# rimelq/VISTAF-RoboSkin-Vision-Integrated-Multimodal-Sensor

Hardware: AMD Instinct MI355X
Metric: frames/sec (224x224 -> force-map) at batch 256 (higher is better)
Workload: dtype f32; 1 GPU; BASELINE configs[2]: batch 256/GPU of 224x224x3 fp16 fringe frames (256 distinct frames) -> 224x224 f32 depth map + force scalars, full FTP path (inpaint, demod, unwrap, detrend, compose, force tail), constants scaled-224; inputs resident in HBM; global_batch=256, input_dtype=fp16, constants=scaled, parallelism=dp1, inflight_batches=3, frames_with_nonzero_status=0

## Files before the change

### vistaf-roboskin-vision-integrated-multimodal-sensor_amd/_lib.py

```python
from __future__ import annotations

import ctypes
import os

_HERE = os.path.dirname(os.path.abspath(__file__))
LIB_PATH = os.path.join(_HERE, "libvistaf_ftp.so")

NSCALARS = 16
NREFINFO = 8
NCONTACT = 16
MAX_CONTACTS = 64

FMT_GRAY_U8, FMT_BGR_U8, FMT_GRAY_F16, FMT_BGR_F16 = 0, 1, 2, 3
FRAME_OK, FRAME_EMPTY_RELIABLE, FRAME_QUEUE_OVERFLOW, FRAME_NO_CARRIER = 0, 1, 2, 3
CURVE_TYPES = {"linear0": 0, "linear": 1, "poly2": 2, "sat_exp": 3, "growth": 4, "hinge_saturating": 5}

EXPORTS = [
    "vistaf_ftp_abi_version", "vistaf_ftp_last_error", "vistaf_ftp_default_config", "vistaf_ftp_create",
    "vistaf_ftp_set_reference", "vistaf_ftp_get_reference_info", "vistaf_ftp_predict_batch", "vistaf_ftp_predict_pairs",
    "vistaf_ftp_get_pair_info", "vistaf_ftp_contacts",
    "vistaf_ftp_get_intermediate", "vistaf_ftp_stage_count", "vistaf_ftp_stage_name",
    "vistaf_ftp_enable_stage_timing", "vistaf_ftp_get_stage_times", "vistaf_ftp_destroy",
    "vistaf_depth_map_to_volume", "vistaf_predict_force_from_volume",
]
TEST_EXPORTS = ["vistaf_ftp_test_set", "vistaf_ftp_test_select", "vistaf_ftp_test_polyfit", "vistaf_ftp_test_gauss"]
TEMP_EXPORTS = ["vistaf_tempseg_default_config", "vistaf_tempseg_create", "vistaf_tempseg_destroy", "vistaf_tempseg_segment",
                "vistaf_temp_feature_planes", "vistaf_temp_color_support",
                "vistaf_temp_clamp_map", "vistaf_temp_inpaint_map", "vistaf_temp_fuse_maps", "vistaf_temp_oriented_blur"]
TEMPSEG_NINFO = 16
TEMPMODEL_EXPORTS = ["vistaf_tmodel_create", "vistaf_tmodel_destroy", "vistaf_tmodel_predict_maps", "vistaf_tmodel_predict_rows"]
TSENSOR_EXPORTS = ["vistaf_tsensor_default_config", "vistaf_tsensor_create", "vistaf_tsensor_destroy", "vistaf_tsensor_predict",
                   "vistaf_tsensor_stats_create", "vistaf_tsensor_stats_destroy", "vistaf_tsensor_map_statistics"]
TSENSOR_NINFO, TSENSOR_NMASKS, TSENSOR_NSTATS = TEMPSEG_NINFO + 4, 5, 6
ALIGN_EXPORTS = [
    "vistaf_align_default_config", "vistaf_align_create", "vistaf_align_destroy", "vistaf_align_geometry",
    "vistaf_align_set_reference", "vistaf_align_batch",
]


class Curve(ctypes.Structure):
    _fields_ = [("type", ctypes.c_int32), ("reserved", ctypes.c_int32),
                ("a", ctypes.c_double), ("b", ctypes.c_double), ("c", ctypes.c_double)]


_INT_FIELDS = [
    "patch_half_width_bins", "dc_exclusion", "fft_pad_px", "roi_erode_px", "apod_taper_px", "reliable_edge_margin_px",
    "poly_order", "frontier_zero_band_px", "valid_close_kernel", "valid_close_iters", "bad_pixel_enable",
    "bad_dilate_ksize", "bad_dilate_iters", "bad_inpaint_radius", "dilate_kernel_size", "dilate_iters", "n_fft_peaks",
    "plane_order_for_removal", "irls_iters", "hole_neighborhood_px", "hole_min_dist_px", "inpaint_radius",
]
_DBL_FIELDS = [
    "pre_blur_sigma_px", "amp_valid_percentile", "quality_smooth_sigma_px", "reliable_smooth_sigma_px", "illum_sigma_px",
    "bad_intensity_percentile", "bad_gradient_percentile", "contact_core_percentile", "contact_percentile",
    "min_contact_frac", "max_contact_frac", "unreliable_smooth_sigma_px", "contact_blob_min_peak_mm",
    "contact_blob_min_peak_rel_frac", "peak_max_dy_from_center", "irls_c", "grating_pitch_mm", "depth_eps_mm", "hole_known_fraction",
]


class CConfig(ctypes.Structure):
    _fields_ = [(n, ctypes.c_int32) for n in _INT_FIELDS] + [(n, ctypes.c_double) for n in _DBL_FIELDS]


class CTempFuseConfig(ctypes.Structure):
    _fields_ = [(n, ctypes.c_double) for n in ("color_t_min", "color_t_max", "color_guard_band", "switch_margin_c", "final_t_min", "final_t_max")]


class CTempSegConfig(ctypes.Structure):
    _fields_ = [(n, ctypes.c_int32) for n in ("seg_band_radius", "seg_dc_exclusion", "seg_illum_sigma", "sat_thresh_gray", "sat_dilate_ksize",
                                                "post_close_kx", "post_close_ky", "post_open_kx", "post_open_ky", "n_peaks")] + \
               [("seg_peak_max_dy_from_center", ctypes.c_double)]


class CTSensorConfig(ctypes.Structure):
    _fields_ = [("seg", CTempSegConfig), ("fuse", CTempFuseConfig)] + \
               [(n, ctypes.c_int32) for n in ("blur_ksize", "color_support_dilate", "wide_inpaint_radius", "color_inpaint_radius")] + \
               [(n, ctypes.c_double) for n in ("color_chroma_min", "color_clamp_pad", "smooth_sigma_across", "smooth_sigma_along")]


_lib = None


def load():
    global _lib
    if _lib is not None:
        return _lib
    if not os.path.exists(LIB_PATH):
        raise RuntimeError(
            f"{LIB_PATH} is missing: build it with `python __graft_entry__.py` (hipcc --offload-arch=gfx950). "
            "This package has no CPU path."
        )
    lib = ctypes.CDLL(LIB_PATH)
    vp, ci, cd = ctypes.c_void_p, ctypes.c_int, ctypes.c_double
    lib.vistaf_ftp_abi_version.restype = ci
    lib.vistaf_ftp_last_error.restype = ctypes.c_char_p
    lib.vistaf_ftp_default_config.argtypes = [ctypes.POINTER(CConfig)]
    lib.vistaf_ftp_create.argtypes = [ctypes.POINTER(CConfig), ci, ci, ci, ci, ci, ci, ctypes.POINTER(Curve), ci,
                                      ctypes.POINTER(Curve), ctypes.POINTER(vp)]
    lib.vistaf_ftp_set_reference.argtypes = [vp, vp, ci, vp]
    lib.vistaf_ftp_get_reference_info.argtypes = [vp, ctypes.POINTER(cd)]
    lib.vistaf_ftp_predict_batch.argtypes = [vp, vp, ci, ci, vp, vp, vp, vp, vp]
    lib.vistaf_ftp_predict_pairs.argtypes = [vp, vp, vp, ci, ci, vp, vp, vp, vp, vp]
    lib.vistaf_ftp_get_pair_info.argtypes = [vp, ci, ctypes.POINTER(cd), vp]
    lib.vistaf_ftp_contacts.argtypes = [vp, ci, ci, vp, vp, vp, vp]
    lib.vistaf_ftp_get_intermediate.argtypes = [vp, ctypes.c_char_p, vp, ci, ctypes.POINTER(ctypes.c_size_t), vp]
    lib.vistaf_ftp_stage_count.restype = ci
    lib.vistaf_ftp_stage_name.restype = ctypes.c_char_p
    lib.vistaf_ftp_stage_name.argtypes = [ci]
    lib.vistaf_ftp_enable_stage_timing.argtypes = [vp, ci]
    lib.vistaf_ftp_get_stage_times.argtypes = [vp, ctypes.POINTER(ctypes.c_float), ci]
    lib.vistaf_ftp_destroy.argtypes = [vp]
    lib.vistaf_ftp_destroy.restype = None
    lib.vistaf_depth_map_to_volume.argtypes = [vp, vp, ci, ci, ci, cd, cd, vp, vp]
    lib.vistaf_predict_force_from_volume.argtypes = [ctypes.POINTER(Curve), cd, ctypes.POINTER(cd)]
    lib.vistaf_ftp_test_set.argtypes = [vp, ctypes.c_char_p, ci]
    lib.vistaf_ftp_test_select.argtypes = [vp, vp, ctypes.c_size_t, vp, ci, vp, ci, vp, vp, ci, ci, ci, vp]
    lib.vistaf_ftp_test_polyfit.argtypes = [vp, vp, ci, ci, ctypes.c_float, ci, ci, vp, vp, ci, ci, ci, ci, vp]
    lib.vistaf_ftp_test_gauss.argtypes = [vp, vp, cd, ci, ci, ci, vp]
    lib.vistaf_tempseg_default_config.argtypes = [ctypes.POINTER(CTempSegConfig)]
    lib.vistaf_tempseg_create.argtypes = [ctypes.POINTER(CTempSegConfig), ci, ci, ctypes.POINTER(vp)]
    lib.vistaf_tempseg_destroy.argtypes = [vp]
    lib.vistaf_tempseg_destroy.restype = None
    lib.vistaf_tempseg_segment.argtypes = [vp, vp, vp, vp, vp, vp, vp, ctypes.POINTER(cd), vp]
    lib.vistaf_temp_feature_planes.argtypes = [vp, vp, ci, vp, vp, vp, vp, vp]
    lib.vistaf_temp_color_support.argtypes = [vp, vp, vp, vp, vp, vp, cd, ci, vp, vp, vp]
    lib.vistaf_temp_clamp_map.argtypes = [vp, vp, vp, cd, cd, vp, vp]
    lib.vistaf_temp_inpaint_map.argtypes = [vp, vp, vp, ci, vp, vp]
    lib.vistaf_temp_fuse_maps.argtypes = [vp, vp, vp, vp, ctypes.POINTER(CTempFuseConfig), vp, vp, ctypes.POINTER(ctypes.c_int64), vp]
    lib.vistaf_temp_oriented_blur.argtypes = [vp, vp, vp, cd, cd, cd, vp, vp]
    i32p, dp = ctypes.POINTER(ctypes.c_int32), ctypes.POINTER(cd)
    lib.vistaf_tmodel_create.argtypes = [ci, i32p, dp, dp, ci, ci, ci, i32p, dp, cd, ci, dp, dp, cd, cd, ci, ctypes.POINTER(vp)]
    lib.vistaf_tmodel_destroy.argtypes = [vp]
    lib.vistaf_tmodel_destroy.restype = None
    lib.vistaf_tmodel_predict_maps.argtypes = [ci, ctypes.POINTER(vp), ctypes.POINTER(vp), ctypes.POINTER(vp), ctypes.POINTER(vp), ctypes.c_int64,
                                               ctypes.c_int64, vp]
    lib.vistaf_tmodel_predict_rows.argtypes = [vp, vp, ci, ctypes.c_int64, vp, vp]
    lib.vistaf_tsensor_default_config.argtypes = [ctypes.POINTER(CTSensorConfig)]
    lib.vistaf_tsensor_create.argtypes = [ctypes.POINTER(CTSensorConfig), ci, ci, vp, vp, ctypes.POINTER(vp)]
    lib.vistaf_tsensor_destroy.argtypes = [vp]
    lib.vistaf_tsensor_destroy.restype = None
    lib.vistaf_tsensor_predict.argtypes = [vp, vp, vp, vp, vp, vp, vp, vp, ctypes.POINTER(cd), vp, ctypes.POINTER(cd), vp]
    lib.vistaf_tsensor_stats_create.argtypes = [ci, ci, ctypes.POINTER(vp)]
    lib.vistaf_tsensor_stats_destroy.argtypes = [vp]
    lib.vistaf_tsensor_stats_destroy.restype = None
    lib.vistaf_tsensor_map_statistics.argtypes = [vp, vp, vp, vp, ctypes.POINTER(cd), vp]
    for fn in EXPORTS + ALIGN_EXPORTS + TEST_EXPORTS + TEMP_EXPORTS + TEMPMODEL_EXPORTS + TSENSOR_EXPORTS:
        getattr(lib, fn)
    _lib = lib
    return lib


def check(rc: int):
    if rc != 0:
        msg = load().vistaf_ftp_last_error().decode("utf-8", "replace")
        if rc == -1:
            raise ValueError(msg)
        raise RuntimeError(f"vistaf_ftp error {rc}: {msg}")
```

### vistaf-roboskin-vision-integrated-multimodal-sensor_amd/csrc/api.hip

```cpp
#include <hip/hip_runtime.h>
#include <algorithm>
#include <cmath>
#include <cstdio>
#include <cstdlib>
#include <cstring>
#include <map>
#include <string>
#include <vector>

#include "../../include/vistaf_ftp.h"
#include "kernels.hpp"

using namespace vf;
#include "test_hooks.h"
#ifdef VISTAF_DEBUG
namespace vf { void telea_debug_dump(); void telea_window_debug_dump(int B); void telea_window_mw_debug_dump(int B); void fit_debug_dump(); void unwrap_big_debug_dump(); void unwrap_batch_debug_dump(); }
#endif

static thread_local std::string g_err;
static int fail(int code, const std::string &msg) { g_err = msg; return code; }
namespace vf { int set_error(int code, const std::string &msg) { return fail(code, msg); } }
#define HIPCHK(x)                                                                                         \
    do {                                                                                                  \
        hipError_t e_ = (x);                                                                              \
        if (e_ != hipSuccess) return fail(VISTAF_E_HIP, std::string(#x) + ": " + hipGetErrorString(e_)); \
    } while (0)

namespace {

struct GKern { float *d = nullptr; int k = 0; };

enum Stage { ST_GRAY_BAD = 0, ST_INPAINT, ST_PREPROC, ST_DEMOD, ST_RELIABLE, ST_UNWRAP_RANK, ST_UNWRAP, ST_UNWRAP_TREE, ST_DETREND, ST_SMOOTH_FLIP, ST_COMPOSE, ST_MM_BLOB,
             ST_TAIL, ST_COUNT };
const char *kStageNames[ST_COUNT] = {"gray+badpix", "inpaint (k_telea_window_mw)", "illum+blur+apod+median", "pruned-dft demod", "reliable mask",
                                     "unwrap check (k_unwrap_fast)", "unwrap flood (fallback)", "unwrap tree (fallback)", "detrend (3x IRLS)", "smooth+flip", "frontier+compose", "mm+blob filter", "tail"};

int cv_round(double v) { return (int)std::nearbyint(v); }

}

struct vistaf_ftp_handle {
    vistaf_ftp_config cfg;
    int h = 0, w = 0, P = 0, cx = 0, cy = 0, r = 0, maxB = 0;
    Curve hcurve, fcurve;
    int use_neg = 1;
    bool have_ref = false;

    uint8_t *roi = nullptr, *valid = nullptr;
    float *apo = nullptr, *roi_den = nullptr;
    GKern g_illum, g_pre, g_qual, g_rel, g_unrel;
    RowSpanSE se_bad, se_close, se_contact;

    double peak_x = 0, peak_y = 0, kx = 0, ky = 0, period = 0, mm_per_px = 0;
    int Hf = 0, Wf = 0, ph = 0, pw = 0, pmax = 0;
    double2 *Ex = nullptr, *Ey = nullptr, *Gx = nullptr, *Gy = nullptr, *cref = nullptr;
    float *win = nullptr, *amp_ref = nullptr;
    CarrierGeom *geom = nullptr;
    double2 *Exf = nullptr, *Eyf = nullptr, *search_tmp = nullptr;
    double *search_mag = nullptr, *search_peaks = nullptr;
    int search_cap = 0;
    CarrierGeom *pgeom = nullptr;
    double2 *pEx = nullptr, *pEy = nullptr, *pGx = nullptr, *pGy = nullptr, *pcref = nullptr;
    float *pamp_ref = nullptr, *pwin = nullptr, *hann_tab = nullptr;
    bool pairs_ready = false;
    Tiers tiers;
    bool keep_planes = false;

    std::map<std::string, std::pair<void *, size_t>> named;
    std::vector<void *> allocs;
    float *img, *grad, *tmpf, *blurA, *inorm, *iw, *amp, *prod, *quality, *wrapped, *unwrapped, *phase1, *resid0, *detr, *z0, *mplane,
        *num, *den, *hmap, *dist, *z0f, *snum, *unitless, *depth;
    double2 *field, *patch;
    double2 *tmpT;
    uint8_t *bad0, *bad1, *rel0, *rel1, *rel2, *reliable, *contact, *contact_d, *background, *cand, *kept;
    uint8_t *out_rel = nullptr, *hole_cand = nullptr;
    float *hole_med = nullptr, *hole_fill = nullptr;
    int32_t *labels, *area, *rowdist, *parent;
    unsigned int *peak_bits;
    uint16_t *morph_pre;
    void *inpaint_scratch, *inpaint_cl_scratch, *inpaint_win_scratch, *unwrap_scratch;
    void *big_scratch = nullptr;
    int32_t *unwrap_need;
    float *thr_hi, *thr_g, *mu, *amp_thr, *thr3, *thr_used, *bg_med, *core_thr, *core_med, *coef;
    int *cnt_a, *cnt_valid, *rel_count, *contact_count, *bg_count, *bad_count, *flipped;
    unsigned int *gmax;
    int32_t *status;
    int32_t *big_only;
    unsigned long long *cc_best;
    double *scalars;
    float *req_hi, *req_g, *req_med, *req_amp, *req_contact, *req_core;

    ContactScratch contacts_ws{};
    int last_batch = 0;
    bool last_pairs = false;

    bool timing = false;
    hipEvent_t ev[ST_COUNT + 1];
    bool ev_made = false;
    float stage_ms[ST_COUNT];
};

namespace {

template <typename T>
int dalloc(vistaf_ftp_handle *hd, T **p, size_t count, const char *name = nullptr, size_t per_frame = 0)
{
    void *q = nullptr;
    hipError_t e = hipMalloc(&q, count * sizeof(T) + 256);
    if (e != hipSuccess) return fail(VISTAF_E_HIP, std::string("hipMalloc: ") + hipGetErrorString(e));
    hd->allocs.push_back(q);
    *p = (T *)q;
    if (name) hd->named[name] = {q, per_frame};
    return 0;
}

int gauss_taps(double sigma, std::vector<float> &f)
{
    int n = cv_round(sigma * 4 * 2 + 1) | 1;
    if (n > 511) return fail(VISTAF_E_INVALID, "gaussian sigma too large (ksize > 511)");
    std::vector<double> t(n);
    double s2 = -0.5 / (sigma * sigma), sum = 0;
    for (int i = 0; i < n; i++) { double x = i - (n - 1) * 0.5; t[i] = std::exp(s2 * x * x); sum += t[i]; }
    f.resize(n);
    for (int i = 0; i < n; i++) f[i] = (float)(t[i] * (1.0 / sum));
    return 0;
}

int make_gkern(vistaf_ftp_handle *hd, double sigma, GKern *g)
{
    g->k = 0; g->d = nullptr;
    if (!(sigma > 0)) return 0;
    std::vector<float> f;
    int rc = gauss_taps(sigma, f);
    if (rc) return rc;
    const int n = (int)f.size();
    rc = dalloc(hd, &g->d, n);
    if (rc) return rc;
    if (hipMemcpy(g->d, f.data(), n * sizeof(float), hipMemcpyHostToDevice) != hipSuccess) return fail(VISTAF_E_HIP, "memcpy gkern");
    g->k = n;
    return 0;
}

bool chamfer_ball(float margin, RowSpanSE *se)
{
    const long long HV = 62587, DG = 89738;
    const long long M = (long long)std::floor((double)margin * 65536.0);
    if (M < 0) return false;
    const int R = (int)(M / HV);
    if (2 * R + 1 > 33 || R > 63) return false;
    se->k = std::max(3, 2 * R + 1);
    const int r = se->k / 2;
    for (int i = 0; i < se->k; i++) {
        const int dy = std::abs(i - r);
        int a = -1;
        for (int dx = 0; dx <= 63; dx++) {
            const long long mn = std::min(dx, dy), mx = std::max(dx, dy);
            if (HV * (mx - mn) + DG * mn <= M) a = dx; else break;
        }
        if (a < 0) { se->lo[i] = 1; se->hi[i] = -1; }
        else { se->lo[i] = (int8_t)-a; se->hi[i] = (int8_t)a; }
    }
    return true;
}

int make_se(int k, RowSpanSE *se, bool force_odd = true)
{
    if (force_odd) k = std::max(3, k | 1);
    if (k > 33) return fail(VISTAF_E_INVALID, "structuring element larger than 33");
    se->k = k;
    int r = k / 2, c = k / 2;
    double inv_r2 = r ? 1.0 / ((double)r * r) : 0.0;
    for (int i = 0; i < k; i++) {
        int dy = i - r;
        int dx = cv_round(c * std::sqrt((r * r - dy * dy) * inv_r2));
        int j1 = std::max(c - dx, 0), j2 = std::min(c + dx + 1, k);
        se->lo[i] = (int8_t)(j1 - c);
        se->hi[i] = (int8_t)(j2 - 1 - c);
    }
    return 0;
}

void blur(vistaf_ftp_handle *hd, const float *src, float *dst, const GKern &g, int B, hipStream_t st)
{
    launch_gauss_blur(src, hd->tmpf, dst, g.d, g.k, B, hd->h, hd->w, st);
}

bool fuses(const vistaf_ftp_handle *hd, const GKern &g) { return hd->tiers.fused_chains && g.k > 0 && g.k <= GF_MAXK; }

float q32_of(double pct) { return (float)pct / 100.0f; }

int upload_req(vistaf_ftp_handle *hd, float **d, const std::vector<float> &v)
{
    int rc = dalloc(hd, d, v.size());
    if (rc) return rc;
    if (hipMemcpy(*d, v.data(), v.size() * sizeof(float), hipMemcpyHostToDevice) != hipSuccess) return fail(VISTAF_E_HIP, "memcpy req");
    return 0;
}

void preprocess(vistaf_ftp_handle *hd, const void *frames, int format, int nframes, hipStream_t st, bool timed, const void *frames2 = nullptr)
{
    const vistaf_ftp_config &c = hd->cfg;
    int h = hd->h, w = hd->w, P = hd->P;
    if (timed) hipEventRecord(hd->ev[ST_GRAY_BAD], st);
    launch_to_gray(frames, format, hd->img, nframes, P, st);
    if (frames2) launch_to_gray(frames2, format, hd->img + (size_t)nframes * P, nframes, P, st);
    const int B = frames2 ? 2 * nframes : nframes;
    hipMemsetAsync(hd->bad_count, 0, sizeof(int) * B, st);
    if (c.bad_pixel_enable) {
        launch_sobel_mag(hd->img, hd->grad, B, h, w, st);
        launch_select(hd->img, hd->valid, 0, nullptr, false, hd->req_hi, 1, hd->thr_hi, hd->cnt_valid, B, P, st, hd->tiers.big_chain ? hd->big_scratch : nullptr);
        launch_select(hd->grad, hd->valid, 0, nullptr, false, hd->req_g, 1, hd->thr_g, nullptr, B, P, st, hd->tiers.big_chain ? hd->big_scratch : nullptr);
        launch_bad_flags(hd->img, hd->grad, hd->valid, hd->thr_hi, hd->thr_g, hd->bad0, B, P, st);
        uint8_t *src = hd->bad0, *dst = hd->bad1;
        if (c.bad_dilate_ksize > 1)
            for (int it = 0; it < c.bad_dilate_iters; it++) { launch_morph(src, dst, B, h, w, hd->se_bad, true, nullptr, nullptr, st); std::swap(src, dst); }
        if (src != hd->bad1) hipMemcpyAsync(hd->bad1, src, (size_t)B * P, hipMemcpyDeviceToDevice, st);
        launch_count_u8(hd->bad1, hd->bad_count, B, P, st);
        {
            int range = std::min(100, std::max(1, cv_round((double)c.bad_inpaint_radius)));
            const uint8_t *seq_mask = hd->bad1;
            const int32_t *only = nullptr;
            int mode = hd->tiers.inpaint;
            if (mode == 2 && (size_t)h * w > (size_t)8 * 14464) mode = 0;
            if (mode == 0 && inpaint_clusters_supported(range)) {
                uint8_t *bad_big = nullptr;
                ClusterPlanes left;
                launch_inpaint_clusters(hd->img, hd->bad1, range, hd->inpaint_cl_scratch, &bad_big, &left, B, h, w, st);
                if (timed) hipEventRecord(hd->ev[ST_INPAINT], st);
                launch_inpaint_big_clusters(hd->img, bad_big, range, hd->inpaint_scratch, hd->status, left, B, h, w, st, hd->tiers.big_queue_lds != 0,
                                            hd->tiers.big_gq_cap);
                if (hd->tiers.big_fallback) {
                    launch_inpaint_big_handback(hd->status, hd->big_only, B, st);
                    launch_inpaint_telea(hd->img, bad_big, range, hd->inpaint_scratch, hd->status, hd->big_only, B, h, w, st);
                }
            } else {
                if (timed && mode == 1) hipEventRecord(hd->ev[ST_INPAINT], st);
                if (mode != 1) only = launch_inpaint_window(hd->img, seq_mask, range, hd->inpaint_win_scratch, B, h, w, st, timed ? hd->ev[ST_INPAINT] : nullptr,
                                                               hd->tiers.telea_two_tier != 0, hd->tiers.telea_mw != 0);
                launch_inpaint_telea(hd->img, seq_mask, range, hd->inpaint_scratch, hd->status, only, B, h, w, st);
            }
        }
    } else if (timed) hipEventRecord(hd->ev[ST_INPAINT], st);
    if (timed) hipEventRecord(hd->ev[ST_PREPROC], st);
    blur(hd, hd->img, hd->blurA, hd->g_illum, B, st);
    if (fuses(hd, hd->g_pre)) launch_illum_pre_apod(hd->img, hd->blurA, hd->apo, hd->iw, hd->g_pre.d, hd->g_pre.k, B, h, w, st);
    else {
        launch_illum_norm(hd->img, hd->blurA, hd->inorm, B, P, st);
        const float *in = hd->inorm;
        if (hd->g_pre.k) { blur(hd, hd->inorm, hd->blurA, hd->g_pre, B, st); in = hd->blurA; }
        launch_mul_static(in, hd->apo, hd->iw, B, P, st);
    }
    launch_select(hd->iw, hd->valid, 0, nullptr, false, hd->req_med, 1, hd->mu, nullptr, B, P, st, hd->tiers.big_chain ? hd->big_scratch : nullptr);
}

std::vector<float> hann_patch(int ph, int pw)
{
    auto hann = [](int M, int i) -> float { return M == 1 ? 1.0f : (float)(0.5 + 0.5 * std::cos(3.14159265358979323846 * (double)(1 - M + 2 * i) / (double)(M - 1))); };
    std::vector<float> win((size_t)ph * pw);
    for (int a = 0; a < ph; a++)
        for (int c = 0; c < pw; c++) win[(size_t)a * pw + c] = hann(ph, a) * hann(pw, c);
    return win;
}

template <typename T>
int upload(vistaf_ftp_handle *hd, T **d, const std::vector<T> &v)
{
    int rc = dalloc(hd, d, v.size());
    if (rc) return rc;
    if (hipMemcpy(*d, v.data(), v.size() * sizeof(T), hipMemcpyHostToDevice) != hipSuccess) return fail(VISTAF_E_HIP, "memcpy upload");
    return 0;
}

}

extern "C" {

int vistaf_ftp_abi_version(void) { return VISTAF_FTP_ABI_VERSION; }
const char *vistaf_ftp_last_error(void) { return g_err.c_str(); }

int vistaf_ftp_default_config(vistaf_ftp_config *c)
{
    if (!c) return fail(VISTAF_E_INVALID, "null config");
    memset(c, 0, sizeof(*c));
    c->patch_half_width_bins = 10; c->dc_exclusion = 10; c->fft_pad_px = 96; c->roi_erode_px = 0; c->apod_taper_px = 120;
    c->reliable_edge_margin_px = 6; c->poly_order = 2; c->frontier_zero_band_px = 200; c->valid_close_kernel = 7;
    c->valid_close_iters = 1; c->bad_pixel_enable = 1; c->bad_dilate_ksize = 5; c->bad_dilate_iters = 1; c->bad_inpaint_radius = 3;
    c->dilate_kernel_size = 15; c->dilate_iters = 2; c->n_fft_peaks = 12; c->plane_order_for_removal = 1; c->irls_iters = 6;
    c->pre_blur_sigma_px = 1.5; c->amp_valid_percentile = 25.0; c->quality_smooth_sigma_px = 6.0; c->reliable_smooth_sigma_px = 2.5;
    c->illum_sigma_px = 45.0; c->bad_intensity_percentile = 99.9; c->bad_gradient_percentile = 99.7; c->contact_core_percentile = 8.0;
    c->contact_percentile = 92.0; c->min_contact_frac = 0.002; c->max_contact_frac = 0.40; c->unreliable_smooth_sigma_px = 9.0;
    c->contact_blob_min_peak_mm = 0.1; c->contact_blob_min_peak_rel_frac = 1.0 / 3.0; c->peak_max_dy_from_center = 0.12;
    c->irls_c = 4.685; c->grating_pitch_mm = 2.0; c->depth_eps_mm = 0.01;
    c->hole_neighborhood_px = 11; c->hole_min_dist_px = 4; c->inpaint_radius = 5; c->hole_known_fraction = 0.70;
    return 0;
}

void vistaf_ftp_destroy(vistaf_ftp_handle *hd)
{
    if (!hd) return;
    for (void *p : hd->allocs) hipFree(p);
    if (hd->ev_made) for (int i = 0; i <= ST_COUNT; i++) hipEventDestroy(hd->ev[i]);
    delete hd;
}

int vistaf_ftp_create(const vistaf_ftp_config *cfg, int h, int w, int cx, int cy, int r, int max_batch,
                      const vistaf_curve *height_curve, int use_negated_height, const vistaf_curve *force_curve,
                      vistaf_ftp_handle **out)
{
    if (!cfg || !out || !height_curve || !force_curve) return fail(VISTAF_E_INVALID, "null argument");
    if (h < 8 || w < 8 || max_batch < 1 || r < 1) return fail(VISTAF_E_INVALID, "bad geometry");
    if (height_curve->type < 0 || height_curve->type > 5 || force_curve->type < 0 || force_curve->type > 5)
        return fail(VISTAF_E_INVALID, "Unknown model type in calibration");
    if (cfg->poly_order < 1 || cfg->poly_order > 2 || cfg->plane_order_for_removal < 0 || cfg->plane_order_for_removal > 2)
        return fail(VISTAF_E_INVALID, "polynomial order must be 1 or 2 (plane_order_for_removal: 0 = no pre-removal)");
    if (cfg->irls_iters < 1) return fail(VISTAF_E_INVALID, "irls_iters must be >= 1 (robust_polyfit2d binds no coefficients otherwise)");
    if (cfg->n_fft_peaks < 1 || cfg->n_fft_peaks > 64) return fail(VISTAF_E_INVALID, "n_fft_peaks must be 1..64");
    int bwp = std::max(3, cfg->patch_half_width_bins);
    if (2 * bwp + 1 > 255) return fail(VISTAF_E_INVALID, "patch too wide");
    vistaf_ftp_handle *hd = new vistaf_ftp_handle();
    hd->cfg = *cfg; hd->h = h; hd->w = w; hd->P = h * w; hd->cx = cx; hd->cy = cy; hd->r = r; hd->maxB = max_batch;
    hd->hcurve = Curve{height_curve->type, height_curve->a, height_curve->b, height_curve->c};
    hd->fcurve = Curve{force_curve->type, force_curve->a, force_curve->b, force_curve->c};
    hd->use_neg = use_negated_height ? 1 : 0;
    int P = hd->P;
    size_t n = (size_t)max_batch * P;
    int rc = 0;
#define TRY(x) do { rc = (x); if (rc) { vistaf_ftp_destroy(hd); return rc; } } while (0)
    std::vector<uint8_t> roi(P), valid(P);
    std::vector<float> apo(P), roif(P);
    int r_valid = std::max(0, r - cfg->roi_erode_px);
    double r_in = std::max(0.0, (double)(r - cfg->apod_taper_px));
    for (int y = 0; y < h; y++)
        for (int x = 0; x < w; x++) {
            long d2 = (long)(x - cx) * (x - cx) + (long)(y - cy) * (y - cy);
            roi[(size_t)y * w + x] = d2 <= (long)r_valid * r_valid;
            double d = std::sqrt((double)d2);
            float a = 0.f;
            if (d <= r_in) a = 1.0f;
            else if (d <= r && cfg->apod_taper_px > 0) {
                double t = (d - r_in) / std::max(1e-6, (double)cfg->apod_taper_px);
                a = (float)(0.5 * (1.0 + std::cos(3.14159265358979323846 * t)));
            }
            apo[(size_t)y * w + x] = a;
            valid[(size_t)y * w + x] = a > 1e-6f;
            roif[(size_t)y * w + x] = roi[(size_t)y * w + x] ? 1.f : 0.f;
        }
    TRY(upload(hd, &hd->roi, roi)); TRY(upload(hd, &hd->valid, valid)); TRY(upload(hd, &hd->apo, apo));
    hd->named["roi"] = {hd->roi, 0};
    TRY(make_gkern(hd, cfg->illum_sigma_px, &hd->g_illum));
    if (!hd->g_illum.k) { vistaf_ftp_destroy(hd); return fail(VISTAF_E_INVALID, "illum_sigma_px must be > 0"); }
    TRY(make_gkern(hd, cfg->pre_blur_sigma_px, &hd->g_pre));
    TRY(make_gkern(hd, cfg->quality_smooth_sigma_px, &hd->g_qual));
    TRY(make_gkern(hd, cfg->reliable_smooth_sigma_px, &hd->g_rel));
    TRY(make_gkern(hd, cfg->unreliable_smooth_sigma_px, &hd->g_unrel));
    TRY(make_se(cfg->bad_dilate_ksize, &hd->se_bad));
    TRY(make_se(cfg->valid_close_kernel, &hd->se_close));
    {
        int k = cfg->dilate_kernel_size;
        if (k < 1 || k > 33) { vistaf_ftp_destroy(hd); return fail(VISTAF_E_INVALID, "dilate_kernel_size out of range"); }
        TRY(make_se(k, &hd->se_contact, false));
    }
    if (!(cfg->reliable_smooth_sigma_px > 0)) {
        if (cfg->hole_neighborhood_px < 1 || cfg->hole_neighborhood_px > 255 || cfg->hole_min_dist_px < 0 || cfg->inpaint_radius < 1 ||
            !(cfg->hole_known_fraction >= 0.0)) {
            vistaf_ftp_destroy(hd);
            return fail(VISTAF_E_INVALID, "hole-stage constants out of range");
        }
    }
#define PLANE(T, name) TRY(dalloc(hd, &hd->name, n, #name, (size_t)P * sizeof(T)))
    PLANE(float, img); PLANE(float, grad); PLANE(float, tmpf); PLANE(float, blurA); PLANE(float, inorm); PLANE(float, iw);
    PLANE(float, amp); PLANE(float, prod); PLANE(float, quality); PLANE(float, wrapped); PLANE(float, unwrapped); PLANE(float, phase1);
    PLANE(float, resid0); PLANE(float, detr); PLANE(float, z0); PLANE(float, mplane); PLANE(float, num); PLANE(float, den);
    PLANE(float, hmap); PLANE(float, dist); PLANE(float, z0f); PLANE(float, snum); PLANE(float, unitless); PLANE(float, depth);
    PLANE(double2, field);
    PLANE(uint8_t, bad0); PLANE(uint8_t, bad1); PLANE(uint8_t, rel0); PLANE(uint8_t, rel1); PLANE(uint8_t, rel2); PLANE(uint8_t, reliable);
    PLANE(uint8_t, contact); PLANE(uint8_t, contact_d); PLANE(uint8_t, background); PLANE(uint8_t, cand); PLANE(uint8_t, kept);
    if (!(cfg->reliable_smooth_sigma_px > 0)) { PLANE(uint8_t, out_rel); PLANE(uint8_t, hole_cand); }
    PLANE(int32_t, labels); PLANE(int32_t, area); PLANE(int32_t, rowdist); PLANE(int32_t, parent);
    PLANE(unsigned int, peak_bits);
    PLANE(uint16_t, morph_pre);
#undef PLANE
    {
        void *p = nullptr;
        TRY(dalloc(hd, (uint8_t **)&p, inpaint_scratch_bytes_per_frame(h, w) * max_batch)); hd->inpaint_scratch = p;
        TRY(dalloc(hd, (uint8_t **)&p, inpaint_cl_scratch_bytes_per_frame(h, w) * max_batch + 2048)); hd->inpaint_cl_scratch = p;
        TRY(dalloc(hd, (uint8_t **)&p, inpaint_win_scratch_bytes(max_batch))); hd->inpaint_win_scratch = p;
        TRY(dalloc(hd, (uint8_t **)&p, unwrap_scratch_bytes_per_frame(h, w) * max_batch + 1024)); hd->unwrap_scratch = p;
        if ((size_t)h * w >= 262144) { TRY(dalloc(hd, (uint8_t **)&p, big_scratch_bytes(max_batch, h, w))); hd->big_scratch = p; }
        TRY(dalloc(hd, &hd->unwrap_need, (size_t)max_batch, "unwrap_need", sizeof(int32_t)));
        HIPCHK(hipMemset(hd->unwrap_need, 0xff, (size_t)max_batch * sizeof(int32_t)));
    }
    int pmax = 2 * bwp + 1;
    hd->pmax = pmax;
    TRY(dalloc(hd, &hd->patch, (size_t)max_batch * pmax * pmax, "patch", (size_t)pmax * pmax * sizeof(double2)));
    TRY(dalloc(hd, &hd->tmpT, (size_t)max_batch * (size_t)std::max(h, w) * pmax));
    TRY(dalloc(hd, &hd->Ex, (size_t)w * pmax)); TRY(dalloc(hd, &hd->Gx, (size_t)w * pmax));
    TRY(dalloc(hd, &hd->Ey, (size_t)h * pmax)); TRY(dalloc(hd, &hd->Gy, (size_t)h * pmax));
    TRY(dalloc(hd, &hd->win, (size_t)pmax * pmax)); TRY(dalloc(hd, &hd->geom, 1));
    TRY(dalloc(hd, &hd->cref, (size_t)P)); TRY(dalloc(hd, &hd->amp_ref, (size_t)P));
    hd->named["cref"] = {hd->cref, 0}; hd->named["amp_ref"] = {hd->amp_ref, 0};
    size_t mb = max_batch;
    TRY(dalloc(hd, &hd->thr_hi, mb)); TRY(dalloc(hd, &hd->thr_g, mb)); TRY(dalloc(hd, &hd->mu, mb)); TRY(dalloc(hd, &hd->amp_thr, mb));
    TRY(dalloc(hd, &hd->thr3, mb * 3)); TRY(dalloc(hd, &hd->thr_used, mb)); TRY(dalloc(hd, &hd->bg_med, mb));
    TRY(dalloc(hd, &hd->core_thr, mb)); TRY(dalloc(hd, &hd->core_med, mb)); TRY(dalloc(hd, &hd->coef, mb * 6));
    TRY(dalloc(hd, &hd->cnt_a, mb)); TRY(dalloc(hd, &hd->cnt_valid, mb)); TRY(dalloc(hd, &hd->rel_count, mb));
    TRY(dalloc(hd, &hd->contact_count, mb)); TRY(dalloc(hd, &hd->bg_count, mb)); TRY(dalloc(hd, &hd->bad_count, mb));
    TRY(dalloc(hd, &hd->flipped, mb)); TRY(dalloc(hd, &hd->gmax, mb)); TRY(dalloc(hd, &hd->status, mb)); TRY(dalloc(hd, &hd->cc_best, mb));
    TRY(dalloc(hd, &hd->big_only, mb));
    TRY(dalloc(hd, &hd->scalars, mb * VISTAF_NSCALARS));
    TRY(dalloc(hd, &hd->hole_med, mb)); TRY(dalloc(hd, &hd->hole_fill, mb));
    {
        ContactScratch &cs = hd->contacts_ws;
        cs.cap = contact_root_capacity(h, w);
        TRY(dalloc(hd, &cs.arg, n)); TRY(dalloc(hd, &cs.list, mb * cs.cap)); TRY(dalloc(hd, &cs.nroots, mb)); TRY(dalloc(hd, &cs.nsel, mb));
        TRY(dalloc(hd, &cs.selkey, mb * VISTAF_MAX_CONTACTS)); TRY(dalloc(hd, &cs.part, contact_part_words(max_batch, P)));
    }
    hd->named["mu"] = {hd->mu, sizeof(float)}; hd->named["thr_hi"] = {hd->thr_hi, sizeof(float)}; hd->named["thr_g"] = {hd->thr_g, sizeof(float)};
    hd->named["coef"] = {hd->coef, 6 * sizeof(float)}; hd->named["thr3"] = {hd->thr3, 3 * sizeof(float)};
    hd->named["core_thr"] = {hd->core_thr, sizeof(float)}; hd->named["core_med"] = {hd->core_med, sizeof(float)};
    TRY(upload_req(hd, &hd->req_hi, {q32_of(cfg->bad_intensity_percentile)}));
    TRY(upload_req(hd, &hd->req_g, {q32_of(cfg->bad_gradient_percentile)}));
    TRY(upload_req(hd, &hd->req_med, {-1.0f}));
    TRY(upload_req(hd, &hd->req_amp, {q32_of(cfg->amp_valid_percentile)}));
    TRY(upload_req(hd, &hd->req_contact, {q32_of(cfg->contact_percentile), q32_of(95.0), q32_of(98.0)}));
    TRY(upload_req(hd, &hd->req_core, {q32_of(cfg->contact_core_percentile)}));
    TRY(dalloc(hd, &hd->roi_den, (size_t)P));
    if (hd->g_unrel.k) {
        float *tmp_roi = nullptr;
        TRY(upload(hd, &tmp_roi, roif));
        launch_gauss_rows(tmp_roi, hd->tmpf, hd->g_unrel.d, hd->g_unrel.k, 1, h, w, 0);
        launch_gauss_cols(hd->tmpf, hd->roi_den, hd->g_unrel.d, hd->g_unrel.k, 1, h, w, 0);
        std::vector<float> hden(P);
        if (hipMemcpy(hden.data(), hd->roi_den, P * sizeof(float), hipMemcpyDeviceToHost) != hipSuccess) { vistaf_ftp_destroy(hd); return fail(VISTAF_E_HIP, "roi_den readback"); }
        for (int i = 0; i < P; i++) hden[i] = hden[i] + 1e-6f;
        if (hipMemcpy(hd->roi_den, hden.data(), P * sizeof(float), hipMemcpyHostToDevice) != hipSuccess) { vistaf_ftp_destroy(hd); return fail(VISTAF_E_HIP, "roi_den upload"); }
    }
    hd->Hf = h + 2 * std::max(0, cfg->fft_pad_px);
    hd->Wf = w + 2 * std::max(0, cfg->fft_pad_px);
    if (hipDeviceSynchronize() != hipSuccess) { vistaf_ftp_destroy(hd); return fail(VISTAF_E_HIP, "create sync"); }
#undef TRY
    *out = hd;
    return 0;
}

static int reference_search(vistaf_ftp_handle *hd, int nb, CarrierGeom *geom_dev, hipStream_t st)
{
    const vistaf_ftp_config &c = hd->cfg;
    const int h = hd->h, w = hd->w, Hf = hd->Hf, Wf = hd->Wf, pad = std::max(0, c.fft_pad_px);
    if (hd->search_cap < nb) {
        int rc;
        if (!hd->Exf) {
            if ((rc = dalloc(hd, &hd->Exf, (size_t)w * (Wf / 2 + 1))) || (rc = dalloc(hd, &hd->Eyf, (size_t)Hf * h))) return rc;
            launch_build_full_tables(hd->Exf, hd->Eyf, h, w, pad, Hf, Wf, st);
        }
        const int cap = std::min(std::max(nb, 2 * hd->search_cap), std::max(nb, hd->maxB));
        if (hd->search_cap > 0) {
            HIPCHK(hipStreamSynchronize(st));
            for (void *q : {(void *)hd->search_tmp, (void *)hd->search_mag, (void *)hd->search_peaks}) {
                auto it = std::find(hd->allocs.begin(), hd->allocs.end(), q);
                if (it != hd->allocs.end()) { hipFree(q); hd->allocs.erase(it); }
            }
            hd->search_tmp = nullptr; hd->search_mag = nullptr; hd->search_peaks = nullptr; hd->search_cap = 0;
        }
        if ((rc = dalloc(hd, &hd->search_tmp, (size_t)cap * h * (Wf / 2 + 1) + 64)) || (rc = dalloc(hd, &hd->search_mag, (size_t)cap * Hf * Wf)) ||
            (rc = dalloc(hd, &hd->search_peaks, (size_t)cap * 192)))
            return rc;
        hd->search_cap = cap;
    }
    const int npk = c.n_fft_peaks;
    launch_dft_full_mag(hd->iw, hd->mu, hd->Exf, hd->Eyf, hd->search_tmp, hd->search_mag, nb, h, w, Hf, Wf, st);
    launch_top_peaks(hd->search_mag, nb, Hf, Wf, c.dc_exclusion, npk, hd->search_peaks, st);
    launch_carrier_choose(hd->search_peaks, npk, hd->search_mag, Hf, Wf, std::max(3, c.patch_half_width_bins), c.peak_max_dy_from_center, geom_dev, nb, st);
    return 0;
}

int vistaf_ftp_set_reference(vistaf_ftp_handle *hd, const void *d_ref, int format, void *stream)
{
    if (!hd || !d_ref) return fail(VISTAF_E_INVALID, "null argument");
    if (format < 0 || format > 3) return fail(VISTAF_E_INVALID, "bad frame format");
    hipStream_t st = (hipStream_t)stream;
    const vistaf_ftp_config &c = hd->cfg;
    int h = hd->h, w = hd->w, P = hd->P, Hf = hd->Hf, Wf = hd->Wf, pad = std::max(0, c.fft_pad_px);
    hd->have_ref = false;
    HIPCHK(hipMemsetAsync(hd->status, 0, sizeof(int32_t) * hd->maxB, st));
    preprocess(hd, d_ref, format, 1, st, false);
    int rc = reference_search(hd, 1, hd->geom, st);
    if (rc) return rc;
    CarrierGeom g;
    HIPCHK(hipMemcpyAsync(&g, hd->geom, sizeof(g), hipMemcpyDeviceToHost, st));
    HIPCHK(hipStreamSynchronize(st));
    if (!g.ok) return fail(VISTAF_E_NOCARRIER, "no carrier peak in the reference spectrum");
    hd->peak_x = g.peak_x; hd->peak_y = g.peak_y; hd->kx = g.kx; hd->ky = g.ky;
    hd->ph = g.ph; hd->pw = g.pw;
    {
        std::vector<float> win = hann_patch(g.ph, g.pw);
        HIPCHK(hipMemcpyAsync(hd->win, win.data(), win.size() * sizeof(float), hipMemcpyHostToDevice, st));
        HIPCHK(hipStreamSynchronize(st));
    }
    launch_build_tables(hd->geom, 0, hd->Ex, hd->Ey, hd->Gx, hd->Gy, 0, 0, 1, h, w, pad, Hf, Wf, hd->pmax, st);
    launch_dft_forward(hd->iw, hd->mu, hd->Ex, hd->Ey, 0, 0, hd->win, hd->tmpT, hd->patch, hd->pmax * hd->pmax, 1, h, w, hd->ph, hd->pw, st);
    launch_dft_inverse(hd->patch, hd->pmax * hd->pmax, hd->Gx, hd->Gy, 0, 0, hd->tmpT, hd->cref, hd->amp_ref, nullptr, nullptr, 0, nullptr, nullptr,
                       1, h, w, hd->ph, hd->pw, st);
    HIPCHK(hipStreamSynchronize(st));
    hd->period = g.period;
    hd->mm_per_px = hd->period > 1e-12 ? c.grating_pitch_mm / hd->period : 0.0;
    hd->have_ref = true;
    (void)P;
    return 0;
}

int vistaf_ftp_get_reference_info(const vistaf_ftp_handle *hd, double *o)
{
    if (!hd || !o) return fail(VISTAF_E_INVALID, "null argument");
    if (!hd->have_ref) return fail(VISTAF_E_STATE, "set_reference has not been called");
    o[0] = hd->peak_x; o[1] = hd->peak_y; o[2] = hd->kx; o[3] = hd->ky; o[4] = hd->Hf; o[5] = hd->Wf; o[6] = hd->period; o[7] = hd->mm_per_px;
    return 0;
}

static int post_demod(vistaf_ftp_handle *hd, int B, float *d_height_mm, uint8_t *d_reliable, double *d_scalars, int32_t *d_status,
                      const CarrierGeom *pair_geom, hipStream_t st, const int *bad_count = nullptr)
{
    if (!bad_count) bad_count = hd->bad_count;
    const vistaf_ftp_config &c = hd->cfg;
    int h = hd->h, w = hd->w, P = hd->P;
    bool timed = hd->timing;

    if (timed) hipEventRecord(hd->ev[ST_RELIABLE], st);
    const float *qual = hd->prod;
    if (hd->g_qual.k) { blur(hd, hd->prod, hd->quality, hd->g_qual, B, st); qual = hd->quality; }
    else HIPCHK(hipMemcpyAsync(hd->quality, hd->prod, (size_t)B * P * sizeof(float), hipMemcpyDeviceToDevice, st));
    qual = hd->quality;
    launch_select(qual, hd->roi, 0, nullptr, false, hd->req_amp, 1, hd->amp_thr, nullptr, B, P, st, hd->tiers.big_chain ? hd->big_scratch : nullptr);
    launch_threshold_mask(qual, hd->roi, hd->amp_thr, hd->rel0, B, P, st);
    {
        uint8_t *src = hd->rel0, *dst = hd->rel1;
        if (c.valid_close_iters >= 1 && 2 * c.valid_close_iters <= 4) {
            int ops[4];
            for (int it = 0; it < c.valid_close_iters; it++) { ops[it] = 1; ops[c.valid_close_iters + it] = 0; }
            launch_morph_seq(hd->rel0, hd->rel1, hd->rel2, B, h, w, hd->se_close, ops, 2 * c.valid_close_iters, hd->roi, nullptr, st, hd->morph_pre);
            src = hd->rel1;
        } else {
            for (int it = 0; it < 2 * c.valid_close_iters; it++) {
                const bool dil = it < c.valid_close_iters;
                launch_morph(src, dst, B, h, w, hd->se_close, dil, it == 2 * c.valid_close_iters - 1 ? hd->roi : nullptr, nullptr, st, hd->morph_pre);
                src = dst;
                dst = dst == hd->rel1 ? hd->rel2 : hd->rel1;
            }
        }
        launch_cc_label(src, hd->labels, B, h, w, st);
        launch_cc_largest(hd->labels, hd->area, hd->cc_best, hd->roi, hd->rel2, B, P, st);
    }
    if (c.reliable_edge_margin_px > 0) {
        RowSpanSE ball;
        if (chamfer_ball((float)c.reliable_edge_margin_px, &ball))
            launch_morph(hd->rel2, hd->reliable, B, h, w, ball, false, nullptr, nullptr, st, hd->morph_pre);
        else {
            launch_chamfer(hd->rel2, false, hd->rowdist, hd->dist, B, h, w, c.reliable_edge_margin_px + 1, st, hd->tiers.chamfer_twopass != 0);
            launch_erode_by_dist(hd->dist, hd->rel2, (float)c.reliable_edge_margin_px, hd->reliable, B, P, st);
        }
    } else HIPCHK(hipMemcpyAsync(hd->reliable, hd->rel2, (size_t)B * P, hipMemcpyDeviceToDevice, st));
    launch_count_u8(hd->reliable, hd->rel_count, B, P, st);
    launch_mark_empty(hd->rel_count, hd->status, B, st);

    if (timed) hipEventRecord(hd->ev[ST_UNWRAP_RANK], st);
    launch_unwrap(hd->wrapped, qual, hd->reliable, hd->unwrapped, hd->parent, hd->unwrap_scratch, hd->status, B, h, w, st,
                  timed ? hd->ev[ST_UNWRAP_TREE] : nullptr, timed ? hd->ev[ST_UNWRAP] : nullptr, hd->tiers.big_flood_handback != 0, hd->tiers.unwrap_fast ? hd->unwrap_need : nullptr);

    if (timed) hipEventRecord(hd->ev[ST_DETREND], st);
    if (c.plane_order_for_removal > 0)
        launch_robust_polyfit(hd->unwrapped, hd->reliable, c.plane_order_for_removal, c.irls_iters, (float)c.irls_c, 200, 500, hd->coef, hd->phase1, B, h, w, st, hd->tiers.big_chain ? hd->big_scratch : nullptr);
    else
        HIPCHK(hipMemcpyAsync(hd->phase1, hd->unwrapped, (size_t)B * P * sizeof(float), hipMemcpyDeviceToDevice, st));
    launch_robust_polyfit(hd->phase1, hd->reliable, c.poly_order, c.irls_iters, (float)c.irls_c, 200, 0, hd->coef, hd->resid0, B, h, w, st, hd->tiers.big_chain ? hd->big_scratch : nullptr);
    launch_select(hd->resid0, hd->reliable, (size_t)P, nullptr, true, hd->req_contact, 3, hd->thr3, nullptr, B, P, st, hd->tiers.big_chain ? hd->big_scratch : nullptr);
    launch_contact_mask(hd->resid0, hd->reliable, hd->thr3, hd->rel_count, hd->contact_count, c.min_contact_frac, c.max_contact_frac,
                        hd->contact, hd->thr_used, B, P, st);
    {
        int iters = c.dilate_iters;
        if (iters <= 0) HIPCHK(hipMemcpyAsync(hd->contact_d, hd->contact, (size_t)B * P, hipMemcpyDeviceToDevice, st));
        else if (iters <= 4) {
            int ops[4] = {1, 1, 1, 1};
            launch_morph_seq(hd->contact, hd->contact_d, hd->cand, B, h, w, hd->se_contact, ops, iters, nullptr, hd->reliable, st, hd->morph_pre);
        } else {
            uint8_t *src = hd->contact, *dst = hd->contact_d;
            uint8_t *bufs[2] = {hd->contact_d, hd->cand};
            for (int it = 0; it < iters; it++) {
                dst = bufs[it & 1];
                launch_morph(src, dst, B, h, w, hd->se_contact, true, nullptr, it == iters - 1 ? hd->reliable : nullptr, st, hd->morph_pre);
                src = dst;
            }
            if (src != hd->contact_d) HIPCHK(hipMemcpyAsync(hd->contact_d, src, (size_t)B * P, hipMemcpyDeviceToDevice, st));
        }
    }
    launch_background(hd->reliable, hd->contact_d, hd->rel_count, hd->bg_count, hd->background, B, P, st);
    launch_robust_polyfit(hd->phase1, hd->background, c.poly_order, c.irls_iters, (float)c.irls_c, 200, 0, hd->coef, hd->detr, B, h, w, st, hd->tiers.big_chain ? hd->big_scratch : nullptr);
    launch_select(hd->detr, hd->background, (size_t)P, nullptr, false, hd->req_med, 1, hd->bg_med, nullptr, B, P, st, hd->tiers.big_chain ? hd->big_scratch : nullptr);

    if (timed) hipEventRecord(hd->ev[ST_SMOOTH_FLIP], st);
    const bool smooth_rel = hd->g_rel.k > 0;
    if (fuses(hd, hd->g_rel)) launch_smooth_reliable(hd->detr, hd->bg_med, hd->reliable, hd->hmap, hd->g_rel.d, hd->g_rel.k, B, h, w, st);
    else if (smooth_rel) {
        launch_sub_scalar_mask(hd->detr, hd->bg_med, hd->reliable, hd->z0, hd->mplane, B, P, st);
        blur(hd, hd->z0, hd->num, hd->g_rel, B, st);
        blur(hd, hd->mplane, hd->den, hd->g_rel, B, st);
        launch_div_planes(hd->num, hd->den, hd->hmap, B, P, st);
    } else launch_zeroed_keep_nan(hd->detr, hd->bg_med, hd->reliable, hd->hmap, B, P, st);
    launch_select(hd->hmap, hd->reliable, (size_t)P, nullptr, false, hd->req_core, 1, hd->core_thr, nullptr, B, P, st, hd->tiers.big_chain ? hd->big_scratch : nullptr);
    launch_select(hd->hmap, hd->reliable, (size_t)P, hd->core_thr, false, hd->req_med, 1, hd->core_med, nullptr, B, P, st, hd->tiers.big_chain ? hd->big_scratch : nullptr);
    launch_core_flip(hd->hmap, hd->core_med, hd->flipped, B, P, st);

    const uint8_t *orel = hd->reliable;
    if (!smooth_rel) {
        const int ksz = std::max(3, c.hole_neighborhood_px | 1);
        launch_chamfer(hd->reliable, false, hd->rowdist, hd->dist, B, h, w, c.hole_min_dist_px + 1, st, hd->tiers.chamfer_twopass != 0);
        launch_hole_candidates(hd->hmap, hd->reliable, hd->dist, ksz, (float)c.hole_known_fraction, (float)c.hole_min_dist_px, hd->hole_cand, B, h, w, st);
        launch_select(hd->hmap, hd->reliable, (size_t)P, nullptr, false, hd->req_med, 1, hd->hole_med, nullptr, B, P, st, hd->tiers.big_chain ? hd->big_scratch : nullptr);
        launch_hole_tmp(hd->hmap, hd->reliable, hd->hole_cand, hd->hole_med, hd->z0, B, P, st);
        launch_select(hd->z0, hd->reliable, (size_t)P, nullptr, false, hd->req_med, 1, hd->hole_fill, nullptr, B, P, st, hd->tiers.big_chain ? hd->big_scratch : nullptr);
        launch_hole_zin(hd->z0, hd->hole_fill, B, P, st);
        {
            const int range = std::min(100, std::max(1, cv_round((double)c.inpaint_radius)));
            const int32_t *only = nullptr;
            if (hd->tiers.inpaint != 1) only = launch_inpaint_window(hd->z0, hd->hole_cand, range, hd->inpaint_win_scratch, B, h, w, st, nullptr, hd->tiers.telea_two_tier != 0, hd->tiers.telea_mw != 0);
            launch_inpaint_telea(hd->z0, hd->hole_cand, range, hd->inpaint_scratch, hd->status, only, B, h, w, st);
        }
        launch_hole_merge(hd->hmap, hd->reliable, hd->hole_cand, hd->z0, hd->out_rel, B, P, st);
        orel = hd->out_rel;
    }

    if (timed) hipEventRecord(hd->ev[ST_COMPOSE], st);
    bool use_band = c.frontier_zero_band_px > 0;
    float band = (float)c.frontier_zero_band_px;
    if (use_band) launch_chamfer_pair(orel, hd->rowdist, hd->dist, hd->area, hd->depth, B, h, w, c.frontier_zero_band_px + 2, st, hd->tiers.chamfer_twopass != 0);
    else HIPCHK(hipMemsetAsync(hd->dist, 0x7f, (size_t)B * P * sizeof(float), st));
    const bool fuse_compose = fuses(hd, hd->g_unrel);
    if (fuse_compose)
        launch_compose_finalize_mm(hd->hmap, orel, hd->roi, hd->dist, use_band ? band : 1.0f, hd->roi_den, use_band ? hd->depth : hd->dist, band,
                                   use_band ? 1 : 0, hd->hcurve, hd->use_neg, hd->unitless, hd->depth, hd->cand, hd->gmax, hd->g_unrel.d, hd->g_unrel.k,
                                   B, h, w, st);
    else {
        launch_frontier_compose(hd->hmap, orel, hd->roi, hd->dist, use_band ? band : 1.0f, hd->z0f, B, P, st);
        if (hd->g_unrel.k) blur(hd, hd->z0f, hd->snum, hd->g_unrel, B, st);
        launch_finalize_unitless(hd->z0f, hd->g_unrel.k ? hd->snum : nullptr, hd->roi_den, orel, hd->roi, use_band ? hd->depth : hd->dist, band, use_band ? 1 : 0,
                                 hd->unitless, B, P, st);
    }

    if (timed) hipEventRecord(hd->ev[ST_MM_BLOB], st);
    if (!fuse_compose) launch_to_mm(hd->unitless, hd->roi, hd->hcurve, hd->use_neg, hd->depth, hd->cand, hd->gmax, B, P, st);
    launch_cc_label(hd->cand, hd->labels, B, h, w, st);
    launch_blob_filter(hd->depth, hd->cand, hd->labels, hd->peak_bits, hd->gmax, c.contact_blob_min_peak_mm,
                       c.contact_blob_min_peak_rel_frac, hd->kept, B, P, st);

    if (timed) hipEventRecord(hd->ev[ST_TAIL], st);
    PostParams pp;
    pp.mm_per_px = hd->mm_per_px; pp.depth_eps_mm = c.depth_eps_mm; pp.period_px = hd->period; pp.force_curve = hd->fcurve;
    pp.pair_geom = pair_geom; pp.grating_pitch_mm = c.grating_pitch_mm;
    launch_tail(hd->depth, nullptr, hd->unitless, hd->roi, pp, hd->scalars, VISTAF_NSCALARS, nullptr, B, P, st, hd->tiers.big_chain ? hd->big_scratch : nullptr,
                hd->big_scratch ? big_scratch_bytes(hd->maxB, h, w) : 0);
    launch_fill_scalars(hd->scalars, VISTAF_NSCALARS, hd->rel_count, hd->flipped, hd->amp_thr, hd->thr_used, hd->bg_med, bad_count, B, st);
    launch_copy_out(hd->depth, orel, hd->status, d_height_mm, d_reliable, B, P, st);
    if (d_scalars) HIPCHK(hipMemcpyAsync(d_scalars, hd->scalars, sizeof(double) * VISTAF_NSCALARS * B, hipMemcpyDeviceToDevice, st));
    if (d_status) HIPCHK(hipMemcpyAsync(d_status, hd->status, sizeof(int32_t) * B, hipMemcpyDeviceToDevice, st));
    if (timed) {
        hipEventRecord(hd->ev[ST_COUNT], st);
        hipEventSynchronize(hd->ev[ST_COUNT]);
        for (int i = 0; i < ST_COUNT; i++) hipEventElapsedTime(&hd->stage_ms[i], hd->ev[i], hd->ev[i + 1]);
    }
#ifdef VISTAF_DEBUG
    if (getenv("VISTAF_TELEA_DBG")) { hipStreamSynchronize(st); telea_debug_dump(); telea_window_debug_dump(B); telea_window_mw_debug_dump(B); fit_debug_dump(); unwrap_big_debug_dump(); unwrap_batch_debug_dump(); }
#endif
    hipError_t e = hipGetLastError();
    if (e != hipSuccess) return fail(VISTAF_E_HIP, std::string("launch: ") + hipGetErrorString(e));
    hd->last_batch = B; hd->last_pairs = pair_geom != nullptr;
    return 0;
}

int vistaf_ftp_predict_batch(vistaf_ftp_handle *hd, const void *d_frames, int format, int B, float *d_height_mm, uint8_t *d_reliable,
                             double *d_scalars, int32_t *d_status, void *stream)
{
    if (!hd || !d_frames) return fail(VISTAF_E_INVALID, "null argument");
    if (!hd->have_ref) return fail(VISTAF_E_STATE, "set_reference has not been called");
    if (B < 1 || B > hd->maxB) return fail(VISTAF_E_STATE, "batch exceeds max_batch");
    if (format < 0 || format > 3) return fail(VISTAF_E_INVALID, "bad frame format");
    if (!(hd->period > 1e-12)) return fail(VISTAF_E_STATE, "Invalid estimated_grating_period_px");
    hipStream_t st = (hipStream_t)stream;
    int h = hd->h, w = hd->w;
    bool timed = hd->timing;
    if (timed && !hd->ev_made) { for (int i = 0; i <= ST_COUNT; i++) hipEventCreate(&hd->ev[i]); hd->ev_made = true; }
    HIPCHK(hipMemsetAsync(hd->status, 0, sizeof(int32_t) * B, st));

    preprocess(hd, d_frames, format, B, st, timed);

    if (timed) hipEventRecord(hd->ev[ST_DEMOD], st);
    launch_dft_forward(hd->iw, hd->mu, hd->Ex, hd->Ey, 0, 0, hd->win, hd->tmpT, hd->patch, hd->pmax * hd->pmax, B, h, w, hd->ph, hd->pw, st);
    launch_dft_inverse(hd->patch, hd->pmax * hd->pmax, hd->Gx, hd->Gy, 0, 0, hd->tmpT, hd->keep_planes ? hd->field : nullptr, hd->amp, hd->cref,
                       hd->amp_ref, 0, hd->prod, hd->wrapped, B, h, w, hd->ph, hd->pw, st);
    return post_demod(hd, B, d_height_mm, d_reliable, d_scalars, d_status, nullptr, st);
}

int vistaf_ftp_predict_pairs(vistaf_ftp_handle *hd, const void *d_refs, const void *d_defs, int format, int B, float *d_height_mm,
                             uint8_t *d_reliable, double *d_scalars, int32_t *d_status, void *stream)
{
    if (!hd || !d_refs || !d_defs) return fail(VISTAF_E_INVALID, "null argument");
    if (B < 1 || B > hd->maxB) return fail(VISTAF_E_STATE, "batch exceeds max_batch");
    if (format < 0 || format > 3) return fail(VISTAF_E_INVALID, "bad frame format");
    hipStream_t st = (hipStream_t)stream;
    const vistaf_ftp_config &c = hd->cfg;
    int h = hd->h, w = hd->w, P = hd->P, pad = std::max(0, c.fft_pad_px), pm = hd->pmax;
    bool timed = hd->timing;
    if (timed && !hd->ev_made) { for (int i = 0; i <= ST_COUNT; i++) hipEventCreate(&hd->ev[i]); hd->ev_made = true; }
    if (!hd->pairs_ready) {
        int rc;
        size_t mb = hd->maxB;
        if ((rc = dalloc(hd, &hd->pgeom, mb)) || (rc = dalloc(hd, &hd->pEx, mb * w * pm)) || (rc = dalloc(hd, &hd->pGx, mb * w * pm)) ||
            (rc = dalloc(hd, &hd->pEy, mb * h * pm)) || (rc = dalloc(hd, &hd->pGy, mb * h * pm)) || (rc = dalloc(hd, &hd->pcref, mb * P)) ||
            (rc = dalloc(hd, &hd->pamp_ref, mb * P)) || (rc = dalloc(hd, &hd->pwin, mb * pm * pm)) || (rc = dalloc(hd, &hd->hann_tab, (size_t)(pm + 1) * pm)))
            return rc;
        std::vector<float> tab((size_t)(pm + 1) * pm, 0.0f);
        for (int M = 1; M <= pm; M++) {
            const std::vector<float> row = hann_patch(1, M);
            std::copy(row.begin(), row.end(), tab.begin() + (size_t)M * pm);
        }
        HIPCHK(hipMemcpy(hd->hann_tab, tab.data(), tab.size() * sizeof(float), hipMemcpyHostToDevice));
        hd->pairs_ready = true;
    }
    HIPCHK(hipMemsetAsync(hd->status, 0, sizeof(int32_t) * B, st));
    const size_t sx = (size_t)w * pm, sy = (size_t)h * pm;
    const bool together = 2 * B <= hd->maxB;
    const float *iw_def = hd->iw, *mu_def = hd->mu;
    const int *bad_def = hd->bad_count;
    if (together) {
        HIPCHK(hipMemsetAsync(hd->status + B, 0, sizeof(int32_t) * B, st));
        preprocess(hd, d_refs, format, B, st, timed, d_defs);
        iw_def = hd->iw + (size_t)B * P; mu_def = hd->mu + B; bad_def = hd->bad_count + B;
    } else preprocess(hd, d_refs, format, B, st, false);
    int rc = reference_search(hd, B, hd->pgeom, st);
    if (rc) return rc;
    launch_pair_status(hd->pgeom, pm, hd->status, together ? hd->status + B : nullptr, B, st);
    launch_build_tables(hd->pgeom, 1, hd->pEx, hd->pEy, hd->pGx, hd->pGy, sx, sy, B, h, w, pad, hd->Hf, hd->Wf, pm, st, hd->hann_tab, hd->pwin);
    launch_dft_forward(hd->iw, hd->mu, hd->pEx, hd->pEy, sx, sy, hd->pwin, hd->tmpT, hd->patch, pm * pm, B, h, w, pm, pm, st, pm * pm);
    launch_dft_inverse(hd->patch, pm * pm, hd->pGx, hd->pGy, sx, sy, hd->tmpT, hd->pcref, hd->pamp_ref, nullptr, nullptr, 0, nullptr, nullptr, B, h, w,
                       pm, pm, st, hd->pgeom);
    if (!together) preprocess(hd, d_defs, format, B, st, timed);
    if (timed) hipEventRecord(hd->ev[ST_DEMOD], st);
    launch_dft_forward(iw_def, mu_def, hd->pEx, hd->pEy, sx, sy, hd->pwin, hd->tmpT, hd->patch, pm * pm, B, h, w, pm, pm, st, pm * pm);
    launch_dft_inverse(hd->patch, pm * pm, hd->pGx, hd->pGy, sx, sy, hd->tmpT, hd->keep_planes ? hd->field : nullptr, hd->amp, hd->pcref, hd->pamp_ref,
                       (size_t)P, hd->prod, hd->wrapped, B, h, w, pm, pm, st, hd->pgeom);
    return post_demod(hd, B, d_height_mm, d_reliable, d_scalars, d_status, hd->pgeom, st, bad_def);
}

int vistaf_ftp_get_pair_info(vistaf_ftp_handle *hd, int batch, double *out , void *stream)
{
    if (!hd || !out) return fail(VISTAF_E_INVALID, "null argument");
    if (!hd->pairs_ready || batch < 1 || batch > hd->maxB) return fail(VISTAF_E_STATE, "predict_pairs has not been called");
    std::vector<CarrierGeom> g(batch);
    HIPCHK(hipMemcpyAsync(g.data(), hd->pgeom, sizeof(CarrierGeom) * batch, hipMemcpyDeviceToHost, (hipStream_t)stream));
    HIPCHK(hipStreamSynchronize((hipStream_t)stream));
    for (int b = 0; b < batch; b++) {
        double *o = out + (size_t)b * VISTAF_NREFINFO;
        o[0] = g[b].peak_x; o[1] = g[b].peak_y; o[2] = g[b].kx; o[3] = g[b].ky; o[4] = hd->Hf; o[5] = hd->Wf; o[6] = g[b].period;
        o[7] = g[b].period > 1e-12 ? hd->cfg.grating_pitch_mm / g[b].period : 0.0;
    }
    return 0;
}

int vistaf_ftp_contacts(vistaf_ftp_handle *hd, int B, int max_contacts, double *d_contacts, int32_t *d_count, int8_t *d_contact_index, void *stream)
{
    if (!hd || !d_contacts || !d_count) return fail(VISTAF_E_INVALID, "null argument");
    if (max_contacts < 1 || max_contacts > VISTAF_MAX_CONTACTS) return fail(VISTAF_E_INVALID, "max_contacts must be 1..64");
    if (hd->last_batch == 0) return fail(VISTAF_E_STATE, "no predict_batch / predict_pairs before contacts");
    if (B != hd->last_batch) return fail(VISTAF_E_STATE, "batch differs from the last predict's");
    const vistaf_ftp_config &c = hd->cfg;
    PostParams pp;
    pp.mm_per_px = hd->mm_per_px; pp.depth_eps_mm = c.depth_eps_mm; pp.period_px = hd->period; pp.force_curve = hd->fcurve;
    pp.pair_geom = hd->last_pairs ? hd->pgeom : nullptr; pp.grating_pitch_mm = c.grating_pitch_mm;
    launch_contacts(hd->depth, hd->kept, hd->labels, hd->peak_bits, hd->status, pp, hd->contacts_ws, max_contacts, d_contacts, VISTAF_NCONTACT, d_count,
                    d_contact_index, B, hd->h, hd->w, (hipStream_t)stream);
    hipError_t e = hipGetLastError();
    if (e != hipSuccess) return fail(VISTAF_E_HIP, std::string("launch: ") + hipGetErrorString(e));
    return 0;
}

int vistaf_ftp_get_intermediate(vistaf_ftp_handle *hd, const char *name, void *d_dst, int batch, size_t *bytes_per_frame, void *stream)
{
    if (!hd || !name) return fail(VISTAF_E_INVALID, "null argument");
    auto it = hd->named.find(name);
    if (it == hd->named.end()) return fail(VISTAF_E_INVALID, std::string("unknown intermediate: ") + name);
    size_t per = it->second.second;
    size_t total = per ? per * (size_t)batch : (std::string(name) == "cref" ? (size_t)hd->P * sizeof(double2) : std::string(name) == "amp_ref" ? (size_t)hd->P * sizeof(float) : (size_t)hd->P);
    if (bytes_per_frame) *bytes_per_frame = per ? per : total;
    if (d_dst) HIPCHK(hipMemcpyAsync(d_dst, it->second.first, total, hipMemcpyDeviceToDevice, (hipStream_t)stream));
    return 0;
}

int vistaf_ftp_stage_count(void) { return ST_COUNT; }
const char *vistaf_ftp_stage_name(int i) { return (i >= 0 && i < ST_COUNT) ? kStageNames[i] : ""; }
int vistaf_ftp_enable_stage_timing(vistaf_ftp_handle *hd, int enable)
{
    if (!hd) return fail(VISTAF_E_INVALID, "null handle");
    hd->timing = enable != 0;
    return 0;
}
int vistaf_ftp_get_stage_times(vistaf_ftp_handle *hd, float *ms_out, int n)
{
    if (!hd || !ms_out) return fail(VISTAF_E_INVALID, "null argument");
    for (int i = 0; i < n && i < ST_COUNT; i++) ms_out[i] = hd->stage_ms[i];
    return 0;
}

int vistaf_ftp_test_set(vistaf_ftp_handle *hd, const char *name, int value)
{
    if (!hd || !name) return fail(VISTAF_E_INVALID, "null argument");
    const std::string n(name);
    if (n == "inpaint_tier" && value >= 0 && value <= 2) hd->tiers.inpaint = value;
    else if (n == "big_flood_handback") hd->tiers.big_flood_handback = value != 0;
    else if (n == "chamfer_twopass") hd->tiers.chamfer_twopass = value != 0;
    else if (n == "telea_two_tier") hd->tiers.telea_two_tier = value != 0;
    else if (n == "telea_mw") hd->tiers.telea_mw = value != 0;
    else if (n == "big_queue_lds") hd->tiers.big_queue_lds = value != 0;
    else if (n == "big_gq_cap" && (value == 0 || (value >= 64 && (value & (value - 1)) == 0))) hd->tiers.big_gq_cap = value;
    else if (n == "big_fallback") hd->tiers.big_fallback = value != 0;
    else if (n == "unwrap_fast") hd->tiers.unwrap_fast = value != 0;
    else if (n == "big_chain") hd->tiers.big_chain = value != 0;
    else if (n == "fused_chains") hd->tiers.fused_chains = value != 0;
    else if (n == "keep_planes") hd->keep_planes = value != 0;
    else return fail(VISTAF_E_INVALID, "unknown test hook or value: " + n);
    return 0;
}

namespace {
int hook_scratch(int variant, int B, int h, int w, bool chain_ok, void **scratch)
{
    *scratch = nullptr;
    if (variant < 0 || variant > 2) return fail(VISTAF_E_INVALID, "variant must be 0, 1 or 2");
    if (variant == 2 && !chain_ok) return fail(VISTAF_E_INVALID, "variant 2: the k_big.hip chain does not take this batch");
    if (variant == 1 || (variant == 0 && (size_t)h * w < 262144)) return 0;
    HIPCHK(hipMalloc(scratch, big_scratch_bytes(B, h, w) + 256));
    return 0;
}
int hook_finish(void *a, void *b, hipStream_t st)
{
    const hipError_t e1 = hipGetLastError(), e2 = hipStreamSynchronize(st);
    if (a) (void)hipFree(a);
    if (b) (void)hipFree(b);
    if (e1 != hipSuccess) return fail(VISTAF_E_HIP, std::string("launch: ") + hipGetErrorString(e1));
    if (e2 != hipSuccess) return fail(VISTAF_E_HIP, std::string("sync: ") + hipGetErrorString(e2));
    return 0;
}
}

int vistaf_ftp_test_select(const float *vals, const uint8_t *mask, size_t mask_stride, const float *le_thr, int use_abs, const float *reqs, int nreq,
                           float *out, int *counts, int B, int P, int variant, void *stream)
{
    if (!vals || !mask || !reqs || !out || B < 1 || P < 1 || nreq < 1 || (mask_stride != 0 && mask_stride != (size_t)P))
        return fail(VISTAF_E_INVALID, "bad argument");
    void *scratch = nullptr;
    int rc = hook_scratch(variant, B, 1, P, nreq <= 4 && big_frames(B, P), &scratch);
    if (rc) return rc;
    launch_select(vals, mask, mask_stride, le_thr, use_abs != 0, reqs, nreq, out, counts, B, P, (hipStream_t)stream, scratch);
    return hook_finish(scratch, nullptr, (hipStream_t)stream);
}

int vistaf_ftp_test_polyfit(const float *z, const uint8_t *mask, int order, int iters, float c, int min_count, int min_mask_count, float *coef,
                            float *resid, int B, int h, int w, int variant, void *stream)
{
    if (!z || !mask || !coef || !resid || B < 1 || h < 1 || w < 1 || (size_t)h * w > 0x7fffffffull || order < 1 || order > 2 || iters < 1)
        return fail(VISTAF_E_INVALID, "bad argument");
    void *scratch = nullptr;
    int rc = hook_scratch(variant, B, h, w, big_frames(B, h * w), &scratch);
    if (rc) return rc;
    const int inst = polyfit_variant(B, h, w, scratch != nullptr);
    launch_robust_polyfit(z, mask, order, iters, c, min_count, min_mask_count, coef, resid, B, h, w, (hipStream_t)stream, scratch);
    rc = hook_finish(scratch, nullptr, (hipStream_t)stream);
    return rc ? rc : inst;
}

int vistaf_ftp_test_gauss(const float *src, float *dst, double sigma, int B, int h, int w, void *stream)
{
    if (!src || !dst || src == dst || B < 1 || h < 1 || w < 1 || !(sigma > 0)) return fail(VISTAF_E_INVALID, "bad argument");
    std::vector<float> f;
    int rc = gauss_taps(sigma, f);
    if (rc) return rc;
    float *taps = nullptr, *tmp = nullptr;
    HIPCHK(hipMalloc((void **)&taps, f.size() * sizeof(float)));
    if (hipMalloc((void **)&tmp, (size_t)B * h * w * sizeof(float)) != hipSuccess) { (void)hipFree(taps); return fail(VISTAF_E_HIP, "hipMalloc"); }
    if (hipMemcpy(taps, f.data(), f.size() * sizeof(float), hipMemcpyHostToDevice) != hipSuccess) {
        (void)hipFree(taps); (void)hipFree(tmp);
        return fail(VISTAF_E_HIP, "memcpy taps");
    }
    launch_gauss_blur(src, tmp, dst, taps, (int)f.size(), B, h, w, (hipStream_t)stream);
    return hook_finish(taps, tmp, (hipStream_t)stream);
}

int vistaf_depth_map_to_volume(const float *d_height, const uint8_t *d_roi, int batch, int h, int w, double mm_per_px,
                               double depth_eps_mm, double *d_out, void *stream)
{
    if (!d_height || !d_out || batch < 1 || h < 1 || w < 1) return fail(VISTAF_E_INVALID, "bad argument");
    PostParams pp;
    pp.mm_per_px = mm_per_px; pp.depth_eps_mm = depth_eps_mm; pp.period_px = 0; pp.force_curve = Curve{0, 0, 0, 0};
    launch_tail(d_height, d_roi, nullptr, nullptr, pp, nullptr, 0, d_out, batch, h * w, (hipStream_t)stream);
    hipError_t e = hipGetLastError();
    if (e != hipSuccess) return fail(VISTAF_E_HIP, std::string("launch: ") + hipGetErrorString(e));
    return 0;
}

int vistaf_predict_force_from_volume(const vistaf_curve *curve, double volume_cm3, double *force_out)
{
    if (!curve || !force_out) return fail(VISTAF_E_INVALID, "null argument");
    if (curve->type < 0 || curve->type > 5) return fail(VISTAF_E_INVALID, "Unknown model type in force calibration JSON");
    Curve cv{curve->type, curve->a, curve->b, curve->c};
    *force_out = curve_eval(cv, volume_cm3);
    return 0;
}

}
```

### vistaf-roboskin-vision-integrated-multimodal-sensor_amd/csrc/k_cc_dist.hip

```cpp
#include <cstdlib>
#include "kernels.hpp"

namespace vf {

__global__ void k_threshold_mask(const float *__restrict__ q, const uint8_t *__restrict__ roi, const float *__restrict__ thr,
                                 uint8_t *__restrict__ out, int P)
{
    int p = blockIdx.x * blockDim.x + threadIdx.x;
    size_t b = blockIdx.y;
    if (p >= P) return;
    float v = q[b * (size_t)P + p];
    out[b * (size_t)P + p] = (uint8_t)(roi[p] && finitef(v) && v >= thr[b]);
}
void launch_threshold_mask(const float *q, const uint8_t *roi, const float *thr, uint8_t *out, int B, int P, hipStream_t st)
{
    hipLaunchKernelGGL(k_threshold_mask, dim3((P + 255) / 256, B), dim3(256), 0, st, q, roi, thr, out, P);
}

__device__ inline int ld_label(const int32_t *L, int i)
{
    return __hip_atomic_load(&L[i], __ATOMIC_RELAXED, __HIP_MEMORY_SCOPE_AGENT);
}
__device__ inline int cc_find(const int32_t *L, int i)
{
    int p = ld_label(L, i);
    while (p != i) { i = p; p = ld_label(L, i); }
    return i;
}
__device__ inline void cc_unite(int32_t *L, int a, int b)
{
    for (;;) {
        a = cc_find(L, a);
        b = cc_find(L, b);
        if (a == b) return;
        if (a > b) { int t = a; a = b; b = t; }
        int old = atomicMin(&L[b], a);
        if (old == b) return;
        b = old;
    }
}

__global__ void k_cc_init(const uint8_t *__restrict__ mask, int32_t *__restrict__ labels, int P, int w)
{
    const int p = blockIdx.x * blockDim.x + threadIdx.x;
    const size_t b = blockIdx.y;
    const int lane = threadIdx.x & 63;
    const bool in = p < P && mask[b * (size_t)P + (p < P ? p : 0)] != 0;
    const int x = p % w;
    const unsigned long long bits = __ballot(in);
    const unsigned long long rowstart = __ballot(x == 0);
    const unsigned long long starts = bits & (~(bits << 1) | rowstart | 1ull);
    if (p >= P) return;
    int lab = -1;
    if (in) {
        const unsigned long long upto = starts & (lane == 63 ? ~0ull : ((2ull << lane) - 1ull));
        lab = p - lane + (63 - __clzll((long long)upto));
    }
    labels[b * (size_t)P + p] = lab;
}
__global__ void k_cc_merge(const uint8_t *__restrict__ mask, int32_t *__restrict__ labels, int h, int w)
{
    int p = blockIdx.x * blockDim.x + threadIdx.x;
    size_t b = blockIdx.y;
    int P = h * w;
    if (p >= P) return;
    const uint8_t *m = mask + b * (size_t)P;
    int32_t *L = labels + b * (size_t)P;
    if (!m[p]) return;
    int y = p / w, x = p - y * w;
    const bool left = x > 0 && m[p - 1];
    if ((threadIdx.x & 63) == 0 && left) cc_unite(L, p, p - 1);
    if (y > 0) {
        const bool ul = x > 0 && m[p - w - 1], up = m[p - w] != 0, ur = x < w - 1 && m[p - w + 1];
        if ((ul || up) && !left) cc_unite(L, p, ul ? p - w - 1 : p - w);
        if (ur && !up) cc_unite(L, p, p - w + 1);
    }
}
__global__ void k_cc_flatten(const uint8_t *__restrict__ mask, int32_t *__restrict__ labels, int P)
{
    int p = blockIdx.x * blockDim.x + threadIdx.x;
    size_t b = blockIdx.y;
    if (p >= P) return;
    int32_t *L = labels + b * (size_t)P;
    if (mask[b * (size_t)P + p]) { int r = cc_find(L, p); if (r != p) atomicMin(&L[p], r); }
}

__device__ inline uint32_t cc16_min(uint16_t *L, int i, uint32_t val)
{
    uint32_t *wp = (uint32_t *)L + (i >> 1);
    const int sh = (i & 1) * 16;
    uint32_t old = *(volatile uint32_t *)wp;
    for (;;) {
        uint32_t cur = (old >> sh) & 0xffffu;
        if (cur <= val) return cur;
        uint32_t nw = (old & ~(0xffffu << sh)) | (val << sh);
        uint32_t prev = atomicCAS(wp, old, nw);
        if (prev == old) return cur;
        old = prev;
    }
}
__device__ inline int cc16_find(uint16_t *L, int i)
{
    volatile uint16_t *V = L;
    for (;;) {
        int p = V[i];
        if (p == i) return i;
        int g = V[p];
        if (g == p) return p;
        V[i] = (uint16_t)g;
        i = g;
    }
}
__device__ inline void cc16_unite(uint16_t *L, int a, int b)
{
    for (;;) {
        a = cc16_find(L, a);
        b = cc16_find(L, b);
        if (a == b) return;
        if (a > b) { int t = a; a = b; b = t; }
        uint32_t old = cc16_min(L, b, (uint32_t)a);
        if ((int)old == b) return;
        b = (int)old;
    }
}

template <bool MLDS>
__global__ __launch_bounds__(1024) void k_cc_label_lds(const uint8_t *__restrict__ mask, int32_t *__restrict__ labels, int h, int w)
{
    extern __shared__ __attribute__((aligned(16))) uint16_t L16[];
    size_t b = blockIdx.x;
    int P = h * w;
    const uint8_t *mg = mask + b * (size_t)P;
    uint8_t *ml = (uint8_t *)(L16 + ((P + 2 + 7) & ~7));
    if (MLDS) {
        for (int p = threadIdx.x * 4; p < P; p += blockDim.x * 4) {
            if (p + 3 < P && ((((uintptr_t)mg) & 3) == 0)) *(uint32_t *)(ml + p) = *(const uint32_t *)(mg + p);
            else for (int k = 0; k < 4 && p + k < P; k++) ml[p + k] = mg[p + k];
        }
        __syncthreads();
    }
    const uint8_t *m = MLDS ? (const uint8_t *)ml : mg;
    {
        const int lane = threadIdx.x & 63, wid = threadIdx.x >> 6, nwv = blockDim.x >> 6;
        for (int y = wid; y < h; y += nwv) {
            int carry = -1;
            for (int x0 = 0; x0 < w; x0 += 64) {
                const int x = x0 + lane;
                const bool on = x < w && m[y * w + x];
                int lz = (x < w && !on) ? x : (int)0x80000000;
                int t;
                t = __builtin_amdgcn_update_dpp((int)0x80000000, lz, 0x111, 0xf, 0xf, false); lz = t > lz ? t : lz;
                t = __builtin_amdgcn_update_dpp((int)0x80000000, lz, 0x112, 0xf, 0xf, false); lz = t > lz ? t : lz;
                t = __builtin_amdgcn_update_dpp((int)0x80000000, lz, 0x114, 0xf, 0xf, false); lz = t > lz ? t : lz;
                t = __builtin_amdgcn_update_dpp((int)0x80000000, lz, 0x118, 0xf, 0xf, false); lz = t > lz ? t : lz;
                t = __builtin_amdgcn_update_dpp((int)0x80000000, lz, 0x142, 0xa, 0xf, false); lz = t > lz ? t : lz;
                t = __builtin_amdgcn_update_dpp((int)0x80000000, lz, 0x143, 0xc, 0xf, false); lz = t > lz ? t : lz;
                lz = lz > carry ? lz : carry;
                carry = __builtin_amdgcn_readlane(lz, 63);
                if (x < w) L16[y * w + x] = on ? (uint16_t)(y * w + lz + 1) : (uint16_t)0xffffu;
            }
        }
    }
    if ((P & 1) && threadIdx.x == 0) L16[P] = 0xffffu;
    __syncthreads();
    for (int p = threadIdx.x; p < P; p += blockDim.x) {
        if (!m[p]) continue;
        const int y = p / w, x = p - y * w;
        if (y == 0) continue;
        const bool left = x > 0 && m[p - 1];
        const bool ul = x > 0 && m[p - w - 1], up = m[p - w] != 0, ur = x < w - 1 && m[p - w + 1];
        if ((ul || up) && !left) cc16_unite(L16, p, ul ? p - w - 1 : p - w);
        if (ur && !up) cc16_unite(L16, p, p - w + 1);
    }
    __syncthreads();
    int32_t *out = labels + b * (size_t)P;
    for (int p = threadIdx.x; p < P; p += blockDim.x) out[p] = m[p] ? cc16_find(L16, p) : -1;
}

void launch_cc_label(const uint8_t *mask, int32_t *labels, int B, int h, int w, hipStream_t st)
{
    int P = h * w;
    const size_t forest = (size_t)((P + 2 + 7) & ~7) * 2;
    if (P <= 65535 && forest + (size_t)P + 16 <= 160 * 1024) {
        static DynLdsOnce lds_once;
        ensure_dyn_lds(lds_once, (const void *)k_cc_label_lds<true>, 160 * 1024);
        hipLaunchKernelGGL(k_cc_label_lds<true>, dim3(B), dim3(1024), forest + (size_t)P + 16, st, mask, labels, h, w);
        return;
    }
    if (P <= 65535 && forest <= 150 * 1024) {
        static DynLdsOnce lds_once;
        ensure_dyn_lds(lds_once, (const void *)k_cc_label_lds<false>, 160 * 1024);
        hipLaunchKernelGGL(k_cc_label_lds<false>, dim3(B), dim3(1024), forest, st, mask, labels, h, w);
        return;
    }
    const dim3 g((P + 255) / 256, B);
    hipLaunchKernelGGL(k_cc_init, g, dim3(256), 0, st, mask, labels, P, w);
    hipLaunchKernelGGL(k_cc_merge, g, dim3(256), 0, st, mask, labels, h, w);
    hipLaunchKernelGGL(k_cc_flatten, g, dim3(256), 0, st, mask, labels, P);
}

__global__ __launch_bounds__(1024) void k_cc_largest(const int32_t *__restrict__ labels, int32_t *__restrict__ area,
                                                     const uint8_t *__restrict__ and_static, uint8_t *__restrict__ out, int P)
{
    __shared__ unsigned long long scratch[16];
    size_t b = blockIdx.x;
    const int32_t *L = labels + b * (size_t)P;
    int32_t *A = area + b * (size_t)P;
    int lane = threadIdx.x & 63;
    constexpr int U = 4;
    const int T = blockDim.x;
    for (int p = threadIdx.x; p < P; p += T) A[p] = 0;
    __threadfence_block();
    __syncthreads();
    int Pr = ((P + U * 1024 - 1) / (U * 1024)) * (U * 1024);
    int run_root = -1, run_cnt = 0;
    for (int p0 = threadIdx.x; p0 < Pr; p0 += U * T) {
        int root[U];
#pragma unroll
        for (int u = 0; u < U; u++) { int p = p0 + u * T; root[u] = p < P ? L[p] : -1; }
#pragma unroll
        for (int u = 0; u < U; u++) {
            unsigned long long active = __ballot(root[u] >= 0);
            while (active) {
                int leader = __ffsll((long long)active) - 1;
                int r0 = __builtin_amdgcn_readlane(root[u], leader);
                unsigned long long same = __ballot(root[u] == r0);
                if (r0 == run_root) run_cnt += (int)__popcll(same);
                else {
                    if (run_root >= 0 && lane == 0) atomicAdd(&A[run_root], run_cnt);
                    run_root = r0; run_cnt = (int)__popcll(same);
                }
                active &= ~same;
            }
        }
    }
    if (run_root >= 0 && lane == 0) atomicAdd(&A[run_root], run_cnt);
    __threadfence_block();
    __syncthreads();
    unsigned long long best = 0;
    for (int p0 = threadIdx.x; p0 < P; p0 += U * T) {
        int lab[U], ar[U];
#pragma unroll
        for (int u = 0; u < U; u++) {
            int p = p0 + u * T;
            lab[u] = p < P ? L[p] : -1;
            ar[u] = p < P ? __hip_atomic_load(&A[p], __ATOMIC_RELAXED, __HIP_MEMORY_SCOPE_AGENT) : 0;
        }
#pragma unroll
        for (int u = 0; u < U; u++) {
            int p = p0 + u * T;
            if (lab[u] != p) continue;
            unsigned long long key = ((unsigned long long)(unsigned int)ar[u] << 32) | (unsigned int)(0x7fffffff - p);
            if (key > best) best = key;
        }
    }
    best = block_max_u64(best, scratch);
    int broot = (best >> 32) ? (0x7fffffff - (int)(best & 0xffffffffu)) : -2;
    for (int p0 = threadIdx.x; p0 < P; p0 += U * T) {
        int lab[U];
        uint8_t as[U];
#pragma unroll
        for (int u = 0; u < U; u++) { int p = p0 + u * T; lab[u] = p < P ? L[p] : -1; as[u] = (p < P && and_static) ? and_static[p] : (uint8_t)1; }
#pragma unroll
        for (int u = 0; u < U; u++) { int p = p0 + u * T; if (p < P) out[b * (size_t)P + p] = (uint8_t)(lab[u] == broot && as[u]); }
    }
}

__global__ __launch_bounds__(256) void k_ccl_area(const int32_t *__restrict__ labels, int32_t *__restrict__ area, int P)
{
    constexpr int U = 4;
    const size_t b = blockIdx.y;
    const int32_t *L = labels + b * (size_t)P;
    int32_t *A = area + b * (size_t)P;
    const int lane = threadIdx.x & 63;
    const int p0 = (blockIdx.x * (blockDim.x >> 6) + (threadIdx.x >> 6)) * (64 * U) + lane;
    int root[U];
#pragma unroll
    for (int u = 0; u < U; u++) { const int p = p0 + u * 64; root[u] = p < P ? L[p] : -1; }
    int run_root = -1, run_cnt = 0;
#pragma unroll
    for (int u = 0; u < U; u++) {
        unsigned long long active = __ballot(root[u] >= 0);
        while (active) {
            const int leader = __ffsll((long long)active) - 1;
            const int r0 = __builtin_amdgcn_readlane(root[u], leader);
            const unsigned long long same = __ballot(root[u] == r0);
            if (r0 == run_root) run_cnt += (int)__popcll(same);
            else {
                if (run_root >= 0 && lane == 0) atomicAdd(&A[run_root], run_cnt);
                run_root = r0; run_cnt = (int)__popcll(same);
            }
            active &= ~same;
        }
    }
    if (run_root >= 0 && lane == 0) atomicAdd(&A[run_root], run_cnt);
}
__global__ __launch_bounds__(256) void k_ccl_best(const int32_t *__restrict__ labels, const int32_t *__restrict__ area, unsigned long long *__restrict__ best, int P)
{
    const size_t b = blockIdx.y;
    const int p = blockIdx.x * blockDim.x + threadIdx.x;
    unsigned long long key = 0;
    if (p < P && labels[b * (size_t)P + p] == p)
        key = ((unsigned long long)(unsigned int)area[b * (size_t)P + p] << 32) | (unsigned int)(0x7fffffff - p);
    if (!__ballot(key != 0)) return;
    for (int o = 32; o; o >>= 1) { const unsigned long long v = __shfl_xor(key, o, 64); key = v > key ? v : key; }
    if ((threadIdx.x & 63) == 0) atomicMax(&best[b], key);
}
__global__ __launch_bounds__(256) void k_ccl_out(const int32_t *__restrict__ labels, const unsigned long long *__restrict__ best,
                                                 const uint8_t *__restrict__ and_static, uint8_t *__restrict__ out, int P)
{
    const size_t b = blockIdx.y;
    const int p = blockIdx.x * blockDim.x + threadIdx.x;
    if (p >= P) return;
    const unsigned long long k = best[b];
    const int broot = (k >> 32) ? (0x7fffffff - (int)(k & 0xffffffffu)) : -2;
    out[b * (size_t)P + p] = (uint8_t)(labels[b * (size_t)P + p] == broot && (and_static ? and_static[p] : (uint8_t)1));
}

void launch_cc_largest(const int32_t *labels, int32_t *area_scratch, unsigned long long *best, const uint8_t *and_static,
                       uint8_t *out, int B, int P, hipStream_t st)
{
    if (best && P >= 262144 && B <= 192) {
        (void)hipMemsetAsync(area_scratch, 0, (size_t)B * P * sizeof(int32_t), st);
        (void)hipMemsetAsync(best, 0, (size_t)B * sizeof(unsigned long long), st);
        hipLaunchKernelGGL(k_ccl_area, dim3((P + 1023) / 1024, B), dim3(256), 0, st, labels, area_scratch, P);
        const dim3 g((P + 255) / 256, B);
        hipLaunchKernelGGL(k_ccl_best, g, dim3(256), 0, st, labels, area_scratch, best, P);
        hipLaunchKernelGGL(k_ccl_out, g, dim3(256), 0, st, labels, best, and_static, out, P);
        return;
    }
    hipLaunchKernelGGL(k_cc_largest, dim3(B), dim3(1024), 0, st, labels, area_scratch, and_static, out, P);
}

constexpr int CH_INF = 1 << 20;
constexpr int CH_HV = 62587;
constexpr int CH_DG = 89738;
constexpr int CH_DIST_MAX = 0x7fffffff >> 2;

__global__ __launch_bounds__(256) void k_rowdist(const uint8_t *__restrict__ src, int invert, int32_t *__restrict__ g, int h, int w, int B)
{
    const int row = blockIdx.x * 4 + (threadIdx.x >> 6), lane = threadIdx.x & 63;
    if (row >= B * h) return;
    const uint8_t *s = src + (size_t)row * w;
    int32_t *o = g + (size_t)row * w;
    const int none = (int)0x80000000;
    int carry = none;
    for (int x0 = 0; x0 < w; x0 += 64) {
        const int x = x0 + lane;
        const bool zero = x < w && (invert ? (s[x] != 0) : (s[x] == 0));
        int lz = zero ? x : none, t;
        t = __builtin_amdgcn_update_dpp(none, lz, 0x111, 0xf, 0xf, false); lz = t > lz ? t : lz;
        t = __builtin_amdgcn_update_dpp(none, lz, 0x112, 0xf, 0xf, false); lz = t > lz ? t : lz;
        t = __builtin_amdgcn_update_dpp(none, lz, 0x114, 0xf, 0xf, false); lz = t > lz ? t : lz;
        t = __builtin_amdgcn_update_dpp(none, lz, 0x118, 0xf, 0xf, false); lz = t > lz ? t : lz;
        t = __builtin_amdgcn_update_dpp(none, lz, 0x142, 0xa, 0xf, false); lz = t > lz ? t : lz;
        t = __builtin_amdgcn_update_dpp(none, lz, 0x143, 0xc, 0xf, false); lz = t > lz ? t : lz;
        lz = lz > carry ? lz : carry;
        carry = __builtin_amdgcn_readlane(lz, 63);
        if (x < w) o[x] = lz == none ? CH_INF : x - lz;
    }
    const int far = 0x7fffffff;
    carry = far;
    for (int x0 = ((w - 1) / 64) * 64; x0 >= 0; x0 -= 64) {
        const int x = x0 + lane;
        const bool zero = x < w && (invert ? (s[x] != 0) : (s[x] == 0));
        int nz = zero ? x : far, t;
        nz = __builtin_amdgcn_ds_bpermute((63 - lane) << 2, nz);
        t = __builtin_amdgcn_update_dpp(far, nz, 0x111, 0xf, 0xf, false); nz = t < nz ? t : nz;
        t = __builtin_amdgcn_update_dpp(far, nz, 0x112, 0xf, 0xf, false); nz = t < nz ? t : nz;
        t = __builtin_amdgcn_update_dpp(far, nz, 0x114, 0xf, 0xf, false); nz = t < nz ? t : nz;
        t = __builtin_amdgcn_update_dpp(far, nz, 0x118, 0xf, 0xf, false); nz = t < nz ? t : nz;
        t = __builtin_amdgcn_update_dpp(far, nz, 0x142, 0xa, 0xf, false); nz = t < nz ? t : nz;
        t = __builtin_amdgcn_update_dpp(far, nz, 0x143, 0xc, 0xf, false); nz = t < nz ? t : nz;
        nz = __builtin_amdgcn_ds_bpermute((63 - lane) << 2, nz);
        nz = nz < carry ? nz : carry;
        carry = __builtin_amdgcn_readlane(nz, 0);
        if (x < w && nz != far) { const int d = nz - x; if (d < o[x]) o[x] = d; }
    }
}

__global__ void k_chamfer_cols(const int32_t *__restrict__ g, float *__restrict__ dist, int h, int w, int cap)
{
    int x = blockIdx.x * blockDim.x + threadIdx.x;
    int y = blockIdx.y;
    size_t b = blockIdx.z;
    if (x >= w) return;
    const int32_t *G = g + b * (size_t)h * w;
    int best = CH_DIST_MAX;
    for (int dy = 0; dy <= cap; dy++) {
        if ((long long)dy * CH_HV >= best) break;
        for (int s = 0; s < 2; s++) {
            if (s && !dy) break;
            int yy = s ? y + dy : y - dy;
            if (yy < 0 || yy >= h) continue;
            int gx = G[(size_t)yy * w + x];
            if (gx >= CH_INF) continue;
            int mn = gx < dy ? gx : dy, mx = gx < dy ? dy : gx;
            int c = CH_HV * (mx - mn) + CH_DG * mn;
            if (c < best) best = c;
        }
    }
    dist[b * (size_t)h * w + (size_t)y * w + x] = (float)best * (1.0f / 65536.0f);
}

constexpr int CH2_INF = 0x7fffffff >> 2;
constexpr int CH2_RING = 4;

__device__ inline int ch2_shr1(int v, int fill) { return __builtin_amdgcn_update_dpp(fill, v, 0x138, 0xf, 0xf, false); }
__device__ inline int ch2_shl1(int v, int fill) { return __builtin_amdgcn_update_dpp(fill, v, 0x130, 0xf, 0xf, false); }
__device__ inline int ch2_scan_min_up(int v)
{
    const int big = 0x7fffffff;
    int t;
    t = __builtin_amdgcn_update_dpp(big, v, 0x111, 0xf, 0xf, false); v = t < v ? t : v;
    t = __builtin_amdgcn_update_dpp(big, v, 0x112, 0xf, 0xf, false); v = t < v ? t : v;
    t = __builtin_amdgcn_update_dpp(big, v, 0x114, 0xf, 0xf, false); v = t < v ? t : v;
    t = __builtin_amdgcn_update_dpp(big, v, 0x118, 0xf, 0xf, false); v = t < v ? t : v;
    t = __builtin_amdgcn_update_dpp(big, v, 0x142, 0xa, 0xf, false); v = t < v ? t : v;
    t = __builtin_amdgcn_update_dpp(big, v, 0x143, 0xc, 0xf, false); v = t < v ? t : v;
    return v;
}

template <int PPL>
__global__ __launch_bounds__(64) void k_chamfer2(const uint8_t *__restrict__ src_all, int invert, int32_t *__restrict__ tmp_all,
                                                 float *__restrict__ dist_all, int32_t *__restrict__ tmp2_all, float *__restrict__ dist2_all, int B,
                                                 int h, int w)
{
    const int lane = threadIdx.x;
    size_t b = blockIdx.x;
    if (b >= (size_t)B) { b -= B; invert = !invert; tmp_all = tmp2_all; dist_all = dist2_all; }
    const size_t P = (size_t)h * w;
    const uint8_t *src = src_all + b * P;
    int32_t *tmp = tmp_all + b * P;
    float *dist = dist_all + b * P;
    const int x0 = lane * PPL;
    const int step = CH_HV * PPL;

    {
        int up[PPL];
#pragma unroll
        for (int j = 0; j < PPL; j++) up[j] = CH2_INF;
        uint8_t ring[CH2_RING][PPL];
#pragma unroll
        for (int r = 0; r < CH2_RING; r++)
#pragma unroll
            for (int j = 0; j < PPL; j++) ring[r][j] = (r < h && x0 + j < w) ? src[(size_t)r * w + x0 + j] : (uint8_t)0;
        for (int y0 = 0; y0 < h; y0 += CH2_RING) {
#pragma unroll
            for (int r = 0; r < CH2_RING; r++) {
                const int y = y0 + r;
                if (y >= h) break;
                const int upl = ch2_shr1(up[PPL - 1], CH2_INF), upr = ch2_shl1(up[0], CH2_INF);
                int t[PPL];
#pragma unroll
                for (int j = 0; j < PPL; j++) {
                    const bool in = x0 + j < w;
                    const bool zero = in && (invert ? ring[r][j] != 0 : ring[r][j] == 0);
                    const int a = (j > 0 ? up[j - 1] : upl) + CH_DG, c = (j < PPL - 1 ? up[j + 1] : upr) + CH_DG, u = up[j] + CH_HV;
                    int m = a < u ? a : u;
                    m = c < m ? c : m;
                    t[j] = zero ? 0 : m;
                }
#pragma unroll
                for (int j = 0; j < PPL; j++) ring[r][j] = (y + CH2_RING < h && x0 + j < w) ? src[(size_t)(y + CH2_RING) * w + x0 + j] : (uint8_t)0;
#pragma unroll
                for (int j = 1; j < PPL; j++) { int v = t[j - 1] + CH_HV; t[j] = v < t[j] ? v : t[j]; }
                const int sc = ch2_scan_min_up(t[PPL - 1] - step * lane) + step * lane;
                const int carry = ch2_shr1(sc, CH2_INF);
#pragma unroll
                for (int j = 0; j < PPL; j++) {
                    int v = carry + CH_HV * (j + 1);
                    up[j] = v < t[j] ? v : t[j];
                    if (x0 + j < w) tmp[(size_t)y * w + x0 + j] = up[j];
                }
            }
        }
    }
    __threadfence_block();
    {
        int dn[PPL];
#pragma unroll
        for (int j = 0; j < PPL; j++) dn[j] = CH2_INF;
        int ring[CH2_RING][PPL];
#pragma unroll
        for (int r = 0; r < CH2_RING; r++)
#pragma unroll
            for (int j = 0; j < PPL; j++) ring[r][j] = (h - 1 - r >= 0 && x0 + j < w) ? tmp[(size_t)(h - 1 - r) * w + x0 + j] : CH2_INF;
        for (int y0 = 0; y0 < h; y0 += CH2_RING) {
#pragma unroll
            for (int r = 0; r < CH2_RING; r++) {
                const int y = h - 1 - (y0 + r);
                if (y < 0) break;
                const int dnl = ch2_shr1(dn[PPL - 1], CH2_INF), dnr = ch2_shl1(dn[0], CH2_INF);
                int t[PPL];
#pragma unroll
                for (int j = 0; j < PPL; j++) {
                    const int a = (j < PPL - 1 ? dn[j + 1] : dnr) + CH_DG, c = (j > 0 ? dn[j - 1] : dnl) + CH_DG, u = dn[j] + CH_HV;
                    int m = a < u ? a : u;
                    m = c < m ? c : m;
                    const int cur = x0 + j < w ? ring[r][j] : CH2_INF;
                    t[j] = m < cur ? m : cur;
                }
#pragma unroll
                for (int j = 0; j < PPL; j++) ring[r][j] = (y - CH2_RING >= 0 && x0 + j < w) ? tmp[(size_t)(y - CH2_RING) * w + x0 + j] : CH2_INF;
#pragma unroll
                for (int j = PPL - 2; j >= 0; j--) { int v = t[j + 1] + CH_HV; t[j] = v < t[j] ? v : t[j]; }
                const int ml = 63 - lane;
                int first = t[0] - step * ml;
                first = __builtin_amdgcn_ds_bpermute(ml << 2, first);
                first = ch2_scan_min_up(first);
                first = __builtin_amdgcn_ds_bpermute(ml << 2, first) + step * ml;
                const int carry = ch2_shl1(first, CH2_INF);
#pragma unroll
                for (int j = 0; j < PPL; j++) {
                    int v = carry + CH_HV * (PPL - j);
                    dn[j] = v < t[j] ? v : t[j];
                    if (x0 + j < w) {
                        int o = dn[j] > CH2_INF ? CH2_INF : dn[j];
                        dist[(size_t)y * w + x0 + j] = (float)o * (1.0f / 65536.0f);
                    }
                }
            }
        }
    }
}

constexpr uint16_t CHL_NONE = 0xffffu;
__global__ __launch_bounds__(1024) void k_chamfer_lds(const uint8_t *__restrict__ src_all, int invert, float *__restrict__ dist_all, int h, int w,
                                                      int cap)
{
    extern __shared__ uint16_t chl_g[];
    const int tid = threadIdx.x, lane = tid & 63, wid = tid >> 6;
    const size_t b = blockIdx.x;
    const int P = h * w;
    const uint8_t *src = src_all + b * (size_t)P;
    constexpr int CHL_W = 8;
    const int nwords = (w + 63) >> 6;
    for (int y = wid; y < h; y += 16) {
        const uint8_t *row = src + (size_t)y * w;
        uint8_t px[CHL_W];
#pragma unroll
        for (int c = 0; c < CHL_W; c++) { const int x = c * 64 + lane; px[c] = (c < nwords && x < w) ? row[x] : (uint8_t)(invert ? 0 : 1); }
        unsigned long long Z[CHL_W];
#pragma unroll
        for (int c = 0; c < CHL_W; c++) {
            const int x = c * 64 + lane;
            Z[c] = __ballot(c < nwords && x < w && (invert ? px[c] != 0 : px[c] == 0));
        }
#pragma unroll
        for (int c = 0; c < CHL_W; c++) {
            if (c >= nwords) break;
            const int x = c * 64 + lane;
            int dl = 0x7fff0000;
            {
                const unsigned long long zl = Z[c] & ((2ull << lane) - 1ull);
                if (zl) dl = lane - (63 - __clzll((long long)zl));
                else {
#pragma unroll
                    for (int k = 1; k < CHL_W; k++) {
                        if (c - k < 0) break;
                        if (Z[c - k]) { dl = lane + 64 * k - (63 - __clzll((long long)Z[c - k])); break; }
                    }
                }
            }
            int dr = 0x7fff0000;
            {
                const unsigned long long zr = Z[c] >> lane;
                if (zr) dr = __ffsll((long long)zr) - 1;
                else {
#pragma unroll
                    for (int k = 1; k < CHL_W; k++) {
                        if (c + k >= nwords) break;
                        if (Z[c + k]) { dr = 64 * k - lane + (__ffsll((long long)Z[c + k]) - 1); break; }
                    }
                }
            }
            const int d = dl < dr ? dl : dr;
            if (x < w) chl_g[y * w + x] = d > 0xfffe ? CHL_NONE : (uint16_t)d;
        }
    }
    __syncthreads();
    float *dist = dist_all + b * (size_t)P;
    for (int p = tid; p < P; p += 1024) {
        const int y = p / w, x = p - y * w;
        int best = CH_DIST_MAX;
        for (int dy = 0; dy <= cap; dy++) {
            if ((long long)dy * CH_HV >= best) break;
#pragma unroll
            for (int s = 0; s < 2; s++) {
                if (s && !dy) break;
                const int yy = s ? y + dy : y - dy;
                if (yy < 0 || yy >= h) continue;
                const int gx = (int)chl_g[yy * w + x];
                if (gx == (int)CHL_NONE) continue;
                const int mn = gx < dy ? gx : dy, mx = gx < dy ? dy : gx;
                const int c = CH_HV * (mx - mn) + CH_DG * mn;
                if (c < best) best = c;
            }
        }
        dist[p] = (float)best * (1.0f / 65536.0f);
    }
}

void launch_chamfer(const uint8_t *src, bool invert, int32_t *rowdist, float *dist, int B, int h, int w, int cap_px, hipStream_t st, bool force_twopass)
{
    int cap = (int)((cap_px + 2) / 0.955) + 2;
    if (cap > h) cap = h;
    if (!force_twopass && cap <= 16 && (size_t)h * w * 2 <= 150 * 1024 && w <= 512) {
        static DynLdsOnce lds_once;
        ensure_dyn_lds(lds_once, (const void *)k_chamfer_lds, 160 * 1024);
        hipLaunchKernelGGL(k_chamfer_lds, dim3(B), dim3(1024), (size_t)h * w * 2, st, src, invert ? 1 : 0, dist, h, w, cap);
        return;
    }
    (void)cap_px;
    if (w <= 256) { hipLaunchKernelGGL(k_chamfer2<4>, dim3(B), dim3(64), 0, st, src, invert ? 1 : 0, rowdist, dist, nullptr, nullptr, B, h, w); return; }
    if (w <= 512) { hipLaunchKernelGGL(k_chamfer2<8>, dim3(B), dim3(64), 0, st, src, invert ? 1 : 0, rowdist, dist, nullptr, nullptr, B, h, w); return; }
    int rows = B * h;
    hipLaunchKernelGGL(k_rowdist, dim3((rows + 3) / 4), dim3(256), 0, st, src, invert ? 1 : 0, rowdist, h, w, B);
    hipLaunchKernelGGL(k_chamfer_cols, dim3((w + 255) / 256, h, B), dim3(256), 0, st, rowdist, dist, h, w, cap);
}

void launch_chamfer_pair(const uint8_t *src, int32_t *tmp_a, float *dist_a, int32_t *tmp_b, float *dist_b, int B, int h, int w, int cap_px,
                         hipStream_t st, bool force_twopass)
{
    int cap = (int)((cap_px + 2) / 0.955) + 2;
    if (cap > h) cap = h;
    const bool two_pass = (force_twopass || cap > 16 || (size_t)h * w * 2 > 150 * 1024) && (w <= 512 || (w <= 1280 && cap > 64 && (B >= 16 || force_twopass)));
    if (!two_pass) {
        launch_chamfer(src, false, tmp_a, dist_a, B, h, w, cap_px, st, false);
        launch_chamfer(src, true, tmp_b, dist_b, B, h, w, cap_px, st, false);
        return;
    }
    if (w <= 256) hipLaunchKernelGGL(k_chamfer2<4>, dim3(2 * B), dim3(64), 0, st, src, 0, tmp_a, dist_a, tmp_b, dist_b, B, h, w);
    else if (w <= 512) hipLaunchKernelGGL(k_chamfer2<8>, dim3(2 * B), dim3(64), 0, st, src, 0, tmp_a, dist_a, tmp_b, dist_b, B, h, w);
    else hipLaunchKernelGGL(k_chamfer2<20>, dim3(2 * B), dim3(64), 0, st, src, 0, tmp_a, dist_a, tmp_b, dist_b, B, h, w);
}

__global__ void k_erode_by_dist(const float *__restrict__ dist, const uint8_t *__restrict__ src, float margin, uint8_t *__restrict__ out, size_t n)
{
    size_t i = (size_t)blockIdx.x * blockDim.x + threadIdx.x;
    if (i >= n) return;
    out[i] = (uint8_t)(src[i] && dist[i] > margin);
}
void launch_erode_by_dist(const float *dist, const uint8_t *src, float margin, uint8_t *out, int B, int P, hipStream_t st)
{
    size_t n = (size_t)B * P;
    hipLaunchKernelGGL(k_erode_by_dist, dim3((unsigned)((n + 255) / 256)), dim3(256), 0, st, dist, src, margin, out, n);
}

}
```

### vistaf-roboskin-vision-integrated-multimodal-sensor_amd/csrc/k_post.hip

```cpp
#include "kernels.hpp"
#include "pixel_ops.hpp"

namespace vf {

__global__ void k_contact_count(const float *__restrict__ res, const uint8_t *__restrict__ reliable, const float *__restrict__ thr3,
                                int *__restrict__ counts, int P)
{
    __shared__ int scratch[16];
    size_t b = blockIdx.y;
    float thr = thr3[b * 3];
    if (!finitef(thr)) thr = thr3[b * 3 + 1];
    int c = 0;
    for (int p = blockIdx.x * blockDim.x + threadIdx.x; p < P; p += gridDim.x * blockDim.x) {
        float v = fabsf(res[b * (size_t)P + p]);
        c += (reliable[b * (size_t)P + p] && finitef(v) && v >= thr);
    }
    c = block_sum<int>(c, scratch);
    if (threadIdx.x == 0 && c) atomicAdd(&counts[b], c);
}

__global__ void k_contact_mask(const float *__restrict__ res, const uint8_t *__restrict__ reliable, const float *__restrict__ thr3,
                               const int *__restrict__ contact_count, const int *__restrict__ rel_count, double min_frac, double max_frac,
                               uint8_t *__restrict__ contact, float *__restrict__ thr_used, int P)
{
    int p = blockIdx.x * blockDim.x + threadIdx.x;
    size_t b = blockIdx.y;
    float thr = thr3[b * 3];
    if (!finitef(thr)) thr = thr3[b * 3 + 1];
    int rc = rel_count[b];
    double frac = (double)contact_count[b] / (double)(rc > 1 ? rc : 1);
    if (frac < min_frac) { float t2 = thr3[b * 3 + 1]; if (finitef(t2)) thr = t2; }
    else if (frac > max_frac) { float t2 = thr3[b * 3 + 2]; if (finitef(t2)) thr = t2; }
    if (p == 0) thr_used[b] = thr;
    if (p >= P) return;
    float v = fabsf(res[b * (size_t)P + p]);
    contact[b * (size_t)P + p] = (uint8_t)(reliable[b * (size_t)P + p] && finitef(v) && v >= thr);
}

void launch_contact_mask(const float *res, const uint8_t *reliable, const float *thr3, const int *rel_count, int *contact_count,
                         double min_frac, double max_frac, uint8_t *contact, float *thr_used, int B, int P, hipStream_t st)
{
    hipMemsetAsync(contact_count, 0, sizeof(int) * B, st);
    int gx = (P + 256 * 16 - 1) / (256 * 16);
    hipLaunchKernelGGL(k_contact_count, dim3(gx, B), dim3(256), 0, st, res, reliable, thr3, contact_count, P);
    hipLaunchKernelGGL(k_contact_mask, dim3((P + 255) / 256, B), dim3(256), 0, st, res, reliable, thr3, contact_count, rel_count, min_frac,
                       max_frac, contact, thr_used, P);
}

__global__ void k_and_not(const uint8_t *__restrict__ a, const uint8_t *__restrict__ b, uint8_t *__restrict__ out, size_t n)
{
    size_t i = (size_t)blockIdx.x * blockDim.x + threadIdx.x;
    if (i < n) out[i] = (uint8_t)(a[i] && !b[i]);
}
__global__ void k_background_fix(const uint8_t *__restrict__ reliable, const int *__restrict__ rel_count, const int *__restrict__ bg_count,
                                 uint8_t *__restrict__ bg, int P)
{
    int p = blockIdx.x * blockDim.x + threadIdx.x;
    size_t b = blockIdx.y;
    if (p >= P) return;
    int limit = (int)(0.15 * (double)rel_count[b]);
    if (bg_count[b] < limit) bg[b * (size_t)P + p] = reliable[b * (size_t)P + p];
}
void launch_background(const uint8_t *reliable, const uint8_t *contact_d, const int *rel_count, int *bg_count, uint8_t *background,
                       int B, int P, hipStream_t st)
{
    size_t n = (size_t)B * P;
    hipLaunchKernelGGL(k_and_not, dim3((unsigned)((n + 255) / 256)), dim3(256), 0, st, reliable, contact_d, background, n);
    launch_count_u8(background, bg_count, B, P, st);
    hipLaunchKernelGGL(k_background_fix, dim3((P + 255) / 256, B), dim3(256), 0, st, reliable, rel_count, bg_count, background, P);
}

__global__ void k_sub_scalar_mask(const float *__restrict__ src, const float *__restrict__ scalar, const uint8_t *__restrict__ mask,
                                  float *__restrict__ z0, float *__restrict__ m_out, int P)
{
    int p = blockIdx.x * blockDim.x + threadIdx.x;
    size_t b = blockIdx.y;
    if (p >= P) return;
    size_t i = b * (size_t)P + p;
    float z, m;
    sub_scalar_mask_px(src[i], scalar[b], mask[i], z, m);
    z0[i] = z;
    m_out[i] = m;
}
void launch_sub_scalar_mask(const float *src, const float *scalar, const uint8_t *mask, float *z0, float *m_out, int B, int P,
                            hipStream_t st)
{
    hipLaunchKernelGGL(k_sub_scalar_mask, dim3((P + 255) / 256, B), dim3(256), 0, st, src, scalar, mask, z0, m_out, P);
}

__global__ void k_div_planes(const float *__restrict__ num, const float *__restrict__ den, float *__restrict__ out, size_t n)
{
    size_t i = (size_t)blockIdx.x * blockDim.x + threadIdx.x;
    if (i < n) out[i] = div_planes_px(num[i], den[i]);
}
void launch_div_planes(const float *num, const float *den, float *out, int B, int P, hipStream_t st)
{
    size_t n = (size_t)B * P;
    hipLaunchKernelGGL(k_div_planes, dim3((unsigned)((n + 255) / 256)), dim3(256), 0, st, num, den, out, n);
}

__global__ void k_core_flip(float *__restrict__ hmap, const float *__restrict__ core_med, int *__restrict__ flipped, int P)
{
    int p = blockIdx.x * blockDim.x + threadIdx.x;
    size_t b = blockIdx.y;
    float m = core_med[b];
    bool flip = finitef(m) && m > 0.f;
    if (p == 0) flipped[b] = flip ? 1 : 0;
    if (p >= P || !flip) return;
    hmap[b * (size_t)P + p] = __fmul_rn(hmap[b * (size_t)P + p], -1.0f);
}
void launch_core_flip(float *hmap, const float *core_med, int *flipped, int B, int P, hipStream_t st)
{
    hipLaunchKernelGGL(k_core_flip, dim3((P + 255) / 256, B), dim3(256), 0, st, hmap, core_med, flipped, P);
}

__global__ void k_frontier_compose(const float *__restrict__ hmap, const uint8_t *__restrict__ reliable, const uint8_t *__restrict__ roi,
                                   const float *__restrict__ dist_in, float band, float *__restrict__ z0, int P)
{
    int p = blockIdx.x * blockDim.x + threadIdx.x;
    size_t b = blockIdx.y;
    if (p >= P) return;
    size_t i = b * (size_t)P + p;
    const bool on = reliable[i] && roi[p];
    z0[i] = frontier_compose_px(on, on ? hmap[i] : 0.f, on ? dist_in[i] : 0.f, band);
}
void launch_frontier_compose(const float *hmap, const uint8_t *reliable, const uint8_t *roi, const float *dist_in, float band,
                             float *hfinal_z0, int B, int P, hipStream_t st)
{
    hipLaunchKernelGGL(k_frontier_compose, dim3((P + 255) / 256, B), dim3(256), 0, st, hmap, reliable, roi, dist_in, band, hfinal_z0, P);
}

__global__ void k_finalize_unitless(const float *__restrict__ z0, const float *__restrict__ smooth_num, const float *__restrict__ roi_den,
                                    const uint8_t *__restrict__ reliable, const uint8_t *__restrict__ roi, const float *__restrict__ dist_out,
                                    float band, int use_band, float *__restrict__ unitless, int P)
{
    int p = blockIdx.x * blockDim.x + threadIdx.x;
    size_t b = blockIdx.y;
    if (p >= P) return;
    size_t i = b * (size_t)P + p;
    const bool in_roi = roi[p] != 0, rel = in_roi && reliable[i] != 0, unrel = in_roi && !rel;
    const bool have_smooth = smooth_num != nullptr;
    unitless[i] = finalize_unitless_px(in_roi, rel, in_roi ? z0[i] : 0.f, have_smooth, unrel && have_smooth ? smooth_num[i] : 0.f,
                                       unrel && have_smooth ? roi_den[p] : 1.f, use_band != 0, unrel && use_band ? dist_out[i] : 0.f, band);
}
void launch_finalize_unitless(const float *hfinal_z0, const float *smooth_num, const float *roi_den, const uint8_t *reliable,
                              const uint8_t *roi, const float *dist_out, float band, int use_band, float *unitless, int B, int P,
                              hipStream_t st)
{
    hipLaunchKernelGGL(k_finalize_unitless, dim3((P + 255) / 256, B), dim3(256), 0, st, hfinal_z0, smooth_num, roi_den, reliable, roi,
                       dist_out, band, use_band, unitless, P);
}

__global__ void k_to_mm(const float *__restrict__ unitless, const uint8_t *__restrict__ roi, Curve curve, int use_neg,
                        float *__restrict__ depth, uint8_t *__restrict__ cand, unsigned int *__restrict__ gmax_bits, int P)
{
    __shared__ unsigned long long scratch[16];
    size_t b = blockIdx.y;
    unsigned int mx = 0;
    for (int p = blockIdx.x * blockDim.x + threadIdx.x; p < P; p += gridDim.x * blockDim.x) {
        size_t i = b * (size_t)P + p;
        float d;
        bool c = to_mm_px(unitless[i], roi[p] != 0, curve, use_neg, d);
        depth[i] = d;
        cand[i] = (uint8_t)c;
        if (c) { unsigned int u = __float_as_uint(d); if (u > mx) mx = u; }
    }
    unsigned long long m = block_max_u64(mx, scratch);
    if (threadIdx.x == 0 && m) atomicMax(&gmax_bits[b], (unsigned int)m);
}
void launch_to_mm(const float *unitless, const uint8_t *roi, Curve curve, int use_neg, float *depth, uint8_t *cand,
                  unsigned int *gmax_bits, int B, int P, hipStream_t st)
{
    hipMemsetAsync(gmax_bits, 0, sizeof(unsigned int) * B, st);
    int gx = (P + 256 * 8 - 1) / (256 * 8);
    hipLaunchKernelGGL(k_to_mm, dim3(gx, B), dim3(256), 0, st, unitless, roi, curve, use_neg, depth, cand, gmax_bits, P);
}

__global__ void k_blob_peaks(const float *__restrict__ depth, const int32_t *__restrict__ labels, unsigned int *__restrict__ peak_bits, int P)
{
    size_t b = blockIdx.y;
    int lane = threadIdx.x & 63;
    int Pr = ((P + 255) / 256) * 256;
    for (int p = blockIdx.x * blockDim.x + threadIdx.x; p < Pr; p += gridDim.x * blockDim.x) {
        int root = p < P ? labels[b * (size_t)P + p] : -1;
        unsigned int v = root >= 0 ? __float_as_uint(depth[b * (size_t)P + p]) : 0u;
        unsigned long long active = __ballot(root >= 0);
        while (active) {
            int leader = __ffsll((long long)active) - 1;
            int r0 = __shfl(root, leader, 64);
            bool same = root == r0;
            unsigned int m = wave_max_u32(same ? v : 0u);
            if (lane == leader) atomicMax(&peak_bits[b * (size_t)P + r0], m);
            active &= ~__ballot(same);
        }
    }
}
__global__ void k_blob_apply(float *__restrict__ depth, const uint8_t *__restrict__ cand, const int32_t *__restrict__ labels,
                             const unsigned int *__restrict__ peak_bits, const unsigned int *__restrict__ gmax_bits, double min_peak_mm,
                             double rel_frac, uint8_t *__restrict__ kept, int P)
{
    int p = blockIdx.x * blockDim.x + threadIdx.x;
    size_t b = blockIdx.y;
    if (p >= P) return;
    size_t i = b * (size_t)P + p;
    bool k = false;
    if (cand[i]) {
        double gmax = (double)__uint_as_float(gmax_bits[b]);
        double thr = min_peak_mm;
        if (rel_frac >= 0.0) thr = fmax(thr, rel_frac * gmax);
        float peak = __uint_as_float(peak_bits[b * (size_t)P + labels[i]]);
        k = peak >= (float)thr;
        if (!k) depth[i] = 0.f;
    }
    if (kept) kept[i] = (uint8_t)k;
}
void launch_blob_filter(float *depth, const uint8_t *cand, const int32_t *labels, unsigned int *peak_bits,
                        const unsigned int *gmax_bits, double min_peak_mm, double rel_frac, uint8_t *kept, int B, int P,
                        hipStream_t st)
{
    hipMemsetAsync(peak_bits, 0, sizeof(unsigned int) * (size_t)B * P, st);
    int gx = (P + 256 * 8 - 1) / (256 * 8);
    hipLaunchKernelGGL(k_blob_peaks, dim3(gx, B), dim3(256), 0, st, depth, labels, peak_bits, P);
    hipLaunchKernelGGL(k_blob_apply, dim3((P + 255) / 256, B), dim3(256), 0, st, depth, cand, labels, peak_bits, gmax_bits, min_peak_mm,
                       rel_frac, kept, P);
}

__global__ __launch_bounds__(1024) void k_tail(const float *__restrict__ height_mm, const uint8_t *__restrict__ roi_frame,
                                               const float *__restrict__ unitless, const uint8_t *__restrict__ roi_static, PostParams pp,
                                               double *__restrict__ scalars, int nscal, double *__restrict__ out3, int P)
{
    __shared__ double sd[16];
    __shared__ unsigned long long s64[16];
    size_t b = blockIdx.x;
    const float *H = height_mm + b * (size_t)P;
    const uint8_t *R = roi_frame ? roi_frame + b * (size_t)P : nullptr;
    const float *U = unitless ? unitless + b * (size_t)P : nullptr;
    const bool want_arg = scalars != nullptr;
    const float eps = (float)pp.depth_eps_mm;
    double sp = 0, sn = 0, volp = 0, voln = 0;
    int cntp = 0, cntn = 0;
    unsigned long long mxp = 0, mxn = 0, am = 0, an = ~0ull;
    constexpr int TU = 4;
    const int T = blockDim.x;
    for (int p0 = threadIdx.x; p0 < P; p0 += TU * T) {
        float v[TU], u[TU];
        uint8_t rf[TU], rs[TU];
#pragma unroll
        for (int k = 0; k < TU; k++) {
            const int p = p0 + k * T;
            const bool inb = p < P;
            v[k] = inb ? H[p] : nanf32();
            rf[k] = (inb && R) ? R[p] : (uint8_t)0;
            rs[k] = (inb && want_arg) ? roi_static[p] : (uint8_t)0;
            u[k] = (inb && U) ? U[p] : nanf32();
        }
#pragma unroll
        for (int k = 0; k < TU; k++) {
            const int p = p0 + k * T;
            if (p >= P) break;
            const float vv = v[k];
            if (vv == vv) { if (vv > 0.f) sp += vv; else sn += -vv; }
            const bool in = R ? rf[k] != 0 : finitef(vv);
            float dp = fmaxf(vv, 0.f), dn = fmaxf(-vv, 0.f);
            if (!in || !finitef(dp)) dp = 0.f;
            if (!in || !finitef(dn)) dn = 0.f;
            if (dp > eps) { volp += dp; cntp++; const unsigned long long key = (unsigned long long)__float_as_uint(dp) << 32; if (key > mxp) mxp = key; }
            if (dn > eps) { voln += dn; cntn++; const unsigned long long key = (unsigned long long)__float_as_uint(dn) << 32; if (key > mxn) mxn = key; }
            if (rs[k] && finitef(vv)) {
                const unsigned long long key = ((unsigned long long)f2key(vv) << 32) | (unsigned int)(0xffffffffu - (unsigned int)p);
                if (key > am) am = key;
            }
            if (rs[k] && finitef(u[k])) {
                const unsigned long long key = ((unsigned long long)f2key(u[k]) << 32) | (unsigned int)p;
                if (key < an) an = key;
            }
        }
    }
    sp = block_sum<double>(sp, sd);
    sn = block_sum<double>(sn, sd);
    const bool use_neg = (float)sn > (float)sp;
    double vol = block_sum<double>(use_neg ? voln : volp, sd);
    double cntd = block_sum<double>((double)(use_neg ? cntn : cntp), sd);
    unsigned long long mx = block_max_u64(use_neg ? mxn : mxp, s64);
    double period_px = pp.period_px, mm_per_px = pp.mm_per_px;
    if (pp.pair_geom) { period_px = pp.pair_geom[b].period; mm_per_px = period_px > 1e-12 ? pp.grating_pitch_mm / period_px : 0.0; }
    double area_px = mm_per_px * mm_per_px;
    double volume_cm3 = cntd > 0 ? (double)(float)vol * area_px / 1000.0 : 0.0;
    double area_mm2 = cntd * area_px;
    double maxd = cntd > 0 ? (double)__uint_as_float((unsigned int)(mx >> 32)) : 0.0;
    if (out3 && threadIdx.x == 0) { out3[b * 3] = volume_cm3; out3[b * 3 + 1] = area_mm2; out3[b * 3 + 2] = maxd; }
    if (!scalars) return;
    am = block_max_u64(am, s64);
    if (unitless) an = block_min_u64(an, s64);
    if (threadIdx.x == 0) {
        double *S = scalars + b * (size_t)nscal;
        S[0] = volume_cm3; S[1] = area_mm2; S[2] = maxd;
        S[3] = curve_eval(pp.force_curve, volume_cm3);
        S[4] = am ? (double)(0xffffffffu - (unsigned int)(am & 0xffffffffu)) : -1.0;
        S[5] = period_px; S[6] = mm_per_px;
        if (unitless && an != ~0ull) { S[7] = (double)key2f((unsigned int)(an >> 32)); S[8] = (double)(unsigned int)(an & 0xffffffffu); }
        else { S[7] = (double)nanf32(); S[8] = -1.0; }
    }
}
constexpr int TP_T = 256, TP_PX = 16, TP_WORDS = 10;
__global__ __launch_bounds__(TP_T) void k_tail_part(const float *__restrict__ height_mm, const uint8_t *__restrict__ roi_frame,
                                                    const float *__restrict__ unitless, const uint8_t *__restrict__ roi_static, float eps, int want_arg,
                                                    unsigned long long *__restrict__ part, int P)
{
    __shared__ double sd[16];
    __shared__ unsigned long long s64[16];
    const size_t b = blockIdx.y;
    const float *H = height_mm + b * (size_t)P;
    const uint8_t *R = roi_frame ? roi_frame + b * (size_t)P : nullptr;
    const float *U = unitless ? unitless + b * (size_t)P : nullptr;
    double sp = 0, sn = 0, volp = 0, voln = 0;
    unsigned long long cntp = 0, cntn = 0, mxp = 0, mxn = 0, am = 0, an = ~0ull;
    const int p0 = blockIdx.x * TP_T * TP_PX + threadIdx.x;
#pragma unroll 4
    for (int k = 0; k < TP_PX; k++) {
        const int p = p0 + k * TP_T;
        if (p >= P) break;
        const float vv = H[p];
        const uint8_t rf = R ? R[p] : (uint8_t)0, rs = want_arg ? roi_static[p] : (uint8_t)0;
        const float uu = U ? U[p] : nanf32();
        if (vv == vv) { if (vv > 0.f) sp += vv; else sn += -vv; }
        const bool in = R ? rf != 0 : finitef(vv);
        float dp = fmaxf(vv, 0.f), dn = fmaxf(-vv, 0.f);
        if (!in || !finitef(dp)) dp = 0.f;
        if (!in || !finitef(dn)) dn = 0.f;
        if (dp > eps) { volp += dp; cntp++; const unsigned long long key = (unsigned long long)__float_as_uint(dp) << 32; if (key > mxp) mxp = key; }
        if (dn > eps) { voln += dn; cntn++; const unsigned long long key = (unsigned long long)__float_as_uint(dn) << 32; if (key > mxn) mxn = key; }
        if (rs && finitef(vv)) {
            const unsigned long long key = ((unsigned long long)f2key(vv) << 32) | (unsigned int)(0xffffffffu - (unsigned int)p);
            if (key > am) am = key;
        }
        if (rs && finitef(uu)) {
            const unsigned long long key = ((unsigned long long)f2key(uu) << 32) | (unsigned int)p;
            if (key < an) an = key;
        }
    }
    sp = block_sum<double>(sp, sd); sn = block_sum<double>(sn, sd);
    volp = block_sum<double>(volp, sd); voln = block_sum<double>(voln, sd);
    cntp = block_sum<unsigned long long>(cntp, s64); cntn = block_sum<unsigned long long>(cntn, s64);
    mxp = block_max_u64(mxp, s64); mxn = block_max_u64(mxn, s64);
    am = block_max_u64(am, s64); an = block_min_u64(an, s64);
    if (threadIdx.x == 0) {
        unsigned long long *o = part + (b * gridDim.x + blockIdx.x) * TP_WORDS;
        o[0] = (unsigned long long)__double_as_longlong(sp); o[1] = (unsigned long long)__double_as_longlong(sn);
        o[2] = (unsigned long long)__double_as_longlong(volp); o[3] = (unsigned long long)__double_as_longlong(voln);
        o[4] = cntp; o[5] = cntn; o[6] = mxp; o[7] = mxn; o[8] = am; o[9] = an;
    }
}
__global__ __launch_bounds__(TP_T) void k_tail_final(const unsigned long long *__restrict__ part, int nblk, int has_unitless, PostParams pp,
                                                     double *__restrict__ scalars, int nscal, double *__restrict__ out3)
{
    __shared__ double sd[16];
    __shared__ unsigned long long s64[16];
    const size_t b = blockIdx.x;
    double sp = 0, sn = 0, volp = 0, voln = 0;
    unsigned long long cntp = 0, cntn = 0, mxp = 0, mxn = 0, am = 0, an = ~0ull;
    for (int k = threadIdx.x; k < nblk; k += TP_T) {
        const unsigned long long *o = part + (b * nblk + k) * TP_WORDS;
        sp += __longlong_as_double((long long)o[0]); sn += __longlong_as_double((long long)o[1]);
        volp += __longlong_as_double((long long)o[2]); voln += __longlong_as_double((long long)o[3]);
        cntp += o[4]; cntn += o[5];
        mxp = o[6] > mxp ? o[6] : mxp; mxn = o[7] > mxn ? o[7] : mxn; am = o[8] > am ? o[8] : am; an = o[9] < an ? o[9] : an;
    }
    sp = block_sum<double>(sp, sd);
    sn = block_sum<double>(sn, sd);
    const bool use_neg = (float)sn > (float)sp;
    const double vol = block_sum<double>(use_neg ? voln : volp, sd);
    const double cntd = (double)block_sum<unsigned long long>(use_neg ? cntn : cntp, s64);
    const unsigned long long mx = block_max_u64(use_neg ? mxn : mxp, s64);
    double period_px = pp.period_px, mm_per_px = pp.mm_per_px;
    if (pp.pair_geom) { period_px = pp.pair_geom[b].period; mm_per_px = period_px > 1e-12 ? pp.grating_pitch_mm / period_px : 0.0; }
    const double area_px = mm_per_px * mm_per_px;
    const double volume_cm3 = cntd > 0 ? (double)(float)vol * area_px / 1000.0 : 0.0;
    const double area_mm2 = cntd * area_px;
    const double maxd = cntd > 0 ? (double)__uint_as_float((unsigned int)(mx >> 32)) : 0.0;
    if (out3 && threadIdx.x == 0) { out3[b * 3] = volume_cm3; out3[b * 3 + 1] = area_mm2; out3[b * 3 + 2] = maxd; }
    if (!scalars) return;
    am = block_max_u64(am, s64);
    an = block_min_u64(an, s64);
    if (threadIdx.x == 0) {
        double *S = scalars + b * (size_t)nscal;
        S[0] = volume_cm3; S[1] = area_mm2; S[2] = maxd;
        S[3] = curve_eval(pp.force_curve, volume_cm3);
        S[4] = am ? (double)(0xffffffffu - (unsigned int)(am & 0xffffffffu)) : -1.0;
        S[5] = period_px; S[6] = mm_per_px;
        if (has_unitless && an != ~0ull) { S[7] = (double)key2f((unsigned int)(an >> 32)); S[8] = (double)(unsigned int)(an & 0xffffffffu); }
        else { S[7] = (double)nanf32(); S[8] = -1.0; }
    }
}

void launch_tail(const float *height_mm, const uint8_t *roi_or_null, const float *unitless_or_null, const uint8_t *roi_static,
                 PostParams pp, double *scalars, int nscal, double *out3_or_null, int B, int P, hipStream_t st, void *scratch, size_t scratch_bytes)
{
    const int nblk = (P + TP_T * TP_PX - 1) / (TP_T * TP_PX);
    if (scratch && P >= 262144 && B <= 192 && (size_t)B * nblk * TP_WORDS * 8 <= scratch_bytes) {
        unsigned long long *part = (unsigned long long *)scratch;
        hipLaunchKernelGGL(k_tail_part, dim3(nblk, B), dim3(TP_T), 0, st, height_mm, roi_or_null, unitless_or_null, roi_static, (float)pp.depth_eps_mm,
                           scalars != nullptr ? 1 : 0, part, P);
        hipLaunchKernelGGL(k_tail_final, dim3(B), dim3(TP_T), 0, st, part, nblk, unitless_or_null != nullptr ? 1 : 0, pp, scalars, nscal, out3_or_null);
        return;
    }
    hipLaunchKernelGGL(k_tail, dim3(B), dim3(1024), 0, st, height_mm, roi_or_null, unitless_or_null, roi_static, pp, scalars, nscal,
                       out3_or_null, P);
}

__global__ void k_fill_scalars(double *__restrict__ scalars, int nscal, const int *__restrict__ rel_count, const int *__restrict__ flipped,
                               const float *__restrict__ amp_thr, const float *__restrict__ contact_thr, const float *__restrict__ bg_med,
                               const int *__restrict__ bad_count, int B)
{
    int b = blockIdx.x * blockDim.x + threadIdx.x;
    if (b >= B) return;
    double *S = scalars + (size_t)b * nscal;
    S[9] = rel_count ? (double)rel_count[b] : 0.0;
    S[10] = flipped ? (double)flipped[b] : 0.0;
    S[11] = amp_thr ? (double)amp_thr[b] : 0.0;
    S[12] = contact_thr ? (double)contact_thr[b] : 0.0;
    S[13] = bg_med ? (double)bg_med[b] : 0.0;
    S[14] = bad_count ? (double)bad_count[b] : 0.0;
    S[15] = 0.0;
}
void launch_fill_scalars(double *scalars, int nscal, const int *rel_count, const int *flipped, const float *amp_thr,
                         const float *contact_thr, const float *bg_med, const int *bad_count, int B, hipStream_t st)
{
    hipLaunchKernelGGL(k_fill_scalars, dim3((B + 63) / 64), dim3(64), 0, st, scalars, nscal, rel_count, flipped, amp_thr, contact_thr, bg_med,
                       bad_count, B);
}

__global__ void k_mark_empty(const int *__restrict__ rel_count, int32_t *__restrict__ status, int B)
{
    int b = blockIdx.x * blockDim.x + threadIdx.x;
    if (b < B && rel_count[b] == 0 && status[b] == 0) status[b] = 1;
}
void launch_mark_empty(const int *rel_count, int32_t *status, int B, hipStream_t st)
{
    hipLaunchKernelGGL(k_mark_empty, dim3((B + 63) / 64), dim3(64), 0, st, rel_count, status, B);
}

__global__ void k_copy_out(const float *__restrict__ depth, const uint8_t *__restrict__ reliable, const int32_t *__restrict__ status,
                           float *__restrict__ out_h, uint8_t *__restrict__ out_r, int P)
{
    int p = blockIdx.x * blockDim.x + threadIdx.x;
    size_t b = blockIdx.y;
    if (p >= P) return;
    size_t i = b * (size_t)P + p;
    bool empty = status[b] == 1 || status[b] == 3;
    if (out_h) out_h[i] = empty ? nanf32() : depth[i];
    if (out_r) out_r[i] = empty ? 0 : reliable[i];
}
void launch_copy_out(const float *depth, const uint8_t *reliable, const int32_t *status, float *out_h, uint8_t *out_r, int B, int P,
                     hipStream_t st)
{
    hipLaunchKernelGGL(k_copy_out, dim3((P + 255) / 256, B), dim3(256), 0, st, depth, reliable, status, out_h, out_r, P);
}

}
```

### vistaf-roboskin-vision-integrated-multimodal-sensor_amd/csrc/kernels.hpp

```cpp
#pragma once
#include <hip/hip_runtime.h>
#include <stdint.h>
#include "common.hpp"

namespace vf {

struct Tiers {
    int inpaint = 2;
    int big_flood_handback = 0;
    int chamfer_twopass = 0;
    int telea_two_tier = 1;
    int unwrap_fast = 1;
    int big_chain = 1;
    int big_queue_lds = 1;
    int big_gq_cap = 0;
    int big_fallback = 1;
    int telea_mw = 1;
    int fused_chains = 1;
};

struct RowSpanSE {
    int k;
    int8_t lo[33];
    int8_t hi[33];
};

void launch_to_gray(const void *frames, int format, float *gray, int B, int P, hipStream_t st);
void launch_sobel_mag(const float *img, float *grad, int B, int h, int w, hipStream_t st);
void launch_bad_flags(const float *img, const float *grad, const uint8_t *valid, const float *thr_hi, const float *thr_g,
                      uint8_t *bad, int B, int P, hipStream_t st);
void launch_morph(const uint8_t *src, uint8_t *dst, int B, int h, int w, const RowSpanSE &se, bool dilate,
                  const uint8_t *and_static, const uint8_t *and_frame, hipStream_t st, uint16_t *prefix_scratch = nullptr);
void launch_morph_seq(const uint8_t *src, uint8_t *dst, uint8_t *tmp, int B, int h, int w, const RowSpanSE &se, const int *dilates, int n,
                      const uint8_t *and_static, const uint8_t *and_frame, hipStream_t st, uint16_t *prefix_scratch = nullptr);
void launch_gauss_rows(const float *src, float *dst, const float *kern, int ksize, int B, int h, int w, hipStream_t st);
void launch_gauss_blur(const float *src, float *tmp, float *dst, const float *kern, int ksize, int B, int h, int w, hipStream_t st);
void launch_gauss_cols(const float *src, float *dst, const float *kern, int ksize, int B, int h, int w, hipStream_t st);
void launch_illum_norm(const float *img, const float *blur, float *out, int B, int P, hipStream_t st);
void launch_mul_static(const float *a, const float *stat, float *out, int B, int P, hipStream_t st);
void launch_count_u8(const uint8_t *m, int *counts, int B, int P, hipStream_t st);

constexpr int GF_MAXK = 15;

void launch_illum_pre_apod(const float *img, const float *blur_illum, const float *apo, float *iw, const float *kern, int ksize, int B, int h,
                           int w, hipStream_t st);
void launch_smooth_reliable(const float *detr, const float *bg_med, const uint8_t *reliable, float *hmap, const float *kern, int ksize, int B,
                            int h, int w, hipStream_t st);
void launch_compose_finalize_mm(const float *hmap, const uint8_t *reliable, const uint8_t *roi, const float *dist_in, float taper_band,
                                const float *roi_den, const float *dist_out, float band, int use_band, Curve curve, int use_neg, float *unitless,
                                float *depth, uint8_t *cand, unsigned int *gmax_bits, const float *kern, int ksize, int B, int h, int w,
                                hipStream_t st);

void launch_select(const float *vals, const uint8_t *mask, size_t mask_stride, const float *le_thr, bool use_abs,
                   const float *reqs_dev, int nreq, float *out, int *counts, int B, int P, hipStream_t st, void *big_scratch = nullptr);

struct CarrierGeom {
    double peak_x, peak_y;
    double kx, ky;
    double dpx, dpy;
    double period;
    int x0, y0, ph, pw;
    int px_i, py_i;
    int px_raw, py_raw;
    int ok;
    int keep_carrier;
};
void launch_dft_forward(const float *iw, const float *mu, const double2 *Ex, const double2 *Ey, size_t tab_stride_x, size_t tab_stride_y,
                        const float *win, double2 *tmpT, double2 *patch, int patch_stride, int B, int h, int w, int ph, int pw, hipStream_t st,
                        int win_stride = 0);
void launch_dft_inverse(const double2 *patch, int patch_stride, const double2 *Gx, const double2 *Gy, size_t tab_stride_x, size_t tab_stride_y,
                        double2 *tmpQ, double2 *field, float *amp, const double2 *cref, const float *amp_ref, size_t ref_stride, float *prod,
                        float *wrapped, int B, int h, int w, int ph, int pw, hipStream_t st, const CarrierGeom *geom = nullptr);
void launch_dft_full_mag(const float *iw, const float *mu, const double2 *Ex_full, const double2 *Ey_full, double2 *tmp,
                         double *mag, int B, int h, int w, int Hf, int Wf, hipStream_t st);
void launch_top_peaks(const double *mag, int B, int Hf, int Wf, int dc, int npeaks, double *out_xyv , hipStream_t st);
void launch_carrier_choose(const double *peaks, int npk, const double *mag, int Hf, int Wf, int bw, double max_dy_frac, CarrierGeom *geom, int B,
                           hipStream_t st);
void launch_build_tables(const CarrierGeom *geom, int geom_stride, double2 *Ex, double2 *Ey, double2 *Gx, double2 *Gy, size_t stride_x,
                         size_t stride_y, int B, int h, int w, int pad, int Hf, int Wf, int pmax, hipStream_t st, const float *pair_hann = nullptr,
                         float *pair_win = nullptr);
void launch_pair_status(const CarrierGeom *geom, int pmax, int32_t *status, const int32_t *status2, int B, hipStream_t st);
void launch_build_full_tables(double2 *Exf, double2 *Eyf, int h, int w, int pad, int Hf, int Wf, hipStream_t st);

void launch_threshold_mask(const float *q, const uint8_t *roi, const float *thr, uint8_t *out, int B, int P, hipStream_t st);
void launch_cc_label(const uint8_t *mask, int32_t *labels, int B, int h, int w, hipStream_t st);
void launch_cc_largest(const int32_t *labels, int32_t *area_scratch, unsigned long long *best, const uint8_t *and_static,
                       uint8_t *out, int B, int P, hipStream_t st);
void launch_chamfer(const uint8_t *src, bool invert, int32_t *rowdist, float *dist, int B, int h, int w, int cap_px, hipStream_t st,
                    bool force_twopass = false);
void launch_chamfer_pair(const uint8_t *src, int32_t *tmp_a, float *dist_a, int32_t *tmp_b, float *dist_b, int B, int h, int w, int cap_px,
                         hipStream_t st, bool force_twopass = false);
void launch_erode_by_dist(const float *dist, const uint8_t *src, float margin, uint8_t *out, int B, int P, hipStream_t st);

size_t inpaint_scratch_bytes_per_frame(int h, int w);
void launch_inpaint_telea(float *img, const uint8_t *bad, int range, void *scratch, int32_t *status, const int32_t *only, int B, int h, int w,
                          hipStream_t st, bool round_u8 = false);

size_t inpaint_win_scratch_bytes(int B);
bool inpaint_window_mw_supported(int range);
void launch_telea_window_mw(float *img, const uint8_t *bad, const int32_t *box, int32_t *fb, int range, int B, int h, int w, hipStream_t st);
int32_t *launch_inpaint_window(float *img, const uint8_t *bad, int range, void *scratch, int B, int h, int w, hipStream_t st,
                               hipEvent_t ev_march = nullptr, bool two_tier = true, bool mw = true);

size_t inpaint_cl_scratch_bytes_per_frame(int h, int w);
bool inpaint_clusters_supported(int range);
struct ClusterPlanes { const int32_t *labels, *list, *count, *xmin, *ymin, *xmax, *ymax; const uint8_t *dil; };
size_t inpaint_big_scratch_bytes_per_frame(int h, int w);
bool inpaint_big_supported(int range);
void launch_inpaint_big_clusters(float *img, const uint8_t *bad_big, int range, void *scratch, int32_t *status, const ClusterPlanes &left, int B, int h,
                                 int w, hipStream_t st, bool lds_queue = true, int gq_cap = 0);
void launch_inpaint_big_handback(int32_t *status, int32_t *only, int B, hipStream_t st);
void launch_inpaint_clusters(float *img, const uint8_t *bad, int range, void *scratch, uint8_t **bad_big_out, ClusterPlanes *left, int B, int h, int w,
                             hipStream_t st);

size_t unwrap_scratch_bytes_per_frame(int h, int w);
void launch_unwrap(const float *wrapped, const float *quality, const uint8_t *mask, float *unwrapped, int32_t *parent,
                   void *scratch, int32_t *status, int B, int h, int w, hipStream_t st, hipEvent_t ev_mid,
                   hipEvent_t ev_flood = nullptr, bool big_handback = false, int32_t *need_buf = nullptr);

void launch_robust_polyfit(const float *z, const uint8_t *mask, int order, int iters, float c, int min_count, int min_mask_count, float *coef_out,
                           float *resid_out, int B, int h, int w, hipStream_t st, void *big_scratch = nullptr);
enum FitVariant { FITV_BIG = 0, FITV_GENERIC, FITV_GENERIC_DIV, FITV_COL16, FITV_COL32, FITV_COL48, FITV_COL56, FITV_COL64, FITV_COL48_G4, FITV_COL56_G4,
                  FITV_COL64_G4, FITV_COUNT };
int polyfit_variant(int B, int h, int w, bool big, int *cols_pad_out = nullptr, int *groups_out = nullptr);

void launch_zeroed_keep_nan(const float *detr, const float *bg_med, const uint8_t *reliable, float *hmap, int B, int P, hipStream_t st);
void launch_hole_candidates(const float *hmap, const uint8_t *reliable, const float *dist, int ksize, float frac_thr, float min_dist, uint8_t *cand,
                            int B, int h, int w, hipStream_t st);
void launch_hole_tmp(const float *hmap, const uint8_t *reliable, const uint8_t *cand, const float *med, float *tmp, int B, int P, hipStream_t st);
void launch_hole_zin(float *tmp_zin, const float *fill, int B, int P, hipStream_t st);
void launch_hole_merge(float *hmap, const uint8_t *reliable, const uint8_t *cand, const float *zin, uint8_t *out_rel, int B, int P, hipStream_t st);

constexpr int LAB_SHIFT = 12, LAB_SHIFT2 = 15, LAB_GAMMA_SHIFT = 3, LAB_CBRT_N = 256 * 3 / 2 * (1 << LAB_GAMMA_SHIFT);
struct LabCoef { int c[9]; int lscale, lshift; };
void launch_feature_planes(const uint8_t *bgr, const uint16_t *gamma_tab, const uint16_t *cbrt_tab, const LabCoef &cf, bool blur, float *L, float *a,
                           float *b, float *gray, int H, int W, hipStream_t st);
void launch_color_support(const float *a, const float *b, const uint8_t *light_d, const uint8_t *roi_eff, const uint8_t *sat, float chroma_min,
                          float *chroma, uint8_t *support, size_t n, hipStream_t st);

struct PostParams {
    double mm_per_px, depth_eps_mm, period_px;
    Curve force_curve;
    const CarrierGeom *pair_geom = nullptr;
    double grating_pitch_mm = 0.0;
};
void launch_contact_mask(const float *res, const uint8_t *reliable, const float *thr3, const int *rel_count, int *contact_count,
                         double min_frac, double max_frac, uint8_t *contact, float *thr_used, int B, int P, hipStream_t st);
void launch_background(const uint8_t *reliable, const uint8_t *contact_d, const int *rel_count, int *bg_count, uint8_t *background,
                       int B, int P, hipStream_t st);
void launch_sub_scalar_mask(const float *src, const float *scalar, const uint8_t *mask, float *z0, float *m_out, int B, int P,
                            hipStream_t st);
void launch_div_planes(const float *num, const float *den, float *out, int B, int P, hipStream_t st);
void launch_core_flip(float *hmap, const float *core_med, int *flipped, int B, int P, hipStream_t st);
void launch_frontier_compose(const float *hmap, const uint8_t *reliable, const uint8_t *roi, const float *dist_in, float band,
                             float *hfinal_z0, int B, int P, hipStream_t st);
void launch_finalize_unitless(const float *hfinal_z0, const float *smooth_num, const float *roi_den, const uint8_t *reliable,
                              const uint8_t *roi, const float *dist_out, float band, int use_band, float *unitless, int B, int P,
                              hipStream_t st);
void launch_to_mm(const float *unitless, const uint8_t *roi, Curve curve, int use_neg, float *depth, uint8_t *cand,
                  unsigned int *gmax_bits, int B, int P, hipStream_t st);
void launch_blob_filter(float *depth, const uint8_t *cand, const int32_t *labels, unsigned int *peak_bits,
                        const unsigned int *gmax_bits, double min_peak_mm, double rel_frac, uint8_t *kept, int B, int P,
                        hipStream_t st);
void launch_tail(const float *height_mm, const uint8_t *roi_or_null, const float *unitless_or_null, const uint8_t *roi_static,
                 PostParams pp, double *scalars, int nscal, double *out3_or_null, int B, int P, hipStream_t st, void *scratch = nullptr,
                 size_t scratch_bytes = 0);
void launch_fill_scalars(double *scalars, int nscal, const int *rel_count, const int *flipped, const float *amp_thr,
                         const float *contact_thr, const float *bg_med, const int *bad_count, int B, hipStream_t st);
void launch_mark_empty(const int *rel_count, int32_t *status, int B, hipStream_t st);
void launch_copy_out(const float *depth, const uint8_t *reliable, const int32_t *status, float *out_h, uint8_t *out_r, int B, int P,
                     hipStream_t st);

struct ContactScratch {
    int32_t *arg;
    int32_t *list; int cap;
    int *nroots, *nsel;
    unsigned long long *selkey;
    unsigned long long *part;
};
int contact_root_capacity(int h, int w);
size_t contact_part_words(int max_batch, int P);
void launch_contacts(const float *depth, const uint8_t *kept, const int32_t *labels, const unsigned int *peak_bits, const int32_t *status,
                     PostParams pp, const ContactScratch &cs, int K, double *contacts, int nfield, int32_t *count, int8_t *index, int B, int h, int w,
                     hipStream_t st);

size_t big_scratch_bytes(int B, int h, int w);
bool big_frames(int B, int P);
void launch_select_big(const float *vals, const uint8_t *mask, size_t mask_stride, const float *le_thr, bool use_abs, const float *reqs_dev, int nreq,
                       float *out, int *counts, int B, int P, void *scratch, hipStream_t st);
void launch_robust_polyfit_big(const float *z, const uint8_t *mask, int order, int iters, float c, int min_count, int min_mask_count, float *coef_out,
                               float *resid_out, int B, int h, int w, void *scratch, hipStream_t st);

struct TmAff { double m[6]; };
struct TmFuse { float color_lo, color_hi, low_th, high_th, final_lo, final_hi; };
void launch_tm_clamp(const float *m, const uint8_t *roi, float lo, float hi, float *out, size_t P, hipStream_t st);
void launch_tm_stats(const float *m, const uint8_t *roi, uint32_t *stats, size_t P, hipStream_t st);
void launch_tm_scale(const float *m, const uint8_t *roi, const uint32_t *stats, float *scaled, uint8_t *miss, size_t P, hipStream_t st);
void launch_tm_unscale(const float *m, const uint8_t *roi, const uint32_t *stats, const float *filled, float *out, size_t P, hipStream_t st);
void launch_tm_fuse(const uint8_t *roi, const float *wide, const float *color, const TmFuse &c, float *fin, uint8_t *source, unsigned long long *counts, size_t P,
                    hipStream_t st);
void launch_tm_zero_nonfinite(const float *m, float *out, size_t P, hipStream_t st);
void launch_tm_warp_linear(const float *src, float *dst, const TmAff &a, int h, int w, hipStream_t st);
void launch_tm_warp_nearest(const uint8_t *src, uint8_t *dst, const TmAff &a, int h, int w, hipStream_t st);
void launch_tm_mask_nan(const float *m, const uint8_t *keep, float *out, size_t P, hipStream_t st);

size_t tstats_scratch_bytes(int h, int w);
bool tstats_needs_big_scratch(int h, int w);
void launch_tstats(const float *map, const uint8_t *valid, int h, int w, void *scratch, void *big_scratch, double *out, hipStream_t st);

}
```

Measured before the change: 67350 frames/s.

## Fuse connected-component labeling, blob filter, tail reduction and copy-out into one kernel

Adds a per-frame fused backend kernel that builds a union-find forest for connected-component labeling in LDS with 16-bit labels, computes blob peaks, applies the keep threshold, runs the tail reduction and writes the output. It replaces the separate cc_label, blob_filter, tail and copy_out launches. The aim is to cut kernel launches and global-memory round trips of the labels, depth and mask planes at 224x224. The chamfer two-pass kernel also gets vectorized row loads and stores. The cost is one block per frame with large LDS use, which limits parallelism, and labels are capped at 16 bits.

```diff
diff --git a/vistaf-roboskin-vision-integrated-multimodal-sensor_amd/_lib.py b/vistaf-roboskin-vision-integrated-multimodal-sensor_amd/_lib.py
--- a/vistaf-roboskin-vision-integrated-multimodal-sensor_amd/_lib.py
+++ b/vistaf-roboskin-vision-integrated-multimodal-sensor_amd/_lib.py
@@ -23,7 +23,8 @@
     "vistaf_ftp_enable_stage_timing", "vistaf_ftp_get_stage_times", "vistaf_ftp_destroy",
     "vistaf_depth_map_to_volume", "vistaf_predict_force_from_volume",
 ]
-TEST_EXPORTS = ["vistaf_ftp_test_set", "vistaf_ftp_test_select", "vistaf_ftp_test_polyfit", "vistaf_ftp_test_gauss"]
+TEST_EXPORTS = ["vistaf_ftp_test_set", "vistaf_ftp_test_select", "vistaf_ftp_test_polyfit", "vistaf_ftp_test_gauss",
+                "vistaf_ftp_test_chamfer"]
 TEMP_EXPORTS = ["vistaf_tempseg_default_config", "vistaf_tempseg_create", "vistaf_tempseg_destroy", "vistaf_tempseg_segment",
                 "vistaf_temp_feature_planes", "vistaf_temp_color_support",
                 "vistaf_temp_clamp_map", "vistaf_temp_inpaint_map", "vistaf_temp_fuse_maps", "vistaf_temp_oriented_blur"]
@@ -116,6 +117,7 @@
     lib.vistaf_ftp_test_select.argtypes = [vp, vp, ctypes.c_size_t, vp, ci, vp, ci, vp, vp, ci, ci, ci, vp]
     lib.vistaf_ftp_test_polyfit.argtypes = [vp, vp, ci, ci, ctypes.c_float, ci, ci, vp, vp, ci, ci, ci, ci, vp]
     lib.vistaf_ftp_test_gauss.argtypes = [vp, vp, cd, ci, ci, ci, vp]
+    lib.vistaf_ftp_test_chamfer.argtypes = [vp, ci, ci, vp, vp, ci, ci, ci, ci, vp]
     lib.vistaf_tempseg_default_config.argtypes = [ctypes.POINTER(CTempSegConfig)]
     lib.vistaf_tempseg_create.argtypes = [ctypes.POINTER(CTempSegConfig), ci, ci, ctypes.POINTER(vp)]
     lib.vistaf_tempseg_destroy.argtypes = [vp]
diff --git a/vistaf-roboskin-vision-integrated-multimodal-sensor_amd/csrc/api.hip b/vistaf-roboskin-vision-integrated-multimodal-sensor_amd/csrc/api.hip
--- a/vistaf-roboskin-vision-integrated-multimodal-sensor_amd/csrc/api.hip
+++ b/vistaf-roboskin-vision-integrated-multimodal-sensor_amd/csrc/api.hip
@@ -647,18 +647,26 @@
 
     if (timed) hipEventRecord(hd->ev[ST_MM_BLOB], st);
     if (!fuse_compose) launch_to_mm(hd->unitless, hd->roi, hd->hcurve, hd->use_neg, hd->depth, hd->cand, hd->gmax, B, P, st);
-    launch_cc_label(hd->cand, hd->labels, B, h, w, st);
-    launch_blob_filter(hd->depth, hd->cand, hd->labels, hd->peak_bits, hd->gmax, c.contact_blob_min_peak_mm,
-                       c.contact_blob_min_peak_rel_frac, hd->kept, B, P, st);
-
-    if (timed) hipEventRecord(hd->ev[ST_TAIL], st);
     PostParams pp;
     pp.mm_per_px = hd->mm_per_px; pp.depth_eps_mm = c.depth_eps_mm; pp.period_px = hd->period; pp.force_curve = hd->fcurve;
     pp.pair_geom = pair_geom; pp.grating_pitch_mm = c.grating_pitch_mm;
-    launch_tail(hd->depth, nullptr, hd->unitless, hd->roi, pp, hd->scalars, VISTAF_NSCALARS, nullptr, B, P, st, hd->tiers.big_chain ? hd->big_scratch : nullptr,
-                hd->big_scratch ? big_scratch_bytes(hd->maxB, h, w) : 0);
+    const bool fused_backend = hd->tiers.fused_backend && backend_fused_fits(h, w);
+    if (fused_backend)
+        launch_backend_fused(hd->depth, hd->cand, hd->gmax, hd->unitless, hd->roi, orel, hd->status, c.contact_blob_min_peak_mm,
+                             c.contact_blob_min_peak_rel_frac, pp, hd->labels, hd->peak_bits, hd->kept, hd->scalars, VISTAF_NSCALARS, d_height_mm,
+                             d_reliable, B, h, w, st);
+    else {
+        launch_cc_label(hd->cand, hd->labels, B, h, w, st);
+        launch_blob_filter(hd->depth, hd->cand, hd->labels, hd->peak_bits, hd->gmax, c.contact_blob_min_peak_mm,
+                           c.contact_blob_min_peak_rel_frac, hd->kept, B, P, st);
+    }
+
+    if (timed) hipEventRecord(hd->ev[ST_TAIL], st);
+    if (!fused_backend)
+        launch_tail(hd->depth, nullptr, hd->unitless, hd->roi, pp, hd->scalars, VISTAF_NSCALARS, nullptr, B, P, st, hd->tiers.big_chain ? hd->big_scratch : nullptr,
+                    hd->big_scratch ? big_scratch_bytes(hd->maxB, h, w) : 0);
     launch_fill_scalars(hd->scalars, VISTAF_NSCALARS, hd->rel_count, hd->flipped, hd->amp_thr, hd->thr_used, hd->bg_med, bad_count, B, st);
-    launch_copy_out(hd->depth, orel, hd->status, d_height_mm, d_reliable, B, P, st);
+    if (!fused_backend) launch_copy_out(hd->depth, orel, hd->status, d_height_mm, d_reliable, B, P, st);
     if (d_scalars) HIPCHK(hipMemcpyAsync(d_scalars, hd->scalars, sizeof(double) * VISTAF_NSCALARS * B, hipMemcpyDeviceToDevice, st));
     if (d_status) HIPCHK(hipMemcpyAsync(d_status, hd->status, sizeof(int32_t) * B, hipMemcpyDeviceToDevice, st));
     if (timed) {
@@ -823,6 +831,7 @@
     else if (n == "unwrap_fast") hd->tiers.unwrap_fast = value != 0;
     else if (n == "big_chain") hd->tiers.big_chain = value != 0;
     else if (n == "fused_chains") hd->tiers.fused_chains = value != 0;
+    else if (n == "fused_backend") hd->tiers.fused_backend = value != 0;
     else if (n == "keep_planes") hd->keep_planes = value != 0;
     else return fail(VISTAF_E_INVALID, "unknown test hook or value: " + n);
     return 0;
@@ -892,6 +901,20 @@
     return hook_finish(taps, tmp, (hipStream_t)stream);
 }
 
+int vistaf_ftp_test_chamfer(const uint8_t *mask, int pair, int invert, float *dist_a, float *dist_b, int B, int h, int w, int cap_px, void *stream)
+{
+    if (!mask || !dist_a || (pair && !dist_b) || B < 1 || h < 1 || w < 1 || (size_t)h * w > 0x7fffffffull || cap_px < 0)
+        return fail(VISTAF_E_INVALID, "bad argument");
+    if (w > 512 && !(pair && w <= 1280)) return fail(VISTAF_E_INVALID, "no two-pass instance for this width");
+    const size_t n = (size_t)B * h * w;
+    int32_t *tmp_a = nullptr, *tmp_b = nullptr;
+    HIPCHK(hipMalloc((void **)&tmp_a, n * sizeof(int32_t)));
+    if (pair && hipMalloc((void **)&tmp_b, n * sizeof(int32_t)) != hipSuccess) { (void)hipFree(tmp_a); return fail(VISTAF_E_HIP, "hipMalloc"); }
+    if (pair) launch_chamfer_pair(mask, tmp_a, dist_a, tmp_b, dist_b, B, h, w, cap_px, (hipStream_t)stream, true);
+    else launch_chamfer(mask, invert != 0, tmp_a, dist_a, B, h, w, cap_px, (hipStream_t)stream, true);
+    return hook_finish(tmp_a, tmp_b, (hipStream_t)stream);
+}
+
 int vistaf_depth_map_to_volume(const float *d_height, const uint8_t *d_roi, int batch, int h, int w, double mm_per_px,
                                double depth_eps_mm, double *d_out, void *stream)
 {
diff --git a/vistaf-roboskin-vision-integrated-multimodal-sensor_amd/csrc/backend_device.hpp b/vistaf-roboskin-vision-integrated-multimodal-sensor_amd/csrc/backend_device.hpp
--- /dev/null
+++ b/vistaf-roboskin-vision-integrated-multimodal-sensor_amd/csrc/backend_device.hpp
@@ -0,0 +1,179 @@
+#pragma once
+#include "kernels.hpp"
+#include "pixel_ops.hpp"
+
+namespace vf {
+
+__device__ inline uint32_t cc16_min(uint16_t *L, int i, uint32_t val)
+{
+    uint32_t *wp = (uint32_t *)L + (i >> 1);
+    const int sh = (i & 1) * 16;
+    uint32_t old = *(volatile uint32_t *)wp;
+    for (;;) {
+        uint32_t cur = (old >> sh) & 0xffffu;
+        if (cur <= val) return cur;
+        uint32_t nw = (old & ~(0xffffu << sh)) | (val << sh);
+        uint32_t prev = atomicCAS(wp, old, nw);
+        if (prev == old) return cur;
+        old = prev;
+    }
+}
+__device__ inline int cc16_find(uint16_t *L, int i)
+{
+    volatile uint16_t *V = L;
+    for (;;) {
+        int p = V[i];
+        if (p == i) return i;
+        int g = V[p];
+        if (g == p) return p;
+        V[i] = (uint16_t)g;
+        i = g;
+    }
+}
+__device__ inline void cc16_unite(uint16_t *L, int a, int b)
+{
+    for (;;) {
+        a = cc16_find(L, a);
+        b = cc16_find(L, b);
+        if (a == b) return;
+        if (a > b) { int t = a; a = b; b = t; }
+        uint32_t old = cc16_min(L, b, (uint32_t)a);
+        if ((int)old == b) return;
+        b = (int)old;
+    }
+}
+__host__ __device__ inline size_t cc_lds_forest_bytes(int P) { return (size_t)((P + 2 + 7) & ~7) * 2; }
+__host__ __device__ inline size_t cc_lds_bytes(int P) { return cc_lds_forest_bytes(P) + (size_t)P + 16; }
+template <bool MLDS>
+__device__ inline const uint8_t *cc_lds_build(const uint8_t *__restrict__ mg, int h, int w, uint16_t *L16)
+{
+    const int P = h * w;
+    uint8_t *ml = (uint8_t *)(L16 + ((P + 2 + 7) & ~7));
+    if (MLDS) {
+        for (int p = threadIdx.x * 4; p < P; p += blockDim.x * 4) {
+            if (p + 3 < P && ((((uintptr_t)mg) & 3) == 0)) *(uint32_t *)(ml + p) = *(const uint32_t *)(mg + p);
+            else for (int k = 0; k < 4 && p + k < P; k++) ml[p + k] = mg[p + k];
+        }
+        __syncthreads();
+    }
+    const uint8_t *m = MLDS ? (const uint8_t *)ml : mg;
+    {
+        const int lane = threadIdx.x & 63, wid = threadIdx.x >> 6, nwv = blockDim.x >> 6;
+        for (int y = wid; y < h; y += nwv) {
+            int carry = -1;
+            for (int x0 = 0; x0 < w; x0 += 64) {
+                const int x = x0 + lane;
+                const bool on = x < w && m[y * w + x];
+                int lz = (x < w && !on) ? x : (int)0x80000000;
+                int t;
+                t = __builtin_amdgcn_update_dpp((int)0x80000000, lz, 0x111, 0xf, 0xf, false); lz = t > lz ? t : lz;
+                t = __builtin_amdgcn_update_dpp((int)0x80000000, lz, 0x112, 0xf, 0xf, false); lz = t > lz ? t : lz;
+                t = __builtin_amdgcn_update_dpp((int)0x80000000, lz, 0x114, 0xf, 0xf, false); lz = t > lz ? t : lz;
+                t = __builtin_amdgcn_update_dpp((int)0x80000000, lz, 0x118, 0xf, 0xf, false); lz = t > lz ? t : lz;
+                t = __builtin_amdgcn_update_dpp((int)0x80000000, lz, 0x142, 0xa, 0xf, false); lz = t > lz ? t : lz;
+                t = __builtin_amdgcn_update_dpp((int)0x80000000, lz, 0x143, 0xc, 0xf, false); lz = t > lz ? t : lz;
+                lz = lz > carry ? lz : carry;
+                carry = __builtin_amdgcn_readlane(lz, 63);
+                if (x < w) L16[y * w + x] = on ? (uint16_t)(y * w + lz + 1) : (uint16_t)0xffffu;
+            }
+        }
+    }
+    if ((P & 1) && threadIdx.x == 0) L16[P] = 0xffffu;
+    __syncthreads();
+    for (int p = threadIdx.x; p < P; p += blockDim.x) {
+        if (!m[p]) continue;
+        const int y = p / w, x = p - y * w;
+        if (y == 0) continue;
+        const bool left = x > 0 && m[p - 1];
+        const bool ul = x > 0 && m[p - w - 1], up = m[p - w] != 0, ur = x < w - 1 && m[p - w + 1];
+        if ((ul || up) && !left) cc16_unite(L16, p, ul ? p - w - 1 : p - w);
+        if (ur && !up) cc16_unite(L16, p, p - w + 1);
+    }
+    __syncthreads();
+    return m;
+}
+
+__device__ inline float blob_keep_threshold(unsigned int gmax_bits, double min_peak_mm, double rel_frac)
+{
+    double gmax = (double)__uint_as_float(gmax_bits);
+    double thr = min_peak_mm;
+    if (rel_frac >= 0.0) thr = fmax(thr, rel_frac * gmax);
+    return (float)thr;
+}
+
+constexpr int TAIL_STATIC_LDS = 16 * 8 * 2;
+template <typename HeightFn>
+__device__ inline void tail_frame(HeightFn height, const uint8_t *__restrict__ R, const float *__restrict__ U, const uint8_t *__restrict__ roi_static,
+                                  const PostParams &pp, double *__restrict__ scalars, int nscal, double *__restrict__ out3, int b, int P)
+{
+    __shared__ double sd[16];
+    __shared__ unsigned long long s64[16];
+    const bool want_arg = scalars != nullptr;
+    const float eps = (float)pp.depth_eps_mm;
+    double sp = 0, sn = 0, volp = 0, voln = 0;
+    int cntp = 0, cntn = 0;
+    unsigned long long mxp = 0, mxn = 0, am = 0, an = ~0ull;
+    constexpr int TU = 4;
+    const int T = blockDim.x;
+    for (int p0 = threadIdx.x; p0 < P; p0 += TU * T) {
+        float v[TU], u[TU];
+        uint8_t rf[TU], rs[TU];
+#pragma unroll
+        for (int k = 0; k < TU; k++) {
+            const int p = p0 + k * T;
+            const bool inb = p < P;
+            v[k] = inb ? height(p) : nanf32();
+            rf[k] = (inb && R) ? R[p] : (uint8_t)0;
+            rs[k] = (inb && want_arg) ? roi_static[p] : (uint8_t)0;
+            u[k] = (inb && U) ? U[p] : nanf32();
+        }
+#pragma unroll
+        for (int k = 0; k < TU; k++) {
+            const int p = p0 + k * T;
+            if (p >= P) break;
+            const float vv = v[k];
+            if (vv == vv) { if (vv > 0.f) sp += vv; else sn += -vv; }
+            const bool in = R ? rf[k] != 0 : finitef(vv);
+            float dp = fmaxf(vv, 0.f), dn = fmaxf(-vv, 0.f);
+            if (!in || !finitef(dp)) dp = 0.f;
+            if (!in || !finitef(dn)) dn = 0.f;
+            if (dp > eps) { volp += dp; cntp++; const unsigned long long key = (unsigned long long)__float_as_uint(dp) << 32; if (key > mxp) mxp = key; }
+            if (dn > eps) { voln += dn; cntn++; const unsigned long long key = (unsigned long long)__float_as_uint(dn) << 32; if (key > mxn) mxn = key; }
+            if (rs[k] && finitef(vv)) {
+                const unsigned long long key = ((unsigned long long)f2key(vv) << 32) | (unsigned int)(0xffffffffu - (unsigned int)p);
+                if (key > am) am = key;
+            }
+            if (rs[k] && finitef(u[k])) {
+                const unsigned long long key = ((unsigned long long)f2key(u[k]) << 32) | (unsigned int)p;
+                if (key < an) an = key;
+            }
+        }
+    }
+    sp = block_sum<double>(sp, sd);
+    sn = block_sum<double>(sn, sd);
+    const bool use_neg = (float)sn > (float)sp;
+    double vol = block_sum<double>(use_neg ? voln : volp, sd);
+    double cntd = block_sum<double>((double)(use_neg ? cntn : cntp), sd);
+    unsigned long long mx = block_max_u64(use_neg ? mxn : mxp, s64);
+    double period_px = pp.period_px, mm_per_px = pp.mm_per_px;
+    if (pp.pair_geom) { period_px = pp.pair_geom[b].period; mm_per_px = period_px > 1e-12 ? pp.grating_pitch_mm / period_px : 0.0; }
+    double area_px = mm_per_px * mm_per_px;
+    double volume_cm3 = cntd > 0 ? (double)(float)vol * area_px / 1000.0 : 0.0;
+    double area_mm2 = cntd * area_px;
+    double maxd = cntd > 0 ? (double)__uint_as_float((unsigned int)(mx >> 32)) : 0.0;
+    if (out3 && threadIdx.x == 0) { out3[b * 3] = volume_cm3; out3[b * 3 + 1] = area_mm2; out3[b * 3 + 2] = maxd; }
+    if (!scalars) return;
+    am = block_max_u64(am, s64);
+    if (U) an = block_min_u64(an, s64);
+    if (threadIdx.x == 0) {
+        double *S = scalars + b * (size_t)nscal;
+        S[0] = volume_cm3; S[1] = area_mm2; S[2] = maxd;
+        S[3] = curve_eval(pp.force_curve, volume_cm3);
+        S[4] = am ? (double)(0xffffffffu - (unsigned int)(am & 0xffffffffu)) : -1.0;
+        S[5] = period_px; S[6] = mm_per_px;
+        if (U && an != ~0ull) { S[7] = (double)key2f((unsigned int)(an >> 32)); S[8] = (double)(unsigned int)(an & 0xffffffffu); }
+        else { S[7] = (double)nanf32(); S[8] = -1.0; }
+    }
+}
+
+}
diff --git a/vistaf-roboskin-vision-integrated-multimodal-sensor_amd/csrc/k_backend.hip b/vistaf-roboskin-vision-integrated-multimodal-sensor_amd/csrc/k_backend.hip
--- /dev/null
+++ b/vistaf-roboskin-vision-integrated-multimodal-sensor_amd/csrc/k_backend.hip
@@ -0,0 +1,103 @@
+#include "kernels.hpp"
+#include "backend_device.hpp"
+
+namespace vf {
+
+__global__ __launch_bounds__(1024) void k_backend_fused(float *__restrict__ depth, const uint8_t *__restrict__ cand, const unsigned int *__restrict__ gmax_bits,
+                                                        const float *__restrict__ unitless, const uint8_t *__restrict__ roi_static,
+                                                        const uint8_t *__restrict__ reliable, const int32_t *__restrict__ status, double min_peak_mm,
+                                                        double rel_frac, PostParams pp, int32_t *__restrict__ labels, unsigned int *__restrict__ peak_bits,
+                                                        uint8_t *__restrict__ kept, double *__restrict__ scalars, int nscal, float *__restrict__ out_h,
+                                                        uint8_t *__restrict__ out_r, int h, int w)
+{
+    extern __shared__ __attribute__((aligned(16))) uint16_t L16[];
+    const size_t b = blockIdx.x;
+    const int P = h * w;
+    const size_t off = b * (size_t)P;
+    const int lane = threadIdx.x & 63;
+
+    const uint8_t *m = cc_lds_build<true>(cand + off, h, w, L16);
+    unsigned int *PB = peak_bits + off;
+    for (int p = threadIdx.x; p < P; p += blockDim.x) {
+        int r = -1;
+        if (m[p]) {
+            r = p;
+            for (int q = ((volatile uint16_t *)L16)[r]; q != r; q = ((volatile uint16_t *)L16)[r]) r = q;
+            L16[p] = (uint16_t)r;
+            if (r == p) __hip_atomic_store(&PB[p], 0u, __ATOMIC_RELAXED, __HIP_MEMORY_SCOPE_AGENT);
+        }
+        labels[off + p] = r;
+    }
+    __threadfence_block();
+    __syncthreads();
+
+    float *D = depth + off;
+    {
+        const int Pr = ((P + 63) / 64) * 64;
+        for (int p = threadIdx.x; p < Pr; p += blockDim.x) {
+            const int root = (p < P && m[p]) ? (int)L16[p] : -1;
+            const unsigned int v = root >= 0 ? __float_as_uint(D[p]) : 0u;
+            unsigned long long active = __ballot(root >= 0);
+            while (active) {
+                const int leader = __ffsll((long long)active) - 1;
+                const int r0 = __shfl(root, leader, 64);
+                const bool same = root == r0;
+                const unsigned int mx = wave_max_u32(same ? v : 0u);
+                if (lane == leader) atomicMax(&PB[r0], mx);
+                active &= ~__ballot(same);
+            }
+        }
+    }
+    __threadfence_block();
+    __syncthreads();
+
+    const float thr = blob_keep_threshold(gmax_bits[b], min_peak_mm, rel_frac);
+    {
+        uint8_t *ml = const_cast<uint8_t *>(m);
+        for (int p = threadIdx.x; p < P; p += blockDim.x) {
+            if (!m[p] || (int)L16[p] != p) continue;
+            const float peak = __uint_as_float(__hip_atomic_load(&PB[p], __ATOMIC_RELAXED, __HIP_MEMORY_SCOPE_AGENT));
+            ml[p] = peak >= thr ? (uint8_t)2 : (uint8_t)1;
+        }
+    }
+    __syncthreads();
+
+    const int32_t stat = status[b];
+    const bool empty = stat == 1 || stat == 3;
+    uint8_t *K = kept ? kept + off : nullptr;
+    float *OH = out_h ? out_h + off : nullptr;
+    uint8_t *OR = out_r ? out_r + off : nullptr;
+    const uint8_t *REL = reliable + off;
+    auto height = [&](int p) -> float {
+        float d = D[p];
+        bool k = false;
+        if (m[p]) {
+            k = m[L16[p]] == 2;
+            if (!k) { d = 0.f; D[p] = 0.f; }
+        }
+        if (K) K[p] = (uint8_t)k;
+        if (OH) OH[p] = empty ? nanf32() : d;
+        if (OR) OR[p] = empty ? (uint8_t)0 : REL[p];
+        return d;
+    };
+    tail_frame(height, (const uint8_t *)nullptr, unitless ? unitless + off : nullptr, roi_static, pp, scalars, nscal, (double *)nullptr, (int)b, P);
+}
+
+bool backend_fused_fits(int h, int w)
+{
+    const size_t P = (size_t)h * w;
+    return P <= 65535 && cc_lds_bytes(h * w) + TAIL_STATIC_LDS <= 160 * 1024;
+}
+
+void launch_backend_fused(float *depth, const uint8_t *cand, const unsigned int *gmax_bits, const float *unitless, const uint8_t *roi_static,
+                          const uint8_t *reliable, const int32_t *status, double min_peak_mm, double rel_frac, PostParams pp, int32_t *labels,
+                          unsigned int *peak_bits, uint8_t *kept, double *scalars, int nscal, float *out_h, uint8_t *out_r, int B, int h, int w,
+                          hipStream_t st)
+{
+    static DynLdsOnce lds_once;
+    ensure_dyn_lds(lds_once, (const void *)k_backend_fused, 160 * 1024 - TAIL_STATIC_LDS);
+    hipLaunchKernelGGL(k_backend_fused, dim3(B), dim3(1024), cc_lds_bytes(h * w), st, depth, cand, gmax_bits, unitless, roi_static, reliable, status,
+                       min_peak_mm, rel_frac, pp, labels, peak_bits, kept, scalars, nscal, out_h, out_r, h, w);
+}
+
+}
diff --git a/vistaf-roboskin-vision-integrated-multimodal-sensor_amd/csrc/k_cc_dist.hip b/vistaf-roboskin-vision-integrated-multimodal-sensor_amd/csrc/k_cc_dist.hip
--- a/vistaf-roboskin-vision-integrated-multimodal-sensor_amd/csrc/k_cc_dist.hip
+++ b/vistaf-roboskin-vision-integrated-multimodal-sensor_amd/csrc/k_cc_dist.hip
@@ -1,5 +1,6 @@
 #include <cstdlib>
 #include "kernels.hpp"
+#include "backend_device.hpp"
 
 namespace vf {
 
@@ -85,94 +86,13 @@
     if (mask[b * (size_t)P + p]) { int r = cc_find(L, p); if (r != p) atomicMin(&L[p], r); }
 }
 
-__device__ inline uint32_t cc16_min(uint16_t *L, int i, uint32_t val)
-{
-    uint32_t *wp = (uint32_t *)L + (i >> 1);
-    const int sh = (i & 1) * 16;
-    uint32_t old = *(volatile uint32_t *)wp;
-    for (;;) {
-        uint32_t cur = (old >> sh) & 0xffffu;
-        if (cur <= val) return cur;
-        uint32_t nw = (old & ~(0xffffu << sh)) | (val << sh);
-        uint32_t prev = atomicCAS(wp, old, nw);
-        if (prev == old) return cur;
-        old = prev;
-    }
-}
-__device__ inline int cc16_find(uint16_t *L, int i)
-{
-    volatile uint16_t *V = L;
-    for (;;) {
-        int p = V[i];
-        if (p == i) return i;
-        int g = V[p];
-        if (g == p) return p;
-        V[i] = (uint16_t)g;
-        i = g;
-    }
-}
-__device__ inline void cc16_unite(uint16_t *L, int a, int b)
-{
-    for (;;) {
-        a = cc16_find(L, a);
-        b = cc16_find(L, b);
-        if (a == b) return;
-        if (a > b) { int t = a; a = b; b = t; }
-        uint32_t old = cc16_min(L, b, (uint32_t)a);
-        if ((int)old == b) return;
-        b = (int)old;
-    }
-}
-
 template <bool MLDS>
 __global__ __launch_bounds__(1024) void k_cc_label_lds(const uint8_t *__restrict__ mask, int32_t *__restrict__ labels, int h, int w)
 {
     extern __shared__ __attribute__((aligned(16))) uint16_t L16[];
     size_t b = blockIdx.x;
     int P = h * w;
-    const uint8_t *mg = mask + b * (size_t)P;
-    uint8_t *ml = (uint8_t *)(L16 + ((P + 2 + 7) & ~7));
-    if (MLDS) {
-        for (int p = threadIdx.x * 4; p < P; p += blockDim.x * 4) {
-            if (p + 3 < P && ((((uintptr_t)mg) & 3) == 0)) *(uint32_t *)(ml + p) = *(const uint32_t *)(mg + p);
-            else for (int k = 0; k < 4 && p + k < P; k++) ml[p + k] = mg[p + k];
-        }
-        __syncthreads();
-    }
-    const uint8_t *m = MLDS ? (const uint8_t *)ml : mg;
-    {
-        const int lane = threadIdx.x & 63, wid = threadIdx.x >> 6, nwv = blockDim.x >> 6;
-        for (int y = wid; y < h; y += nwv) {
-            int carry = -1;
-            for (int x0 = 0; x0 < w; x0 += 64) {
-                const int x = x0 + lane;
-                const bool on = x < w && m[y * w + x];
-                int lz = (x < w && !on) ? x : (int)0x80000000;
-                int t;
-                t = __builtin_amdgcn_update_dpp((int)0x80000000, lz, 0x111, 0xf, 0xf, false); lz = t > lz ? t : lz;
-                t = __builtin_amdgcn_update_dpp((int)0x80000000, lz, 0x112, 0xf, 0xf, false); lz = t > lz ? t : lz;
-                t = __builtin_amdgcn_update_dpp((int)0x80000000, lz, 0x114, 0xf, 0xf, false); lz = t > lz ? t : lz;
-                t = __builtin_amdgcn_update_dpp((int)0x80000000, lz, 0x118, 0xf, 0xf, false); lz = t > lz ? t : lz;
-                t = __builtin_amdgcn_update_dpp((int)0x80000000, lz, 0x142, 0xa, 0xf, false); lz = t > lz ? t : lz;
-                t = __builtin_amdgcn_update_dpp((int)0x80000000, lz, 0x143, 0xc, 0xf, false); lz = t > lz ? t : lz;
-                lz = lz > carry ? lz : carry;
-                carry = __builtin_amdgcn_readlane(lz, 63);
-                if (x < w) L16[y * w + x] = on ? (uint16_t)(y * w + lz + 1) : (uint16_t)0xffffu;
-            }
-        }
-    }
-    if ((P & 1) && threadIdx.x == 0) L16[P] = 0xffffu;
-    __syncthreads();
-    for (int p = threadIdx.x; p < P; p += blockDim.x) {
-        if (!m[p]) continue;
-        const int y = p / w, x = p - y * w;
-        if (y == 0) continue;
-        const bool left = x > 0 && m[p - 1];
-        const bool ul = x > 0 && m[p - w - 1], up = m[p - w] != 0, ur = x < w - 1 && m[p - w + 1];
-        if ((ul || up) && !left) cc16_unite(L16, p, ul ? p - w - 1 : p - w);
-        if (ur && !up) cc16_unite(L16, p, p - w + 1);
-    }
-    __syncthreads();
+    const uint8_t *m = cc_lds_build<MLDS>(mask + b * (size_t)P, h, w, L16);
     int32_t *out = labels + b * (size_t)P;
     for (int p = threadIdx.x; p < P; p += blockDim.x) out[p] = m[p] ? cc16_find(L16, p) : -1;
 }
@@ -180,11 +100,11 @@
 void launch_cc_label(const uint8_t *mask, int32_t *labels, int B, int h, int w, hipStream_t st)
 {
     int P = h * w;
-    const size_t forest = (size_t)((P + 2 + 7) & ~7) * 2;
-    if (P <= 65535 && forest + (size_t)P + 16 <= 160 * 1024) {
+    const size_t forest = cc_lds_forest_bytes(P);
+    if (P <= 65535 && cc_lds_bytes(P) <= 160 * 1024) {
         static DynLdsOnce lds_once;
         ensure_dyn_lds(lds_once, (const void *)k_cc_label_lds<true>, 160 * 1024);
-        hipLaunchKernelGGL(k_cc_label_lds<true>, dim3(B), dim3(1024), forest + (size_t)P + 16, st, mask, labels, h, w);
+        hipLaunchKernelGGL(k_cc_label_lds<true>, dim3(B), dim3(1024), cc_lds_bytes(P), st, mask, labels, h, w);
         return;
     }
     if (P <= 65535 && forest <= 150 * 1024) {
@@ -404,7 +324,7 @@
 }
 
 constexpr int CH2_INF = 0x7fffffff >> 2;
-constexpr int CH2_RING = 4;
+__host__ __device__ constexpr int ch2_ring(int ppl) { return ppl == 4 ? 31 : ppl == 8 ? 15 : 6; }
 
 __device__ inline int ch2_shr1(int v, int fill) { return __builtin_amdgcn_update_dpp(fill, v, 0x138, 0xf, 0xf, false); }
 __device__ inline int ch2_shl1(int v, int fill) { return __builtin_amdgcn_update_dpp(fill, v, 0x130, 0xf, 0xf, false); }
@@ -420,12 +340,71 @@
     t = __builtin_amdgcn_update_dpp(big, v, 0x143, 0xc, 0xf, false); v = t < v ? t : v;
     return v;
 }
+template <int PPL>
+__device__ inline void ch2_load_mask(const uint8_t *__restrict__ src, int y, int h, int w, int x0, bool vec, uint32_t (&m)[PPL / 4])
+{
+#pragma unroll
+    for (int q = 0; q < PPL / 4; q++) {
+        const int x = x0 + 4 * q;
+        uint32_t v = 0;
+        if (y < h && x < w) {
+            const uint8_t *s = src + (size_t)y * w + x;
+            if (vec) v = *(const uint32_t *)s;
+            else {
+                v = s[0];
+                if (x + 1 < w) v |= (uint32_t)s[1] << 8;
+                if (x + 2 < w) v |= (uint32_t)s[2] << 16;
+                if (x + 3 < w) v |= (uint32_t)s[3] << 24;
+            }
+        }
+        m[q] = v;
+    }
+}
+template <int PPL>
+__device__ inline void ch2_load_tmp(const int32_t *__restrict__ tmp, int y, int w, int x0, bool vec, int (&v)[PPL])
+{
+#pragma unroll
+    for (int q = 0; q < PPL / 4; q++) {
+        const int x = x0 + 4 * q;
+        int4 t = make_int4(CH2_INF, CH2_INF, CH2_INF, CH2_INF);
+        if (y >= 0 && x < w) {
+            const int32_t *s = tmp + (size_t)y * w + x;
+            if (vec) t = *(const int4 *)s;
+            else {
+                t.x = s[0];
+                if (x + 1 < w) t.y = s[1];
+                if (x + 2 < w) t.z = s[2];
+                if (x + 3 < w) t.w = s[3];
+            }
+        }
+        v[4 * q] = t.x; v[4 * q + 1] = t.y; v[4 * q + 2] = t.z; v[4 * q + 3] = t.w;
+    }
+}
+template <int PPL, typename T, typename T4>
+__device__ inline void ch2_store_row(T *__restrict__ dst, int y, int w, int x0, bool vec, const T (&v)[PPL])
+{
+#pragma unroll
+    for (int q = 0; q < PPL / 4; q++) {
+        const int x = x0 + 4 * q;
+        if (x >= w) continue;
+        T *d = dst + (size_t)y * w + x;
+        if (vec) { T4 t; t.x = v[4 * q]; t.y = v[4 * q + 1]; t.z = v[4 * q + 2]; t.w = v[4 * q + 3]; *(T4 *)d = t; }
+        else {
+            d[0] = v[4 * q];
+            if (x + 1 < w) d[1] = v[4 * q + 1];
+            if (x + 2 < w) d[2] = v[4 * q + 2];
+            if (x + 3 < w) d[3] = v[4 * q + 3];
+        }
+    }
+}
 
 template <int PPL>
 __global__ __launch_bounds__(64) void k_chamfer2(const uint8_t *__restrict__ src_all, int invert, int32_t *__restrict__ tmp_all,
                                                  float *__restrict__ dist_all, int32_t *__restrict__ tmp2_all, float *__restrict__ dist2_all, int B,
                                                  int h, int w)
 {
+    static_assert(PPL % 4 == 0, "columns per lane come in groups of four");
+    constexpr int RING = ch2_ring(PPL);
     const int lane = threadIdx.x;
     size_t b = blockIdx.x;
     if (b >= (size_t)B) { b -= B; invert = !invert; tmp_all = tmp2_all; dist_all = dist2_all; }
@@ -435,19 +414,18 @@
     float *dist = dist_all + b * P;
     const int x0 = lane * PPL;
     const int step = CH_HV * PPL;
+    const bool vec = (w & 3) == 0 && ((uintptr_t)src_all & 3) == 0 && ((uintptr_t)tmp_all & 15) == 0 && ((uintptr_t)dist_all & 15) == 0;
 
     {
         int up[PPL];
 #pragma unroll
         for (int j = 0; j < PPL; j++) up[j] = CH2_INF;
-        uint8_t ring[CH2_RING][PPL];
-#pragma unroll
-        for (int r = 0; r < CH2_RING; r++)
-#pragma unroll
-            for (int j = 0; j < PPL; j++) ring[r][j] = (r < h && x0 + j < w) ? src[(size_t)r * w + x0 + j] : (uint8_t)0;
-        for (int y0 = 0; y0 < h; y0 += CH2_RING) {
-#pragma unroll
-            for (int r = 0; r < CH2_RING; r++) {
+        uint32_t ring[RING][PPL / 4];
+#pragma unroll
+        for (int r = 0; r < RING; r++) ch2_load_mask<PPL>(src, r, h, w, x0, vec, ring[r]);
+        for (int y0 = 0; y0 < h; y0 += RING) {
+#pragma unroll
+            for (int r = 0; r < RING; r++) {
                 const int y = y0 + r;
                 if (y >= h) break;
                 const int upl = ch2_shr1(up[PPL - 1], CH2_INF), upr = ch2_shl1(up[0], CH2_INF);
@@ -455,14 +433,14 @@
 #pragma unroll
                 for (int j = 0; j < PPL; j++) {
                     const bool in = x0 + j < w;
-                    const bool zero = in && (invert ? ring[r][j] != 0 : ring[r][j] == 0);
+                    const uint32_t px = (ring[r][j >> 2] >> (8 * (j & 3))) & 0xffu;
+                    const bool zero = in && (invert ? px != 0 : px == 0);
                     const int a = (j > 0 ? up[j - 1] : upl) + CH_DG, c = (j < PPL - 1 ? up[j + 1] : upr) + CH_DG, u = up[j] + CH_HV;
                     int m = a < u ? a : u;
                     m = c < m ? c : m;
                     t[j] = zero ? 0 : m;
                 }
-#pragma unroll
-                for (int j = 0; j < PPL; j++) ring[r][j] = (y + CH2_RING < h && x0 + j < w) ? src[(size_t)(y + CH2_RING) * w + x0 + j] : (uint8_t)0;
+                ch2_load_mask<PPL>(src, y + RING, h, w, x0, vec, ring[r]);
 #pragma unroll
                 for (int j = 1; j < PPL; j++) { int v = t[j - 1] + CH_HV; t[j] = v < t[j] ? v : t[j]; }
                 const int sc = ch2_scan_min_up(t[PPL - 1] - step * lane) + step * lane;
@@ -471,8 +449,8 @@
                 for (int j = 0; j < PPL; j++) {
                     int v = carry + CH_HV * (j + 1);
                     up[j] = v < t[j] ? v : t[j];
-                    if (x0 + j < w) tmp[(size_t)y * w + x0 + j] = up[j];
                 }
+                ch2_store_row<PPL, int32_t, int4>(tmp, y, w, x0, vec, up);
             }
         }
     }
@@ -481,14 +459,12 @@
         int dn[PPL];
 #pragma unroll
         for (int j = 0; j < PPL; j++) dn[j] = CH2_INF;
-        int ring[CH2_RING][PPL];
-#pragma unroll
-        for (int r = 0; r < CH2_RING; r++)
-#pragma unroll
-            for (int j = 0; j < PPL; j++) ring[r][j] = (h - 1 - r >= 0 && x0 + j < w) ? tmp[(size_t)(h - 1 - r) * w + x0 + j] : CH2_INF;
-        for (int y0 = 0; y0 < h; y0 += CH2_RING) {
-#pragma unroll
-            for (int r = 0; r < CH2_RING; r++) {
+        int ring[RING][PPL];
+#pragma unroll
+        for (int r = 0; r < RING; r++) ch2_load_tmp<PPL>(tmp, h - 1 - r, w, x0, vec, ring[r]);
+        for (int y0 = 0; y0 < h; y0 += RING) {
+#pragma unroll
+            for (int r = 0; r < RING; r++) {
                 const int y = h - 1 - (y0 + r);
                 if (y < 0) break;
                 const int dnl = ch2_shr1(dn[PPL - 1], CH2_INF), dnr = ch2_shl1(dn[0], CH2_INF);
@@ -501,8 +477,7 @@
                     const int cur = x0 + j < w ? ring[r][j] : CH2_INF;
                     t[j] = m < cur ? m : cur;
                 }
-#pragma unroll
-                for (int j = 0; j < PPL; j++) ring[r][j] = (y - CH2_RING >= 0 && x0 + j < w) ? tmp[(size_t)(y - CH2_RING) * w + x0 + j] : CH2_INF;
+                ch2_load_tmp<PPL>(tmp, y - RING, w, x0, vec, ring[r]);
 #pragma unroll
                 for (int j = PPL - 2; j >= 0; j--) { int v = t[j + 1] + CH_HV; t[j] = v < t[j] ? v : t[j]; }
                 const int ml = 63 - lane;
@@ -511,15 +486,14 @@
                 first = ch2_scan_min_up(first);
                 first = __builtin_amdgcn_ds_bpermute(ml << 2, first) + step * ml;
                 const int carry = ch2_shl1(first, CH2_INF);
+                float o[PPL];
 #pragma unroll
                 for (int j = 0; j < PPL; j++) {
                     int v = carry + CH_HV * (PPL - j);
                     dn[j] = v < t[j] ? v : t[j];
-                    if (x0 + j < w) {
-                        int o = dn[j] > CH2_INF ? CH2_INF : dn[j];
-                        dist[(size_t)y * w + x0 + j] = (float)o * (1.0f / 65536.0f);
-                    }
+                    o[j] = (float)(dn[j] > CH2_INF ? CH2_INF : dn[j]) * (1.0f / 65536.0f);
                 }
+                ch2_store_row<PPL, float, float4>(dist, y, w, x0, vec, o);
             }
         }
     }
diff --git a/vistaf-roboskin-vision-integrated-multimodal-sensor_amd/csrc/k_post.hip b/vistaf-roboskin-vision-integrated-multimodal-sensor_amd/csrc/k_post.hip
--- a/vistaf-roboskin-vision-integrated-multimodal-sensor_amd/csrc/k_post.hip
+++ b/vistaf-roboskin-vision-integrated-multimodal-sensor_amd/csrc/k_post.hip
@@ -1,4 +1,5 @@
 #include "kernels.hpp"
+#include "backend_device.hpp"
 #include "pixel_ops.hpp"
 
 namespace vf {
@@ -205,11 +206,8 @@
     size_t i = b * (size_t)P + p;
     bool k = false;
     if (cand[i]) {
-        double gmax = (double)__uint_as_float(gmax_bits[b]);
-        double thr = min_peak_mm;
-        if (rel_frac >= 0.0) thr = fmax(thr, rel_frac * gmax);
         float peak = __uint_as_float(peak_bits[b * (size_t)P + labels[i]]);
-        k = peak >= (float)thr;
+        k = peak >= blob_keep_threshold(gmax_bits[b], min_peak_mm, rel_frac);
         if (!k) depth[i] = 0.f;
     }
     if (kept) kept[i] = (uint8_t)k;
@@ -229,78 +227,10 @@
                                                const float *__restrict__ unitless, const uint8_t *__restrict__ roi_static, PostParams pp,
                                                double *__restrict__ scalars, int nscal, double *__restrict__ out3, int P)
 {
-    __shared__ double sd[16];
-    __shared__ unsigned long long s64[16];
-    size_t b = blockIdx.x;
+    const size_t b = blockIdx.x;
     const float *H = height_mm + b * (size_t)P;
-    const uint8_t *R = roi_frame ? roi_frame + b * (size_t)P : nullptr;
-    const float *U = unitless ? unitless + b * (size_t)P : nullptr;
-    const bool want_arg = scalars != nullptr;
-    const float eps = (float)pp.depth_eps_mm;
-    double sp = 0, sn = 0, volp = 0, voln = 0;
-    int cntp = 0, cntn = 0;
-    unsigned long long mxp = 0, mxn = 0, am = 0, an = ~0ull;
-    constexpr int TU = 4;
-    const int T = blockDim.x;
-    for (int p0 = threadIdx.x; p0 < P; p0 += TU * T) {
-        float v[TU], u[TU];
-        uint8_t rf[TU], rs[TU];
-#pragma unroll
-        for (int k = 0; k < TU; k++) {
-            const int p = p0 + k * T;
-            const bool inb = p < P;
-            v[k] = inb ? H[p] : nanf32();
-            rf[k] = (inb && R) ? R[p] : (uint8_t)0;
-            rs[k] = (inb && want_arg) ? roi_static[p] : (uint8_t)0;
-            u[k] = (inb && U) ? U[p] : nanf32();
-        }
-#pragma unroll
-        for (int k = 0; k < TU; k++) {
-            const int p = p0 + k * T;
-            if (p >= P) break;
-            const float vv = v[k];
-            if (vv == vv) { if (vv > 0.f) sp += vv; else sn += -vv; }
-            const bool in = R ? rf[k] != 0 : finitef(vv);
-            float dp = fmaxf(vv, 0.f), dn = fmaxf(-vv, 0.f);
-            if (!in || !finitef(dp)) dp = 0.f;
-            if (!in || !finitef(dn)) dn = 0.f;
-            if (dp > eps) { volp += dp; cntp++; const unsigned long long key = (unsigned long long)__float_as_uint(dp) << 32; if (key > mxp) mxp = key; }
-            if (dn > eps) { voln += dn; cntn++; const unsigned long long key = (unsigned long long)__float_as_uint(dn) << 32; if (key > mxn) mxn = key; }
-            if (rs[k] && finitef(vv)) {
-                const unsigned long long key = ((unsigned long long)f2key(vv) << 32) | (unsigned int)(0xffffffffu - (unsigned int)p);
-                if (key > am) am = key;
-            }
-            if (rs[k] && finitef(u[k])) {
-                const unsigned long long key = ((unsigned long long)f2key(u[k]) << 32) | (unsigned int)p;
-                if (key < an) an = key;
-            }
-        }
-    }
-    sp = block_sum<double>(sp, sd);
-    sn = block_sum<double>(sn, sd);
-    const bool use_neg = (float)sn > (float)sp;
-    double vol = block_sum<double>(use_neg ? voln : volp, sd);
-    double cntd = block_sum<double>((double)(use_neg ? cntn : cntp), sd);
-    unsigned long long mx = block_max_u64(use_neg ? mxn : mxp, s64);
-    double period_px = pp.period_px, mm_per_px = pp.mm_per_px;
-    if (pp.pair_geom) { period_px = pp.pair_geom[b].period; mm_per_px = period_px > 1e-12 ? pp.grating_pitch_mm / period_px : 0.0; }
-    double area_px = mm_per_px * mm_per_px;
-    double volume_cm3 = cntd > 0 ? (double)(float)vol * area_px / 1000.0 : 0.0;
-    double area_mm2 = cntd * area_px;
-    double maxd = cntd > 0 ? (double)__uint_as_float((unsigned int)(mx >> 32)) : 0.0;
-    if (out3 && threadIdx.x == 0) { out3[b * 3] = volume_cm3; out3[b * 3 + 1] = area_mm2; out3[b * 3 + 2] = maxd; }
-    if (!scalars) return;
-    am = block_max_u64(am, s64);
-    if (unitless) an = block_min_u64(an, s64);
-    if (threadIdx.x == 0) {
-        double *S = scalars + b * (size_t)nscal;
-        S[0] = volume_cm3; S[1] = area_mm2; S[2] = maxd;
-        S[3] = curve_eval(pp.force_curve, volume_cm3);
-        S[4] = am ? (double)(0xffffffffu - (unsigned int)(am & 0xffffffffu)) : -1.0;
-        S[5] = period_px; S[6] = mm_per_px;
-        if (unitless && an != ~0ull) { S[7] = (double)key2f((unsigned int)(an >> 32)); S[8] = (double)(unsigned int)(an & 0xffffffffu); }
-        else { S[7] = (double)nanf32(); S[8] = -1.0; }
-    }
+    tail_frame([H](int p) { return H[p]; }, roi_frame ? roi_frame + b * (size_t)P : nullptr, unitless ? unitless + b * (size_t)P : nullptr, roi_static,
+               pp, scalars, nscal, out3, (int)b, P);
 }
 constexpr int TP_T = 256, TP_PX = 16, TP_WORDS = 10;
 __global__ __launch_bounds__(TP_T) void k_tail_part(const float *__restrict__ height_mm, const uint8_t *__restrict__ roi_frame,
diff --git a/vistaf-roboskin-vision-integrated-multimodal-sensor_amd/csrc/kernels.hpp b/vistaf-roboskin-vision-integrated-multimodal-sensor_amd/csrc/kernels.hpp
--- a/vistaf-roboskin-vision-integrated-multimodal-sensor_amd/csrc/kernels.hpp
+++ b/vistaf-roboskin-vision-integrated-multimodal-sensor_amd/csrc/kernels.hpp
@@ -16,6 +16,7 @@
     int big_gq_cap = 0;
     int big_fallback = 1;
     int telea_mw = 1;
+    int fused_backend = 1;
     int fused_chains = 1;
 };
 
@@ -208,4 +209,10 @@
 bool tstats_needs_big_scratch(int h, int w);
 void launch_tstats(const float *map, const uint8_t *valid, int h, int w, void *scratch, void *big_scratch, double *out, hipStream_t st);
 
+bool backend_fused_fits(int h, int w);
+void launch_backend_fused(float *depth, const uint8_t *cand, const unsigned int *gmax_bits, const float *unitless, const uint8_t *roi_static,
+                          const uint8_t *reliable, const int32_t *status, double min_peak_mm, double rel_frac, PostParams pp, int32_t *labels,
+                          unsigned int *peak_bits, uint8_t *kept, double *scalars, int nscal, float *out_h, uint8_t *out_r, int B, int h, int w,
+                          hipStream_t st);
+
 }
```

New measurement: 68180 frames/s (median of 6 runs). +1.2%, better.
